# astaka-pe/Dual-DMP

Hardware: AMD Instinct MI355X
Metric: training iters/sec + MAD score, 1M-face mesh @ 1/2/4/8 MI355X (higher is better)
Workload: dtype f32 (f16x3 split-MFMA GEMMs, f32 accumulate); 1 GPU; synthetic torus-grid manifold mesh, 1000000 faces / 500000 verts, float32 features, k=(3,4,4,4,1), bnfloop=1, native numbering (BASELINE.json configs[2]); faces=1000000, verts=500000, parallelism=1 GPU, hipgraph_replay=True, two_streams=True

## Files before the change

dual-dmp_amd/csrc/ddmp_internal.h:

```cpp
#pragma once
#include "../../include/ddmp_hip.h"
#ifdef __cplusplus
extern "C" {
#endif
int ddmp_bf16_to_f32(const uint16_t* in, float* out, int64_t n, ddmp_stream stream);
int ddmp_graph_tables(const ddmp_graph* g, const int32_t** rowptr, const int32_t** col, const float** dinv);
int ddmp_bn_bwd_apply_f32(const float* dZ, int64_t lddz, const float* Y, int64_t ldy, float* dY, int64_t lddy,
                          int64_t n_rows, int C, const float* scale, const float* shift, const float* c1,
                          const float* c0, float slope, double* dbias_sums , void* workspace,
                          size_t workspace_bytes, ddmp_stream stream);
int ddmp_gemm_nn_bf16(const uint16_t* A, int64_t lda, const float* W, int64_t ldw, uint16_t* Y, int64_t ldy,
                      int64_t n_rows, int M, int K, void* workspace, size_t workspace_bytes, ddmp_stream stream);
int ddmp_gemm_nt_bf16(const uint16_t* A, int64_t lda, const float* W, int64_t ldw, uint16_t* Y, int64_t ldy,
                      int64_t n_rows, int K, int M, const float* bias, const float* pro_scale, const float* pro_shift,
                      float slope, void* workspace, size_t workspace_bytes, ddmp_stream stream);
size_t ddmp_gemm_rows_bf16_workspace_bytes(int K, int M);
int ddmp_gemm_tn_bf16(const uint16_t* G, int64_t ldg, const uint16_t* Z, int64_t ldz, float* dW, int64_t lddw,
                      int64_t n_rows, int M, int K, const float* pro_scale, const float* pro_shift, float slope,
                      void* workspace, size_t workspace_bytes, ddmp_stream stream);
size_t ddmp_gemm_tn_bf16_workspace_bytes(int64_t n_rows, int M, int K);
int ddmp_head_bwd_bf16(const uint16_t* Y, int64_t ldy, int64_t n_rows, const float* scale, const float* shift,
                       float slope, const float* W1, const float* b1, const float* W2, const float* b2, int kind,
                       const float* dout, uint16_t* dZ, int64_t lddz, float* dW1, float* db1, float* dW2, float* db2,
                       void* workspace, size_t workspace_bytes, ddmp_stream stream);
int ddmp_head_bwd_f32(const float* Y, int64_t ldy, int64_t n_rows, const float* scale, const float* shift,
                      float slope, const float* W1, const float* b1, const float* W2, const float* b2,
                      int kind, const float* dout, float* dZ, int64_t lddz, float* dW1, float* db1,
                      float* dW2, float* db2, void* workspace, size_t workspace_bytes, ddmp_stream stream);
int ddmp_head_fwd_bf16(const uint16_t* Y, int64_t ldy, int64_t n_rows, const float* scale, const float* shift,
                       float slope, const float* W1, const float* b1, const float* W2, const float* b2, int kind,
                       const float* x_pos , float* out, ddmp_stream stream);
int ddmp_head_fwd_f32(const float* Y, int64_t ldy, int64_t n_rows, const float* scale, const float* shift,
                      float slope, const float* W1, const float* b1, const float* W2, const float* b2,
                      int kind, const float* x_pos , float* out, ddmp_stream stream);
int ddmp_spmm_bf16(const ddmp_graph* g, const uint16_t* X, int64_t ldx, uint16_t* Y, int64_t ldy, int C,
                   const float* bias, const float* pro_scale, const float* pro_shift, float slope, ddmp_stream stream);
int ddmp_spmm_bnbwd_bf16(const ddmp_graph* g, const uint16_t* dZ, int64_t lddz, const uint16_t* Yb, int64_t ldyb,
                         uint16_t* out, int64_t ld_out, int C, const float* a, const float* b, const float* c1,
                         const float* c0, float slope, ddmp_stream stream);
size_t ddmp_spmm_bnred_bf16_workspace_bytes(int64_t n_rows, int C);
size_t ddmp_spmm_bnred_workspace_bytes(int64_t n_rows, int C);
#ifdef __cplusplus
}

namespace ddmp {
struct CallCtx;
}
int ddmp_bn_stats(const void* Y, int64_t ldy, int64_t n_rows, int C, int dtype, double* sums, void* workspace,
                  size_t workspace_bytes, ddmp_stream stream, ddmp::CallCtx& ctx);
int ddmp_bn_stats_f32(const float* Y, int64_t ldy, int64_t n_rows, int C, double* sums, void* workspace, size_t workspace_bytes,
                      ddmp_stream stream, ddmp::CallCtx& ctx);
int ddmp_bn_stats_bf16(const uint16_t* Y, int64_t ldy, int64_t n_rows, int C, double* sums, void* workspace,
                       size_t workspace_bytes, ddmp_stream stream, ddmp::CallCtx& ctx);
int ddmp_bn_bwd_reduce(const void* dZ, int64_t lddz, const void* Y, int64_t ldy, int64_t n_rows, int C, int dtype,
                       const float* scale, const float* shift, const float* mean, const float* rstd, float slope, double* sums2,
                       void* workspace, size_t workspace_bytes, ddmp_stream stream, ddmp::CallCtx& ctx);
int ddmp_bn_bwd_reduce_f32(const float* dZ, int64_t lddz, const float* Y, int64_t ldy, int64_t n_rows, int C, const float* scale,
                           const float* shift, const float* mean, const float* rstd, float slope, double* sums2 ,
                           void* workspace, size_t workspace_bytes, ddmp_stream stream, ddmp::CallCtx& ctx);
int ddmp_bn_bwd_reduce_bf16(const uint16_t* dZ, int64_t lddz, const uint16_t* Y, int64_t ldy, int64_t n_rows, int C,
                            const float* scale, const float* shift, const float* mean, const float* rstd, float slope,
                            double* sums2, void* workspace, size_t workspace_bytes, ddmp_stream stream, ddmp::CallCtx& ctx);
int ddmp_spmm_stats(const ddmp_graph* g, const void* X, int64_t ldx, void* Y, int64_t ldy, int C, int dtype, const float* bias,
                    const float* pro_scale, const float* pro_shift, float slope, const float* ref, double* sums2, void* workspace,
                    size_t workspace_bytes, ddmp_stream stream, ddmp::CallCtx& ctx);
int ddmp_spmm_stats_f32(const ddmp_graph* g, const float* X, int64_t ldx, float* Y, int64_t ldy, int C, const float* bias,
                        const float* pro_scale, const float* pro_shift, float slope, const float* ref ,
                        double* sums2 , void* workspace, size_t workspace_bytes, ddmp_stream stream, ddmp::CallCtx& ctx);
int ddmp_spmm_stats_bf16(const ddmp_graph* g, const uint16_t* X, int64_t ldx, uint16_t* Y, int64_t ldy, int C,
                         const float* bias , const float* pro_scale , const float* pro_shift ,
                         float slope, const float* ref , double* sums2 , void* workspace,
                         size_t workspace_bytes, ddmp_stream stream, ddmp::CallCtx& ctx);
int ddmp_spmm_bnred(const ddmp_graph* g, const void* X, int64_t ldx, void* Y, int64_t ldy, int C, int dtype, const void* Yp,
                    int64_t ldyp, const float* scale, const float* shift, const float* mean, const float* rstd, float slope,
                    double* sums2, void* workspace, size_t workspace_bytes, ddmp_stream stream, ddmp::CallCtx& ctx);
int ddmp_spmm_bnred_f32(const ddmp_graph* g, const float* X, int64_t ldx, float* Y, int64_t ldy, int C, const float* Yp,
                        int64_t ldyp, const float* scale, const float* shift, const float* mean, const float* rstd, float slope,
                        double* sums2 , void* workspace, size_t workspace_bytes, ddmp_stream stream, ddmp::CallCtx& ctx);
int ddmp_spmm_bnred_bf16(const ddmp_graph* g, const uint16_t* X, int64_t ldx, uint16_t* Y, int64_t ldy, int C, const uint16_t* Yp,
                         int64_t ldyp, const float* scale, const float* shift, const float* mean, const float* rstd, float slope,
                         double* sums2 , void* workspace, size_t workspace_bytes, ddmp_stream stream, ddmp::CallCtx& ctx);
int ddmp_gemm_nt(const void* A, int64_t lda, const float* W, int64_t ldw, void* Y, int64_t ldy, int64_t n_rows, int K, int M,
                 int dtype, const float* bias, const float* pro_scale, const float* pro_shift, float slope, void* workspace,
                 size_t workspace_bytes, ddmp_stream stream, ddmp::CallCtx& ctx);
int ddmp_gemm_nt_f32(const float* A, int64_t lda, const float* W, int64_t ldw, float* Y, int64_t ldy, int64_t n_rows, int K,
                     int M, const float* bias, const float* pro_scale, const float* pro_shift, float slope, void* workspace,
                     size_t workspace_bytes, ddmp_stream stream, ddmp::CallCtx& ctx);
int ddmp_gemm_nn(const void* A, int64_t lda, const float* W, int64_t ldw, void* Y, int64_t ldy, int64_t n_rows, int M, int K,
                 int dtype, void* workspace, size_t workspace_bytes, ddmp_stream stream, ddmp::CallCtx& ctx);
int ddmp_gemm_nn_f32(const float* A, int64_t lda, const float* W, int64_t ldw, float* Y, int64_t ldy, int64_t n_rows, int M,
                     int K, void* workspace , size_t workspace_bytes, ddmp_stream stream, ddmp::CallCtx& ctx);
int ddmp_gemm_tn(const void* G, int64_t ldg, const void* Z, int64_t ldz, float* dW, int64_t lddw, int64_t n_rows, int M, int K,
                 int dtype, const float* pro_scale, const float* pro_shift, float slope, void* workspace, size_t workspace_bytes,
                 ddmp_stream stream, ddmp::CallCtx& ctx);
int ddmp_gemm_tn_f32(const float* G, int64_t ldg, const float* Z, int64_t ldz, float* dW, int64_t lddw, int64_t n_rows, int M,
                     int K, const float* pro_scale, const float* pro_shift, float slope, void* workspace, size_t workspace_bytes,
                     ddmp_stream stream, ddmp::CallCtx& ctx);
int ddmp_gemm_nt_stats_f32(const float* A, int64_t lda, const float* W, int64_t ldw, float* Y, int64_t ldy, int64_t n_rows, int K,
                           int M, const float* bias, const float* pro_scale, const float* pro_shift, float slope, double* sums2,
                           void* workspace, size_t workspace_bytes, void* stats_ws, size_t stats_ws_bytes, ddmp_stream stream,
                           ddmp::CallCtx& ctx);
int ddmp_gemm_nt_stats_bf16(const uint16_t* A, int64_t lda, const float* W, int64_t ldw, uint16_t* Y, int64_t ldy, int64_t n_rows,
                            int K, int M, const float* bias, const float* pro_scale, const float* pro_shift, float slope,
                            double* sums2, void* workspace, size_t workspace_bytes, void* stats_ws, size_t stats_ws_bytes,
                            ddmp_stream stream, ddmp::CallCtx& ctx);
int ddmp_gemm_nn_bnred_f32(const float* A, int64_t lda, const float* W, int64_t ldw, float* out, int64_t ld_out, int64_t n_rows,
                           int M, int K, const float* Yp, int64_t ldyp, const float* scale, const float* shift, const float* mean,
                           const float* rstd, float slope, double* sums2, void* workspace, size_t workspace_bytes, void* stats_ws,
                           size_t stats_ws_bytes, ddmp_stream stream, ddmp::CallCtx& ctx);
int ddmp_gemm_nn_bnbwd_f32(const float* dZ, int64_t lddz, const float* Yb, int64_t ldyb, const float* W, int64_t ldw, float* out,
                           int64_t ld_out, int64_t n_rows, int M, int K, const float* a, const float* b, const float* c1,
                           const float* c0, float slope, void* workspace, size_t workspace_bytes, ddmp_stream stream,
                           ddmp::CallCtx& ctx);
int ddmp_gemm_tn_bnbwd_f32(const float* dZ, int64_t lddz, const float* Yb, int64_t ldyb, const float* Z, int64_t ldz, float* dW,
                           int64_t lddw, int64_t n_rows, int M, int K, const float* a, const float* b, const float* c1,
                           const float* c0, const float* pro_scale, const float* pro_shift, float slope, void* workspace,
                           size_t workspace_bytes, ddmp_stream stream, ddmp::CallCtx& ctx);
#endif
```

dual-dmp_amd/csrc/gemm.hip:

```cpp
#include "ddmp_common.h"
#include "finalize.h"
#include "gemm_tn_rm.h"

#include <algorithm>
#include <cstdlib>
#include <type_traits>
#include <vector>

namespace {

using namespace ddmp;

typedef float f32x16 __attribute__((ext_vector_type(16)));

constexpr int kBM = 128;
constexpr int kBK = 32;
constexpr int kLd = kBK + 4;

template <int TN, bool B_KMAJOR, bool PRO>
__global__ __launch_bounds__(256) void gemm_rows_kernel(
    const float* __restrict__ A, int64_t lda, const float* __restrict__ B, int64_t ldb,
    float* __restrict__ Y, int64_t ldy, int n_rows, int KD, int MD,
    const float* __restrict__ bias, const float* __restrict__ pscale, const float* __restrict__ pshift,
    float slope, int n_row_tiles, int n_col_tiles) {
// ... 592 lines not shown
        if constexpr (PM == 0) {
            if (NJ == 4) {
                if (mode == 6) DDMP_PANEL_RS(3, 4); else DDMP_PANEL_RS(2, 4);
            } else {
                if (mode == 6) DDMP_PANEL_RS(3, 2); else DDMP_PANEL_RS(2, 2);
            }
        }
#undef DDMP_PANEL_RS
    } else if (WC == 4) {
        if (mode == 6) DDMP_PANEL(2, 4, 3, 4); else DDMP_PANEL(2, 4, 2, 4);
    } else if (WC == 2) {
        if (mode == 6) DDMP_PANEL(4, 2, 3, 4); else DDMP_PANEL(4, 2, 2, 4);
    } else {
        if (NJ == 4) {
            if (mode == 6) DDMP_PANEL(8, 1, 3, 4); else DDMP_PANEL(8, 1, 2, 4);
        } else if (NJ == 2) {
            if (mode == 6) DDMP_PANEL(8, 1, 3, 2); else DDMP_PANEL(8, 1, 2, 2);
        } else {
            if (mode == 6) DDMP_PANEL(8, 1, 3, 1); else DDMP_PANEL(8, 1, 2, 1);
        }
    }
#undef DDMP_PANEL
    if (stats && sums) {
        const size_t pbytes = ((size_t)n_row_tiles * WR * 2 * MP * sizeof(double) + 255) / 256 * 256;
        fpartials_reduce(stats, n_row_tiles * WR, MP, MD, (double*)((char*)stats + pbytes), sums, st, ctx.take_fin(MD));
    }
}

static inline bool ws_ok(int KD, int MD, const float* Y, int64_t ldy, const void* ws, size_t ws_bytes) {
    return ws_enabled() && KD % 32 == 0 && KD >= 96 && MD % 4 == 0 && MD <= 1024 && ldy % 4 == 0 &&
           (reinterpret_cast<uintptr_t>(Y) & 15) == 0 && ws && (reinterpret_cast<uintptr_t>(ws) & 15) == 0 &&
           ws_bytes >= ddmp_gemm_rows_workspace_bytes(KD, MD);
}

static int g_gemm_mode = -1, g_gemm_f16 = 0;
static int gemm_mode() {
    if (g_gemm_mode < 0) {
        const char* e = getenv("DDMP_GEMM_MODE");
        int m = e ? atoi(e) : 13;
        g_gemm_f16 = m == 13 ? m : 0;
        g_gemm_mode = (m == 0 || m == 3 || m == 6) ? m : 6;
    }
    return g_gemm_mode;
}
static int gemm_f16() {
    (void)gemm_mode();
    return g_gemm_f16;
}
extern "C" int ddmp_set_gemm_mode(int mode) {
    if (mode != 0 && mode != 3 && mode != 6 && mode != 13) return DDMP_EINVAL;
    g_gemm_f16 = mode > 10 ? mode : 0;
    g_gemm_mode = mode > 10 ? 6 : mode;
    return DDMP_OK;
}
extern "C" int ddmp_get_gemm_mode(void) { return gemm_f16() ? gemm_f16() : gemm_mode(); }

extern "C" int ddmp_gemm_scales_roll(float* slots, int n_slots, ddmp_stream stream) {
    ARG_TRY(slots && n_slots > 0);
    hipLaunchKernelGGL(f16s_roll_kernel, dim3((unsigned)cdiv(n_slots, 64)), dim3(64), 0, (hipStream_t)stream, slots, n_slots);
    LAUNCH_TRY();
    return DDMP_OK;
}

static inline bool aligned16(const void* p) { return (reinterpret_cast<uintptr_t>(p) & 15) == 0; }

extern "C" size_t ddmp_gemm_rows_workspace_bytes(int K, int M) {
    if (K <= 0 || M <= 0) return 0;
    const size_t kp = ((size_t)K + 127) / 128 * 128, mp = ((size_t)M + 127) / 128 * 128;
    return 3 * kp * mp * 2;
}

static bool presplit_w(const float* W, int64_t ldw, int M, int K, int transpose, void* ws, size_t ws_bytes,
                       hipStream_t st, bool prepared) {
    const int mode = gemm_mode();
    const int RK = transpose ? M : K;
    if (mode == 0 || !ws || ws_bytes < ddmp_gemm_rows_workspace_bytes(K, M) || RK % 8 != 0 ||
        (reinterpret_cast<uintptr_t>(ws) & 15))
        return false;
    const int grid = (int)std::min<int64_t>(cdiv((int64_t)M * K, 256), 1024);
    if (w_prepared(prepared, W, ldw, ws, kWPlain, mode == 6 ? 3 : 2, M, K, transpose, 0)) return true;
    if (mode == 6)
        hipLaunchKernelGGL((split_w_kernel<3>), dim3(grid), dim3(256), 0, st, W, ldw, M, K, transpose, (__bf16*)ws);
    else
        hipLaunchKernelGGL((split_w_kernel<2>), dim3(grid), dim3(256), 0, st, W, ldw, M, K, transpose, (__bf16*)ws);
    return hipGetLastError() == hipSuccess;
}

static WPrepDesc plan_w(int form, int64_t n_rows, const float* W, int64_t ldw, int M, int K, int has_pro, void* planes,
                        size_t planes_bytes) {
    WPrepDesc d{W, planes, ldw, 0, 0, 0, 0, 0, 0};
    const int mode = gemm_mode();
    if (mode == 0 || !planes || (reinterpret_cast<uintptr_t>(planes) & 15) || planes_bytes < ddmp_gemm_rows_workspace_bytes(K, M))
        return d;
    const int KD = form ? M : K, MD = form ? K : M;
    d.transpose = form ? 1 : 0;
    d.nterm = mode == 6 ? 3 : 2;
    float dummy;
    if (!(has_pro && KD > 512) && panel_ok(KD, MD, &dummy, MD, planes, planes_bytes, n_rows)) {
        const int WC = MD > 256 ? 4 : MD > 128 ? 2 : 1;
        const int NJ = MD > 128 ? 4 : MD > 64 ? 4 : MD > 32 ? 2 : 1;
        d.P = 32 * NJ * WC;
        d.MD = MD;
        d.KD = KD;
        if (mode == 6 && WC > 1 && gemm_f16()) {
            d.kind = kWPanelF16;
            d.nterm = 2;
        } else {
            d.kind = kWPanelB16;
        }
        return d;
    }
    if (ws_ok(KD, MD, (const float*)nullptr, 4, planes, planes_bytes)) {
        d.kind = kWTiled;
        d.MD = MD;
        d.KD = KD;
        d.P = 64 * (MD > 64 ? 2 : 1);
        return d;
    }
    if (KD % 8 == 0) {
        d.kind = kWPlain;
        d.MD = M;
        d.KD = K;
    }
    return d;
}

extern "C" int ddmp_gemm_forget_planes(const void* planes) {
    for (size_t e = 0; e < g_w_registry.size();)
        if (planes == nullptr || g_w_registry[e].planes == planes) g_w_registry.erase(g_w_registry.begin() + e); else ++e;
    return DDMP_OK;
}

extern "C" int ddmp_gemm_prepare_weights(int n, const float* const* W, const int64_t* ldw, const int* M, const int* K,
                                         const int* form, const int* has_pro, void* const* planes, const size_t* planes_bytes,
                                         int64_t n_rows, float* scratch, ddmp_stream stream) {
    ARG_TRY(n > 0 && n <= kWPrepMax && W && ldw && M && K && form && planes && planes_bytes && scratch && n_rows > 0);
    WPrepBatch b;
    b.n = 0;
    bool any_f16 = false;
    for (int i = 0; i < n; ++i) {
        ARG_TRY(W[i] && M[i] > 0 && K[i] > 0 && ldw[i] >= K[i] && aligned16(W[i]) && ldw[i] % 4 == 0);
        const WPrepDesc d = plan_w(form[i], n_rows, W[i], ldw[i], M[i], K[i], has_pro ? has_pro[i] : 0, planes[i], planes_bytes[i]);
        for (size_t e = 0; e < g_w_registry.size();)
            if (g_w_registry[e].planes == planes[i]) g_w_registry.erase(g_w_registry.begin() + e); else ++e;
        if (d.kind == 0) continue;
        any_f16 |= d.kind == kWPanelF16;
        b.d[b.n++] = d;
    }
    if (b.n == 0) return DDMP_OK;
    hipStream_t st = (hipStream_t)stream;
    if (any_f16) hipLaunchKernelGGL(wprep_max_kernel, dim3(8, (unsigned)b.n), dim3(256), 0, st, b, scratch);
    hipLaunchKernelGGL(wprep_split_kernel, dim3(128, (unsigned)b.n), dim3(256), 0, st, b, (const float*)scratch);
    LAUNCH_TRY();
    for (int i = 0; i < b.n; ++i) g_w_registry.push_back(b.d[i]);
    return DDMP_OK;
}

int ddmp_gemm_nt_f32(const float* A, int64_t lda, const float* W, int64_t ldw, float* Y, int64_t ldy, int64_t n_rows, int K,
                     int M, const float* bias, const float* pro_scale, const float* pro_shift, float slope, void* workspace,
                     size_t workspace_bytes, ddmp_stream stream, ddmp::CallCtx& ctx) {
    ARG_TRY(A && W && Y && n_rows > 0 && K > 0 && M > 0 && n_rows < INT32_MAX);
    ARG_TRY(K % 4 == 0 && lda % 4 == 0 && ldw % 4 == 0 && lda >= K && ldw >= K && ldy >= M);
    ARG_TRY(aligned16(A) && aligned16(W));
    ARG_TRY((pro_scale == nullptr) == (pro_shift == nullptr));
    ARG_TRY(!pro_scale || (aligned16(pro_scale) && aligned16(pro_shift)));
    hipStream_t st = (hipStream_t)stream;
    const int n_row_tiles = (int)cdiv(n_rows, kBM);
    const int TN = M > 64 ? 2 : 1;
    const int n_col_tiles = (int)cdiv(M, 64 * TN);
    dim3 grid((unsigned)(cdiv(n_row_tiles, kXcd) * kXcd * n_col_tiles)), block(256);
    if (gemm_mode() != 0 && !(pro_scale && K > 512) && panel_ok(K, M, Y, ldy, workspace, workspace_bytes, n_rows)) {
        if (pro_scale) launch_panel<1>(gemm_mode(), A, lda, nullptr, 0, W, ldw, 0, workspace, Y, ldy, (int)n_rows, K, M, bias, pro_scale, pro_shift, nullptr, nullptr, slope, st, nullptr, nullptr, ctx);
        else launch_panel<0>(gemm_mode(), A, lda, nullptr, 0, W, ldw, 0, workspace, Y, ldy, (int)n_rows, K, M, bias, nullptr, nullptr, nullptr, nullptr, slope, st, nullptr, nullptr, ctx);
        LAUNCH_TRY();
        return DDMP_OK;
    }
    if (gemm_mode() != 0 && !(pro_scale && K > 512) && ws_ok(K, M, Y, ldy, workspace, workspace_bytes)) {
        if (pro_scale) launch_ws<true>(gemm_mode(), A, lda, W, ldw, 0, workspace, Y, ldy, (int)n_rows, K, M, bias, pro_scale, pro_shift, slope, st, ctx.prepared);
        else launch_ws<false>(gemm_mode(), A, lda, W, ldw, 0, workspace, Y, ldy, (int)n_rows, K, M, bias, nullptr, nullptr, slope, st, ctx.prepared);
        LAUNCH_TRY();
        return DDMP_OK;
    }
    const bool pre = !(pro_scale && K > 512) && presplit_w(W, ldw, M, K, 0, workspace, workspace_bytes, st, ctx.prepared);
    const float* Bop = pre ? (const float*)workspace : W;
#define DDMP_LAUNCH_NT(KERNEL_, PRO_)                                                                    \
    hipLaunchKernelGGL((KERNEL_), grid, block, 0, st, A, lda, Bop, ldw, Y, ldy, (int)n_rows, K, M, bias, \
                       pro_scale, pro_shift, slope, n_row_tiles, n_col_tiles)
#define DDMP_NT_PICK(TN_, NTERM_, PRO_)                                                                   \
    do {                                                                                                  \
        if (pre && kt_) DDMP_LAUNCH_NT((gemm_rows_bf16_kernel<TN_, NTERM_, false, PRO_, true, true>), PRO_);   \
        else if (pre) DDMP_LAUNCH_NT((gemm_rows_bf16_kernel<TN_, NTERM_, false, PRO_, false, true>), PRO_);    \
        else if (kt_) DDMP_LAUNCH_NT((gemm_rows_bf16_kernel<TN_, NTERM_, false, PRO_, true, false>), PRO_);    \
        else DDMP_LAUNCH_NT((gemm_rows_bf16_kernel<TN_, NTERM_, false, PRO_, false, false>), PRO_);            \
    } while (0)
#define DDMP_NT_BY_MODE(TN_, PRO_)                                                          \
    do {                                                                                    \
        const int mode_ = (PRO_ && K > 512) ? 0 : gemm_mode();                              \
        const bool kt_ = (K % 16) != 0;                                                     \
        if (mode_ == 6) DDMP_NT_PICK(TN_, 3, PRO_);                                         \
        else if (mode_ == 3) DDMP_NT_PICK(TN_, 2, PRO_);                                    \
        else hipLaunchKernelGGL((gemm_rows_kernel<TN_, false, PRO_>), grid, block, 0, st, A, lda, W, ldw, Y, ldy,  \
                                (int)n_rows, K, M, bias, pro_scale, pro_shift, slope, n_row_tiles, n_col_tiles); \
    } while (0)
    if (TN == 2) {
        if (pro_scale) DDMP_NT_BY_MODE(2, true); else DDMP_NT_BY_MODE(2, false);
    } else {
        if (pro_scale) DDMP_NT_BY_MODE(1, true); else DDMP_NT_BY_MODE(1, false);
    }
#undef DDMP_NT_PICK
#undef DDMP_NT_BY_MODE
#undef DDMP_LAUNCH_NT
    LAUNCH_TRY();
    return DDMP_OK;
}
extern "C" int ddmp_gemm_nt_f32(const float* A, int64_t lda, const float* W, int64_t ldw, float* Y,
                                int64_t ldy, int64_t n_rows, int K, int M, const float* bias,
                                const float* pro_scale, const float* pro_shift, float slope,
                                void* workspace, size_t workspace_bytes, ddmp_stream stream) {
    ddmp::CallCtx ctx;
    return ddmp_gemm_nt_f32(A, lda, W, ldw, Y, ldy, n_rows, K, M, bias, pro_scale, pro_shift, slope, workspace, workspace_bytes,
                            stream, ctx);
}

int ddmp_gemm_nn_f32(const float* A, int64_t lda, const float* W, int64_t ldw, float* Y, int64_t ldy, int64_t n_rows, int M,
                     int K, void* workspace, size_t workspace_bytes, ddmp_stream stream, ddmp::CallCtx& ctx) {
    ARG_TRY(A && W && Y && n_rows > 0 && K > 0 && M > 0 && n_rows < INT32_MAX);
    ARG_TRY(M % 4 == 0 && K % 4 == 0 && lda % 4 == 0 && ldw % 4 == 0 && lda >= M && ldw >= K && ldy >= K);
    ARG_TRY(aligned16(A) && aligned16(W));
    hipStream_t st = (hipStream_t)stream;
    const int n_row_tiles = (int)cdiv(n_rows, kBM);
    const int TN = K > 64 ? 2 : 1;
    const int n_col_tiles = (int)cdiv(K, 64 * TN);
    dim3 grid((unsigned)(cdiv(n_row_tiles, kXcd) * kXcd * n_col_tiles)), block(256);
    if (gemm_mode() != 0 && panel_ok(M, K, Y, ldy, workspace, workspace_bytes, n_rows)) {
        launch_panel<0>(gemm_mode(), A, lda, nullptr, 0, W, ldw, 1, workspace, Y, ldy, (int)n_rows, M, K, nullptr, nullptr, nullptr, nullptr, nullptr, 0.f, st, nullptr, nullptr, ctx);
        LAUNCH_TRY();
        return DDMP_OK;
    }
    if (gemm_mode() != 0 && ws_ok(M, K, Y, ldy, workspace, workspace_bytes)) {
        launch_ws<false>(gemm_mode(), A, lda, W, ldw, 1, workspace, Y, ldy, (int)n_rows, M, K, nullptr, nullptr, nullptr, 0.f, st, ctx.prepared);
        LAUNCH_TRY();
        return DDMP_OK;
    }
    const bool pre = presplit_w(W, ldw, M, K, 1, workspace, workspace_bytes, st, ctx.prepared);
#define DDMP_LAUNCH_NN(KERNEL_)                                                                        \
    hipLaunchKernelGGL((KERNEL_), grid, block, 0, st, A, lda, W, ldw, Y, ldy, (int)n_rows, M, K, nullptr, \
                       nullptr, nullptr, 0.f, n_row_tiles, n_col_tiles)
#define DDMP_LAUNCH_NNP(KERNEL_)                                                                       \
    hipLaunchKernelGGL((KERNEL_), grid, block, 0, st, A, lda, (const float*)workspace, (int64_t)M, Y, ldy, \
                       (int)n_rows, M, K, nullptr, nullptr, nullptr, 0.f, n_row_tiles, n_col_tiles)
    const int mode = gemm_mode();
    const bool kt = (M % 16) != 0;
    if (pre) {
        if (TN == 2) {
            if (mode == 6 && kt) DDMP_LAUNCH_NNP((gemm_rows_bf16_kernel<2, 3, false, false, true, true>));
            else if (mode == 6) DDMP_LAUNCH_NNP((gemm_rows_bf16_kernel<2, 3, false, false, false, true>));
            else if (kt) DDMP_LAUNCH_NNP((gemm_rows_bf16_kernel<2, 2, false, false, true, true>));
            else DDMP_LAUNCH_NNP((gemm_rows_bf16_kernel<2, 2, false, false, false, true>));
        } else {
            if (mode == 6 && kt) DDMP_LAUNCH_NNP((gemm_rows_bf16_kernel<1, 3, false, false, true, true>));
            else if (mode == 6) DDMP_LAUNCH_NNP((gemm_rows_bf16_kernel<1, 3, false, false, false, true>));
            else if (kt) DDMP_LAUNCH_NNP((gemm_rows_bf16_kernel<1, 2, false, false, true, true>));
            else DDMP_LAUNCH_NNP((gemm_rows_bf16_kernel<1, 2, false, false, false, true>));
        }
    } else if (TN == 2) {
        if (mode == 6 && kt) DDMP_LAUNCH_NN((gemm_rows_bf16_kernel<2, 3, true, false, true, false>));
        else if (mode == 6) DDMP_LAUNCH_NN((gemm_rows_bf16_kernel<2, 3, true, false, false, false>));
        else if (mode == 3 && kt) DDMP_LAUNCH_NN((gemm_rows_bf16_kernel<2, 2, true, false, true, false>));
        else if (mode == 3) DDMP_LAUNCH_NN((gemm_rows_bf16_kernel<2, 2, true, false, false, false>));
        else DDMP_LAUNCH_NN((gemm_rows_kernel<2, true, false>));
    } else {
        if (mode == 6 && kt) DDMP_LAUNCH_NN((gemm_rows_bf16_kernel<1, 3, true, false, true, false>));
        else if (mode == 6) DDMP_LAUNCH_NN((gemm_rows_bf16_kernel<1, 3, true, false, false, false>));
        else if (mode == 3 && kt) DDMP_LAUNCH_NN((gemm_rows_bf16_kernel<1, 2, true, false, true, false>));
        else if (mode == 3) DDMP_LAUNCH_NN((gemm_rows_bf16_kernel<1, 2, true, false, false, false>));
        else DDMP_LAUNCH_NN((gemm_rows_kernel<1, true, false>));
    }
#undef DDMP_LAUNCH_NNP
#undef DDMP_LAUNCH_NN
    LAUNCH_TRY();
    return DDMP_OK;
}

static inline bool tn_wide_ok(int rows_per_split, int64_t ld0, int64_t ld1, int64_t ld2) {
    const int64_t r = (int64_t)rows_per_split + 64, lim = (int64_t)1 << 31;
    return r * ld0 * 4 < lim && r * ld1 * 4 < lim && r * ld2 * 4 < lim;
}
static void launch_tn_wide(const float* G, int64_t ldg, const float* G2, int64_t ldg2, const float* Z, int64_t ldz, float* part,
                           int64_t sstride, int64_t n_rows, int M, int K, const TnPlan& p, const float* ps, const float* psh,
                           const float* ga, const float* gb, const float* gk1, const float* gk0, float slope, float* gslot,
                           float* zslot, int target, int heal, hipStream_t st) {
    ddmp::TnRmArgs a;
    a.G = G; a.ldg = ldg; a.G2 = G2; a.ldg2 = ldg2; a.Z = Z; a.ldz = ldz; a.part = part; a.ld_out = K; a.split_stride = sstride;
    a.n_rows = (int)n_rows; a.M = M; a.K = K; a.rows_per_split = p.rows_per_split; a.n_tiles_m = p.n_tiles_m;
    a.n_tiles_k = p.n_tiles_k; a.n_splits = p.n_splits; a.pscale = ps; a.pshift = psh; a.ga = ga; a.gb = gb; a.gk1 = gk1;
    a.gk0 = gk0; a.slope = slope; a.gslot = gslot; a.zslot = zslot; a.target = target; a.heal = heal;
    a.tm = p.tm; a.tk = p.tk;
    ddmp::launch_tn_rm(a, st);
}

extern "C" size_t ddmp_gemm_tn_workspace_bytes(int64_t n_rows, int M, int K) {
    if (n_rows <= 0 || M <= 0 || K <= 0) return 0;
    const TnPlan p = tn_plan(n_rows, M, K), q = tn_plan(n_rows, M, K, true);
    return (size_t)std::max(p.n_splits, q.n_splits) * (size_t)M * (size_t)K * sizeof(float) + 64;
}

int ddmp_gemm_tn_f32(const float* G, int64_t ldg, const float* Z, int64_t ldz, float* dW, int64_t lddw, int64_t n_rows, int M,
                     int K, const float* pro_scale, const float* pro_shift, float slope, void* workspace, size_t workspace_bytes,
                     ddmp_stream stream, ddmp::CallCtx& ctx) {
    ARG_TRY(G && Z && dW && n_rows > 0 && M > 0 && K > 0 && n_rows < INT32_MAX);
    ARG_TRY(M % 4 == 0 && K % 4 == 0 && ldg % 4 == 0 && ldz % 4 == 0 && ldg >= M && ldz >= K && lddw >= K);
    ARG_TRY(aligned16(G) && aligned16(Z));
    ARG_TRY((pro_scale == nullptr) == (pro_shift == nullptr));
    ARG_TRY(!pro_scale || (aligned16(pro_scale) && aligned16(pro_shift)));
    hipStream_t st = (hipStream_t)stream;
    const bool f16_route = gemm_mode() == 6 && gemm_f16();
    TnPlan p = tn_plan(n_rows, M, K, f16_route);
    if (p.T == 4 && p.tm + p.tk < 512 && !tn_wide_ok(p.rows_per_split, ldg, 0, ldz)) p = tn_plan(n_rows, M, K);
    const size_t need = (size_t)p.n_splits * (size_t)M * (size_t)K * sizeof(float) + 64;
    if (!workspace || workspace_bytes < need) return DDMP_EWORKSPACE;
    float* part = (float*)workspace;
    const int64_t sstride = (int64_t)M * K;
    const int n_tiles = p.n_tiles_m * p.n_tiles_k;
    if (p.T == 4) {
        dim3 pgrid((unsigned)(cdiv(p.n_splits, kXcd) * kXcd * n_tiles)), pblock(512);
        float* gslot = nullptr;
        float* zslot = nullptr;
        int target = 0, heal_ = 0;
#define DDMP_LAUNCH_TNP(KERNEL_)                                                                              \
    hipLaunchKernelGGL((KERNEL_), pgrid, pblock, 0, st, G, ldg, (const float*)nullptr, (int64_t)0, Z, ldz, part, \
                       (int64_t)K, sstride, (int)n_rows, M, K, p.rows_per_split, p.n_tiles_m, p.n_tiles_k,       \
                       p.n_splits, pro_scale, pro_shift, (const float*)nullptr, (const float*)nullptr,           \
                       (const float*)nullptr, (const float*)nullptr, slope, gslot, zslot, target, heal_)
        const int mode_ = gemm_mode();
        if (mode_ == 6 && gemm_f16() && tn_wide_ok(p.rows_per_split, ldg, 0, ldz)) {
            float* tail = (float*)((char*)workspace + need - 64);
            const bool own = !(ctx.slot_a && ctx.slot_b);
            gslot = own ? tail : ctx.slot_a;
            zslot = own ? tail + 4 : ctx.slot_b;
            const bool prime = own || ctx.prime;
            target = prime ? kF16TargetExact : kF16TargetStale;
            if (prime) {
                f16s_measure<0>(G, ldg, nullptr, 0, n_rows, M, nullptr, nullptr, nullptr, nullptr, slope, gslot, st);
                if (pro_scale) f16s_measure<1>(Z, ldz, nullptr, 0, n_rows, K, pro_scale, pro_shift, nullptr, nullptr, slope, zslot, st);
                else f16s_measure<0>(Z, ldz, nullptr, 0, n_rows, K, nullptr, nullptr, nullptr, nullptr, slope, zslot, st);
            }
            for (heal_ = 0; heal_ <= (prime ? 0 : 1); ++heal_)
                launch_tn_wide(G, ldg, nullptr, 0, Z, ldz, part, sstride, n_rows, M, K, p, pro_scale, pro_shift, nullptr, nullptr,
                               nullptr, nullptr, slope, gslot, zslot, target, heal_, st);
            heal_ = 0;
        } else if (pro_scale) {
            if (mode_ == 6) DDMP_LAUNCH_TNP((gemm_tn_panel_kernel<3, true, false>)); else DDMP_LAUNCH_TNP((gemm_tn_panel_kernel<2, true, false>));
        } else {
            if (mode_ == 6) DDMP_LAUNCH_TNP((gemm_tn_panel_kernel<3, false, false>)); else DDMP_LAUNCH_TNP((gemm_tn_panel_kernel<2, false, false>));
        }
#undef DDMP_LAUNCH_TNP
        LAUNCH_TRY();
        hipLaunchKernelGGL(reduce_splits_kernel, dim3((unsigned)cdiv((int64_t)M * K, 256)), dim3(256), 0, st, part,
                           sstride, p.n_splits, dW, lddw, M, K);
        LAUNCH_TRY();
        return DDMP_OK;
    }
    dim3 grid((unsigned)(cdiv(p.n_splits, kXcd) * kXcd * n_tiles)), block(256);
#define DDMP_LAUNCH_TN(KERNEL_)                                                                           \
    hipLaunchKernelGGL((KERNEL_), grid, block, 0, st, G, ldg, Z, ldz, part, (int64_t)K, sstride, (int)n_rows, \
                       M, K, p.rows_per_split, p.n_tiles_m, p.n_tiles_k, p.n_splits, pro_scale, pro_shift, slope)
#define DDMP_TN_BY_MODE(T_, PRO_)                                                 \
    do {                                                                          \
        const int mode_ = gemm_mode();                                            \
        if (mode_ == 6) DDMP_LAUNCH_TN((gemm_tn_bf16_kernel<T_, 3, PRO_, (T_ == 1 ? 32 : 16)>));       \
        else if (mode_ == 3) DDMP_LAUNCH_TN((gemm_tn_bf16_kernel<T_, 2, PRO_, (T_ == 1 ? 32 : 16)>));  \
        else DDMP_LAUNCH_TN((gemm_tn_kernel<T_, PRO_>));                          \
    } while (0)
    if (p.T == 2) {
        if (pro_scale) DDMP_TN_BY_MODE(2, true); else DDMP_TN_BY_MODE(2, false);
    } else {
        if (pro_scale) DDMP_TN_BY_MODE(1, true); else DDMP_TN_BY_MODE(1, false);
    }
#undef DDMP_TN_BY_MODE
#undef DDMP_LAUNCH_TN
    LAUNCH_TRY();
    hipLaunchKernelGGL(reduce_splits_kernel, dim3((unsigned)cdiv((int64_t)M * K, 256)), dim3(256), 0, st, part,
                       sstride, p.n_splits, dW, lddw, M, K);
    LAUNCH_TRY();
    return DDMP_OK;
}


extern "C" int ddmp_gemm_nn_bnred_supported(int M, int K, int64_t n_rows) {
    if (gemm_mode() == 6 && gemm_f16() && rr_enabled() && panel_enabled() && n_rows >= kRRMinRows && M % 32 == 0 && M >= 64 &&
        M <= kMaxProK && K > 128 && K <= 512 && K % 4 == 0)
        return 1;
    static const bool narrow = !ddmp::unfused("dgrad_red_narrow");
    return (narrow && (gemm_mode() == 6 || gemm_mode() == 3) && panel_enabled() && n_rows >= kPanelMinRows && M % 32 == 0 &&
            M >= 32 && M <= kMaxProK && (K == 128 || K == 64)) ? 2 : 0;
}
int ddmp_gemm_nn_bnred_f32(const float* A, int64_t lda, const float* W, int64_t ldw, float* out, int64_t ld_out, int64_t n_rows,
                           int M, int K, const float* Yp, int64_t ldyp, const float* scale, const float* shift, const float* mean,
                           const float* rstd, float slope, double* sums2, void* workspace, size_t workspace_bytes, void* stats_ws,
                           size_t stats_ws_bytes, ddmp_stream stream, ddmp::CallCtx& ctx) {
    ARG_TRY(A && W && out && Yp && scale && shift && mean && rstd && sums2 && n_rows > 0 && n_rows < INT32_MAX);
    ARG_TRY(M % 4 == 0 && K % 4 == 0 && lda % 4 == 0 && ldw % 4 == 0 && lda >= M && ldw >= K && ld_out >= K && ldyp >= K);
    ARG_TRY(aligned16(A) && aligned16(W));
    const int form = ddmp_gemm_nn_bnred_supported(M, K, n_rows);
    if (!form || (form == 1 && !rr_route_ok(n_rows, M, lda, 0)) || !panel_ok(M, K, out, ld_out, workspace, workspace_bytes, n_rows))
        return DDMP_EINVAL;
    if (stats_ws_bytes < ddmp_gemm_nt_stats_workspace_bytes(n_rows, K)) return DDMP_EWORKSPACE;
    const float* bn4[4] = {scale, shift, mean, rstd};
    launch_panel<0>(gemm_mode(), A, lda, nullptr, 0, W, ldw, 1, workspace, out, ld_out, (int)n_rows, M, K, nullptr, nullptr, nullptr,
                    nullptr, nullptr, slope, (hipStream_t)stream, (double*)stats_ws, sums2, ctx, Yp, ldyp, bn4);
    LAUNCH_TRY();
    return DDMP_OK;
}
extern "C" int ddmp_gemm_nn_bnred_f32(const float* A, int64_t lda, const float* W, int64_t ldw, float* out, int64_t ld_out,
                                      int64_t n_rows, int M, int K, const float* Yp, int64_t ldyp, const float* scale,
                                      const float* shift, const float* mean, const float* rstd, float slope, double* sums2,
                                      void* workspace, size_t workspace_bytes, void* stats_ws, size_t stats_ws_bytes,
                                      ddmp_stream stream) {
    ddmp::CallCtx ctx;
    return ddmp_gemm_nn_bnred_f32(A, lda, W, ldw, out, ld_out, n_rows, M, K, Yp, ldyp, scale, shift, mean, rstd, slope, sums2,
                                  workspace, workspace_bytes, stats_ws, stats_ws_bytes, stream, ctx);
}

extern "C" int ddmp_gemm_bnbwd_supported(int cout, int cin, int64_t n_rows) {
    if (gemm_mode() == 0 || !panel_enabled() || !tn_panel_enabled() || n_rows < kTnPanelMinRows) return 0;
    const bool nn = cout % 32 == 0 && cout >= 64 && cout <= kMaxProK && cin % 4 == 0 && cin >= 16 && cin <= 512;
    const bool tn = cout % 4 == 0 && ((cout >= 256 && cin >= 256) || cin <= 128);
    static const bool narrow = !ddmp::unfused("bnbwd_narrow");
    return (nn && tn && (cin > 128 || narrow)) ? 1 : 0;
}

extern "C" int ddmp_gemm_tn_bnbwd_supported(int cout, int cin, int64_t n_rows) {
    if (gemm_mode() == 0 || !tn_panel_enabled() || n_rows < kTnPanelMinRows) return 0;
    const int mode_ = gemm_mode();
    const bool panel = cout >= 256 && cin >= 256;
    return (cout % 4 == 0 && cin % 4 == 0 && (panel || mode_ == 6 || mode_ == 3)) ? 1 : 0;
}

int ddmp_gemm_nn_bnbwd_f32(const float* dZ, int64_t lddz, const float* Yb, int64_t ldyb, const float* W, int64_t ldw, float* out,
                           int64_t ld_out, int64_t n_rows, int M, int K, const float* a, const float* b, const float* c1,
                           const float* c0, float slope, void* workspace, size_t workspace_bytes, ddmp_stream stream,
                           ddmp::CallCtx& ctx) {
    ARG_TRY(dZ && Yb && W && out && a && b && c1 && c0 && n_rows > 0 && n_rows < INT32_MAX && M > 0 && K > 0);
    ARG_TRY(lddz % 4 == 0 && ldyb % 4 == 0 && ldw % 4 == 0 && lddz >= M && ldyb >= M && ldw >= K && ld_out >= K);
    ARG_TRY(aligned16(dZ) && aligned16(Yb) && aligned16(W));
    if (!ddmp_gemm_bnbwd_supported(M, K, n_rows) || !panel_ok(M, K, out, ld_out, workspace, workspace_bytes, n_rows)) return DDMP_EINVAL;
    launch_panel<2>(gemm_mode(), dZ, lddz, Yb, ldyb, W, ldw, 1, workspace, out, ld_out, (int)n_rows, M, K, nullptr, a, b,
                    c1, c0, slope, (hipStream_t)stream, nullptr, nullptr, ctx);
    LAUNCH_TRY();
    return DDMP_OK;
}
extern "C" int ddmp_gemm_nn_bnbwd_f32(const float* dZ, int64_t lddz, const float* Yb, int64_t ldyb, const float* W,
                                      int64_t ldw, float* out, int64_t ld_out, int64_t n_rows, int M, int K,
                                      const float* a, const float* b, const float* c1, const float* c0, float slope,
                                      void* workspace, size_t workspace_bytes, ddmp_stream stream) {
    ddmp::CallCtx ctx;
    return ddmp_gemm_nn_bnbwd_f32(dZ, lddz, Yb, ldyb, W, ldw, out, ld_out, n_rows, M, K, a, b, c1, c0, slope, workspace,
                                  workspace_bytes, stream, ctx);
}

int ddmp_gemm_tn_bnbwd_f32(const float* dZ, int64_t lddz, const float* Yb, int64_t ldyb, const float* Z, int64_t ldz, float* dW,
                           int64_t lddw, int64_t n_rows, int M, int K, const float* a, const float* b, const float* c1,
                           const float* c0, const float* pro_scale, const float* pro_shift, float slope, void* workspace,
                           size_t workspace_bytes, ddmp_stream stream, ddmp::CallCtx& ctx) {
    ARG_TRY(dZ && Yb && Z && dW && a && b && c1 && c0 && n_rows > 0 && n_rows < INT32_MAX && M > 0 && K > 0);
    ARG_TRY(M % 4 == 0 && K % 4 == 0 && lddz >= M && ldyb >= M && ldz >= K && lddw >= K);
    ARG_TRY((pro_scale == nullptr) == (pro_shift == nullptr));
    if (!ddmp_gemm_tn_bnbwd_supported(M, K, n_rows)) return DDMP_EINVAL;
    hipStream_t st = (hipStream_t)stream;
    const bool f16_route = gemm_mode() == 6 && gemm_f16() && lddz % 4 == 0 && ldyb % 4 == 0 && ldz % 4 == 0 && aligned16(dZ) &&
                           aligned16(Yb) && aligned16(Z);
    TnPlan p = tn_plan(n_rows, M, K, f16_route);
    if (p.T == 4 && p.tm + p.tk < 512 && !tn_wide_ok(p.rows_per_split, lddz, ldyb, ldz)) p = tn_plan(n_rows, M, K);
    const size_t need = (size_t)p.n_splits * (size_t)M * (size_t)K * sizeof(float) + 64;
    if (!workspace || workspace_bytes < need) return DDMP_EWORKSPACE;
    float* part = (float*)workspace;
    const int64_t sstride = (int64_t)M * K;
    const int n_tiles = p.n_tiles_m * p.n_tiles_k;
    if (p.T != 4) {
        const int mode_ = gemm_mode();
        if (mode_ != 6 && mode_ != 3) return DDMP_EINVAL;
        dim3 grid((unsigned)(cdiv(p.n_splits, kXcd) * kXcd * n_tiles)), block(256);
#define DDMP_LAUNCH_TNG(T_, NT_, PRO_)                                                                                 \
    hipLaunchKernelGGL((gemm_tn_bf16_kernel<T_, NT_, PRO_, (T_ == 1 ? 32 : 16), true>), grid, block, 0, st, dZ, lddz, Z, ldz,  \
                       part, (int64_t)K, sstride, (int)n_rows, M, K, p.rows_per_split, p.n_tiles_m, p.n_tiles_k,       \
                       p.n_splits, pro_scale, pro_shift, slope, Yb, ldyb, a, b, c1, c0)
        if (p.T == 2) {
            if (mode_ == 6) { if (pro_scale) DDMP_LAUNCH_TNG(2, 3, true); else DDMP_LAUNCH_TNG(2, 3, false); }
            else { if (pro_scale) DDMP_LAUNCH_TNG(2, 2, true); else DDMP_LAUNCH_TNG(2, 2, false); }
        } else {
            if (mode_ == 6) { if (pro_scale) DDMP_LAUNCH_TNG(1, 3, true); else DDMP_LAUNCH_TNG(1, 3, false); }
            else { if (pro_scale) DDMP_LAUNCH_TNG(1, 2, true); else DDMP_LAUNCH_TNG(1, 2, false); }
        }
#undef DDMP_LAUNCH_TNG
        LAUNCH_TRY();
        hipLaunchKernelGGL(reduce_splits_kernel, dim3((unsigned)cdiv((int64_t)M * K, 256)), dim3(256), 0, st, part, sstride,
                           p.n_splits, dW, lddw, M, K);
        LAUNCH_TRY();
        return DDMP_OK;
    }
    dim3 pgrid((unsigned)(cdiv(p.n_splits, kXcd) * kXcd * n_tiles)), pblock(512);
    float* gslot = nullptr;
    float* zslot = nullptr;
    int target = 0, heal_ = 0;
#define DDMP_LAUNCH_TNP(KERNEL_)                                                                                 \
    hipLaunchKernelGGL((KERNEL_), pgrid, pblock, 0, st, dZ, lddz, Yb, ldyb, Z, ldz, part, (int64_t)K, sstride,     \
                       (int)n_rows, M, K, p.rows_per_split, p.n_tiles_m, p.n_tiles_k, p.n_splits, pro_scale,       \
                       pro_shift, a, b, c1, c0, slope, gslot, zslot, target, heal_)
    const int mode_ = gemm_mode();
    if (mode_ == 6 && gemm_f16() && lddz % 4 == 0 && ldyb % 4 == 0 && ldz % 4 == 0 && tn_wide_ok(p.rows_per_split, lddz, ldyb, ldz) &&
        aligned16(dZ) && aligned16(Yb) && aligned16(Z)) {
        float* tail = (float*)((char*)workspace + need - 64);
        const bool own = !(ctx.slot_a && ctx.slot_b);
        gslot = own ? tail : ctx.slot_a;
        zslot = own ? tail + 4 : ctx.slot_b;
        const bool prime = own || ctx.prime;
        target = prime ? kF16TargetExact : kF16TargetStale;
        if (prime) {
            f16s_measure<2>(dZ, lddz, Yb, ldyb, n_rows, M, a, b, c1, c0, slope, gslot, st);
            if (pro_scale) f16s_measure<1>(Z, ldz, nullptr, 0, n_rows, K, pro_scale, pro_shift, nullptr, nullptr, slope, zslot, st);
            else f16s_measure<0>(Z, ldz, nullptr, 0, n_rows, K, nullptr, nullptr, nullptr, nullptr, slope, zslot, st);
        }
        for (heal_ = 0; heal_ <= (prime ? 0 : 1); ++heal_)
            launch_tn_wide(dZ, lddz, Yb, ldyb, Z, ldz, part, sstride, n_rows, M, K, p, pro_scale, pro_shift, a, b, c1, c0, slope,
                           gslot, zslot, target, heal_, st);
        heal_ = 0;
    } else if (pro_scale) {
        if (mode_ == 6) DDMP_LAUNCH_TNP((gemm_tn_panel_kernel<3, true, true>)); else DDMP_LAUNCH_TNP((gemm_tn_panel_kernel<2, true, true>));
    } else {
        if (mode_ == 6) DDMP_LAUNCH_TNP((gemm_tn_panel_kernel<3, false, true>)); else DDMP_LAUNCH_TNP((gemm_tn_panel_kernel<2, false, true>));
    }
#undef DDMP_LAUNCH_TNP
    LAUNCH_TRY();
    hipLaunchKernelGGL(reduce_splits_kernel, dim3((unsigned)cdiv((int64_t)M * K, 256)), dim3(256), 0, st, part, sstride,
                       p.n_splits, dW, lddw, M, K);
    LAUNCH_TRY();
    return DDMP_OK;
}
extern "C" int ddmp_gemm_tn_bnbwd_f32(const float* dZ, int64_t lddz, const float* Yb, int64_t ldyb, const float* Z,
                                      int64_t ldz, float* dW, int64_t lddw, int64_t n_rows, int M, int K,
                                      const float* a, const float* b, const float* c1, const float* c0,
                                      const float* pro_scale, const float* pro_shift, float slope, void* workspace,
                                      size_t workspace_bytes, ddmp_stream stream) {
    ddmp::CallCtx ctx;
    return ddmp_gemm_tn_bnbwd_f32(dZ, lddz, Yb, ldyb, Z, ldz, dW, lddw, n_rows, M, K, a, b, c1, c0, pro_scale, pro_shift, slope,
                                  workspace, workspace_bytes, stream, ctx);
}


extern "C" size_t ddmp_gemm_nt_stats_workspace_bytes(int64_t n_rows, int M) {
    if (n_rows <= 0 || M <= 0) return 0;
    const size_t fused = (size_t)(cdiv(n_rows, 64) + 8) * 2 * 512 * sizeof(double) + 256 + fpartials_mid_bytes(512);
    return std::max(fused, ddmp_colreduce_workspace_bytes(n_rows, M));
}

int ddmp_gemm_nt_stats_f32(const float* A, int64_t lda, const float* W, int64_t ldw, float* Y, int64_t ldy, int64_t n_rows, int K,
                           int M, const float* bias, const float* pro_scale, const float* pro_shift, float slope, double* sums2,
                           void* workspace, size_t workspace_bytes, void* stats_ws, size_t stats_ws_bytes, ddmp_stream stream,
                           ddmp::CallCtx& ctx) {
    ARG_TRY(sums2 && stats_ws);
    if (stats_ws_bytes < ddmp_gemm_nt_stats_workspace_bytes(n_rows, M)) return DDMP_EWORKSPACE;
    const bool fused = A && W && Y && n_rows > 0 && n_rows < INT32_MAX && K > 0 && M > 0 && K % 4 == 0 && lda % 4 == 0 &&
                       ldw % 4 == 0 && lda >= K && ldw >= K && ldy >= M && aligned16(A) && aligned16(W) &&
                       (pro_scale == nullptr) == (pro_shift == nullptr) && gemm_mode() != 0 && !(pro_scale && K > 512) &&
                       panel_ok(K, M, Y, ldy, workspace, workspace_bytes, n_rows);
    if (fused) {
        hipStream_t st = (hipStream_t)stream;
        if (pro_scale) launch_panel<1>(gemm_mode(), A, lda, nullptr, 0, W, ldw, 0, workspace, Y, ldy, (int)n_rows, K, M, bias, pro_scale, pro_shift, nullptr, nullptr, slope, st, (double*)stats_ws, sums2, ctx);
        else launch_panel<0>(gemm_mode(), A, lda, nullptr, 0, W, ldw, 0, workspace, Y, ldy, (int)n_rows, K, M, bias, nullptr, nullptr, nullptr, nullptr, slope, st, (double*)stats_ws, sums2, ctx);
        LAUNCH_TRY();
        return DDMP_OK;
    }
    int rc = ddmp_gemm_nt_f32(A, lda, W, ldw, Y, ldy, n_rows, K, M, bias, pro_scale, pro_shift, slope, workspace,
                              workspace_bytes, stream, ctx);
    if (rc != DDMP_OK) return rc;
    return ddmp_bn_stats_f32(Y, ldy, n_rows, M, sums2, stats_ws, stats_ws_bytes, stream, ctx);
}
extern "C" int ddmp_gemm_nt_stats_f32(const float* A, int64_t lda, const float* W, int64_t ldw, float* Y, int64_t ldy,
                                      int64_t n_rows, int K, int M, const float* bias, const float* pro_scale,
                                      const float* pro_shift, float slope, double* sums2, void* workspace,
                                      size_t workspace_bytes, void* stats_ws, size_t stats_ws_bytes,
                                      ddmp_stream stream) {
    ddmp::CallCtx ctx;
    return ddmp_gemm_nt_stats_f32(A, lda, W, ldw, Y, ldy, n_rows, K, M, bias, pro_scale, pro_shift, slope, sums2, workspace,
                                  workspace_bytes, stats_ws, stats_ws_bytes, stream, ctx);
}
```

dual-dmp_amd/csrc/head.hip:

```cpp
#include "b16_common.h"

#include <algorithm>

namespace {

using namespace ddmp;

constexpr int H0 = 32, H1 = 16, H2 = 3;
constexpr int kNPar = H1 * H0 + H1 + H2 * H1 + H2;

struct HeadW {
    const float *W1, *b1, *W2, *b2;
};

__device__ __forceinline__ void load_row32(const float* __restrict__ yrow, float (&y)[H0]) {
#pragma unroll
    for (int q = 0; q < H0 / 4; ++q) {
        const float4 v = *reinterpret_cast<const float4*>(yrow + q * 4);
        y[q * 4 + 0] = v.x; y[q * 4 + 1] = v.y; y[q * 4 + 2] = v.z; y[q * 4 + 3] = v.w;
    }
}
__device__ __forceinline__ void load_row32(const bf16_t* __restrict__ yrow, float (&y)[H0]) {
#pragma unroll
    for (int q = 0; q < H0 / 8; ++q) {
        float t[8];
        bf_unpack8(ld8b(yrow + q * 8), t);
#pragma unroll
        for (int e = 0; e < 8; ++e) y[q * 8 + e] = t[e];
    }
}
__device__ __forceinline__ void store_quad(float* p, const float (&d)[4]) {
    *reinterpret_cast<float4*>(p) = make_float4(d[0], d[1], d[2], d[3]);
}
__device__ __forceinline__ void store_quad(bf16_t* p, const float (&d)[4]) {
    *reinterpret_cast<uint2*>(p) = make_uint2(bf_pack(d[0], d[1]), bf_pack(d[2], d[3]));
}

template <typename T>
__device__ __forceinline__ void head_forward_row(const T* __restrict__ yrow, const float* __restrict__ scale,
                                                 const float* __restrict__ shift, float slope, const HeadW& w,
                                                 float (&z)[H0], float (&tp)[H1], float (&u)[H2]) {
    load_row32(yrow, z);
#pragma unroll
    for (int j = 0; j < H0; ++j) z[j] = lrelu(fmaf(z[j], scale[j], shift[j]), slope);
#pragma unroll
    for (int i = 0; i < H1; ++i) {
        float s = w.b1[i];
#pragma unroll
        for (int j = 0; j < H0; ++j) s = fmaf(w.W1[i * H0 + j], z[j], s);
        tp[i] = s;
    }
#pragma unroll
    for (int o = 0; o < H2; ++o) {
        float s = w.b2[o];
#pragma unroll
        for (int i = 0; i < H1; ++i) s = fmaf(w.W2[o * H1 + i], lrelu(tp[i], slope), s);
        u[o] = s;
    }
}

template <typename T>
__global__ __launch_bounds__(256) void head_fwd_kernel(const T* __restrict__ Y, int64_t ldy, int n_rows,
                                                       const float* __restrict__ scale,
                                                       const float* __restrict__ shift, float slope, HeadW w,
                                                       int kind, const float* __restrict__ x_pos,
                                                       float* __restrict__ out) {
    for (int row = blockIdx.x * 256 + threadIdx.x; row < n_rows; row += gridDim.x * 256) {
        float z[H0], tp[H1], u[H2];
        head_forward_row(Y + (int64_t)row * ldy, scale, shift, slope, w, z, tp, u);
        float* o = out + (int64_t)row * 3;
        if (kind == 0) {
            const float* xp = x_pos + (int64_t)row * 3;
            o[0] = xp[0] + u[0];
            o[1] = xp[1] + u[1];
            o[2] = xp[2] + u[2];
        } else {
            const float v0 = tanhf(u[0]), v1 = tanhf(u[1]), v2 = tanhf(u[2]);
            const float r = sqrtf(v0 * v0 + v1 * v1 + v2 * v2);
            const float s = 1.0f / (r + 1.0e-12f);
            o[0] = v0 * s;
            o[1] = v1 * s;
            o[2] = v2 * s;
        }
    }
}

template <typename T>
__global__ __launch_bounds__(256) void head_bwd_kernel(const T* __restrict__ Y, int64_t ldy, int n_rows,
                                                       const float* __restrict__ scale,
                                                       const float* __restrict__ shift, float slope, HeadW w,
                                                       int kind, const float* __restrict__ dout,
                                                       T* __restrict__ dZ, int64_t lddz,
                                                       float* __restrict__ partial ) {
    __shared__ float zs[256][H0 + 1];
    __shared__ float dtps[256][H1 + 1];
    __shared__ float ts[256][H1 + 1];
    __shared__ float dus[256][4];
    const int tid = threadIdx.x;
    const int w1_j = tid & 31, w1_i = tid >> 5;
    float accA = 0.f, accB = 0.f;
    float accC = 0.f;

    const int n_tiles = (n_rows + 255) / 256;
    for (int tile = blockIdx.x; tile < n_tiles; tile += gridDim.x) {
        const int row = tile * 256 + tid;
        float z[H0], tp[H1], u[H2], du[H2], dtp[H1];
        if (row < n_rows) {
            head_forward_row(Y + (int64_t)row * ldy, scale, shift, slope, w, z, tp, u);
            const float* g = dout + (int64_t)row * 3;
            if (kind == 0) {
                du[0] = g[0]; du[1] = g[1]; du[2] = g[2];
            } else {
                const float v0 = tanhf(u[0]), v1 = tanhf(u[1]), v2 = tanhf(u[2]);
                const float r = sqrtf(v0 * v0 + v1 * v1 + v2 * v2);
                const float s = 1.0f / (r + 1.0e-12f);
                const float gv = g[0] * v0 + g[1] * v1 + g[2] * v2;
                const float k = r > 0.f ? s * s * gv / r : 0.f;
                du[0] = (s * g[0] - k * v0) * (1.f - v0 * v0);
                du[1] = (s * g[1] - k * v1) * (1.f - v1 * v1);
                du[2] = (s * g[2] - k * v2) * (1.f - v2 * v2);
            }
#pragma unroll
            for (int i = 0; i < H1; ++i) {
                float s = 0.f;
#pragma unroll
                for (int o = 0; o < H2; ++o) s = fmaf(w.W2[o * H1 + i], du[o], s);
                dtp[i] = s * lrelu_grad(tp[i], slope);
            }
            T* dz = dZ + (int64_t)row * lddz;
#pragma unroll
            for (int q = 0; q < H0 / 4; ++q) {
                float d[4];
#pragma unroll
                for (int e = 0; e < 4; ++e) {
                    float s = 0.f;
#pragma unroll
                    for (int i = 0; i < H1; ++i) s = fmaf(w.W1[i * H0 + q * 4 + e], dtp[i], s);
                    d[e] = s;
                }
                store_quad(dz + q * 4, d);
            }
        } else {
#pragma unroll
            for (int j = 0; j < H0; ++j) z[j] = 0.f;
#pragma unroll
            for (int i = 0; i < H1; ++i) { tp[i] = 0.f; dtp[i] = 0.f; }
            du[0] = du[1] = du[2] = 0.f;
        }
        __syncthreads();
#pragma unroll
        for (int j = 0; j < H0; ++j) zs[tid][j] = z[j];
#pragma unroll
        for (int i = 0; i < H1; ++i) {
            dtps[tid][i] = dtp[i];
            ts[tid][i] = row < n_rows ? lrelu(tp[i], slope) : 0.f;
        }
        dus[tid][0] = du[0]; dus[tid][1] = du[1]; dus[tid][2] = du[2];
        __syncthreads();
        for (int r = 0; r < 256; ++r) {
            const float zj = zs[r][w1_j];
            accA = fmaf(dtps[r][w1_i], zj, accA);
            accB = fmaf(dtps[r][w1_i + 8], zj, accB);
        }
        if (tid < H2 * H1) {
            const int o = tid / H1, i = tid % H1;
            for (int r = 0; r < 256; ++r) accC = fmaf(dus[r][o], ts[r][i], accC);
        } else if (tid >= 64 && tid < 64 + H1) {
            for (int r = 0; r < 256; ++r) accC += dtps[r][tid - 64];
        } else if (tid >= 128 && tid < 128 + H2) {
            for (int r = 0; r < 256; ++r) accC += dus[r][tid - 128];
        }
    }
    float* p = partial + (int64_t)blockIdx.x * kNPar;
    p[w1_i * H0 + w1_j] = accA;
    p[(w1_i + 8) * H0 + w1_j] = accB;
    if (tid < H2 * H1) p[H1 * H0 + H1 + tid] = accC;
    else if (tid >= 64 && tid < 64 + H1) p[H1 * H0 + (tid - 64)] = accC;
    else if (tid >= 128 && tid < 128 + H2) p[H1 * H0 + H1 + H2 * H1 + (tid - 128)] = accC;
}

__global__ __launch_bounds__(256) void head_reduce_kernel(const float* __restrict__ partial, int nblk,
                                                          float* __restrict__ dW1, float* __restrict__ db1,
                                                          float* __restrict__ dW2, float* __restrict__ db2) {
    __shared__ double sm[256];
    const int i = blockIdx.x * 32 + (threadIdx.x & 31), sl = threadIdx.x >> 5;
    double s = 0.0;
    if (i < kNPar)
        for (int b = sl; b < nblk; b += 8) s += (double)partial[(int64_t)b * kNPar + i];
    sm[threadIdx.x] = s;
    __syncthreads();
    if (sl != 0 || i >= kNPar) return;
    double r = 0.0;
#pragma unroll
    for (int u = 0; u < 8; ++u) r += sm[threadIdx.x + 32 * u];
    const float v = (float)r;
    if (i < H1 * H0) dW1[i] = v;
    else if (i < H1 * H0 + H1) db1[i - H1 * H0] = v;
    else if (i < H1 * H0 + H1 + H2 * H1) dW2[i - H1 * H0 - H1] = v;
    else db2[i - H1 * H0 - H1 - H2 * H1] = v;
}

int head_bwd_blocks(int64_t n_rows) { return (int)std::max<int64_t>(1, std::min<int64_t>(512, cdiv(n_rows, 256))); }

}

extern "C" int ddmp_head_fwd_f32(const float* Y, int64_t ldy, int64_t n_rows, const float* scale,
                                 const float* shift, float slope, const float* W1, const float* b1,
                                 const float* W2, const float* b2, int kind, const float* x_pos, float* out,
                                 ddmp_stream stream) {
    ARG_TRY(Y && scale && shift && W1 && b1 && W2 && b2 && out && n_rows > 0 && n_rows < INT32_MAX);
    ARG_TRY(ldy >= H0 && ldy % 4 == 0 && (kind == 0 || kind == 1) && (kind == 1 || x_pos));
    const int grid = (int)std::min<int64_t>(cdiv(n_rows, 256), 256 * 8);
    HeadW w{W1, b1, W2, b2};
    hipLaunchKernelGGL(head_fwd_kernel<float>, dim3(grid), dim3(256), 0, (hipStream_t)stream, Y, ldy, (int)n_rows, scale,
                       shift, slope, w, kind, x_pos, out);
    LAUNCH_TRY();
    return DDMP_OK;
}

extern "C" size_t ddmp_head_bwd_workspace_bytes(int64_t n_rows) {
    if (n_rows <= 0) return 0;
    return (size_t)head_bwd_blocks(n_rows) * kNPar * sizeof(float);
}

extern "C" int ddmp_head_bwd_f32(const float* Y, int64_t ldy, int64_t n_rows, const float* scale,
                                 const float* shift, float slope, const float* W1, const float* b1,
                                 const float* W2, const float* b2, int kind, const float* dout, float* dZ,
                                 int64_t lddz, float* dW1, float* db1, float* dW2, float* db2, void* ws,
                                 size_t ws_bytes, ddmp_stream stream) {
    ARG_TRY(Y && scale && shift && W1 && b1 && W2 && b2 && dout && dZ && dW1 && db1 && dW2 && db2);
    ARG_TRY(n_rows > 0 && n_rows < INT32_MAX && ldy >= H0 && ldy % 4 == 0 && lddz >= H0 && lddz % 4 == 0);
    ARG_TRY(kind == 0 || kind == 1);
    const int nblk = head_bwd_blocks(n_rows);
    if (!ws || ws_bytes < (size_t)nblk * kNPar * sizeof(float)) return DDMP_EWORKSPACE;
    HeadW w{W1, b1, W2, b2};
    hipLaunchKernelGGL(head_bwd_kernel<float>, dim3(nblk), dim3(256), 0, (hipStream_t)stream, Y, ldy, (int)n_rows, scale,
                       shift, slope, w, kind, dout, dZ, lddz, (float*)ws);
    LAUNCH_TRY();
    hipLaunchKernelGGL(head_reduce_kernel, dim3((unsigned)cdiv(kNPar, 32)), dim3(256), 0, (hipStream_t)stream,
                       (const float*)ws, nblk, dW1, db1, dW2, db2);
    LAUNCH_TRY();
    return DDMP_OK;
}


extern "C" int ddmp_head_fwd_bf16(const uint16_t* Y, int64_t ldy, int64_t n_rows, const float* scale, const float* shift,
                                  float slope, const float* W1, const float* b1, const float* W2, const float* b2,
                                  int kind, const float* x_pos, float* out, ddmp_stream stream) {
    ARG_TRY(Y && scale && shift && W1 && b1 && W2 && b2 && out && n_rows > 0 && n_rows < INT32_MAX);
    ARG_TRY(ldy >= H0 && ldy % 8 == 0 && b16_aligned(Y) && (kind == 0 || kind == 1) && (kind == 1 || x_pos));
    const int grid = (int)std::min<int64_t>(cdiv(n_rows, 256), 256 * 8);
    HeadW w{W1, b1, W2, b2};
    hipLaunchKernelGGL(head_fwd_kernel<bf16_t>, dim3(grid), dim3(256), 0, (hipStream_t)stream, Y, ldy, (int)n_rows, scale,
                       shift, slope, w, kind, x_pos, out);
    LAUNCH_TRY();
    return DDMP_OK;
}

extern "C" int ddmp_head_bwd_bf16(const uint16_t* Y, int64_t ldy, int64_t n_rows, const float* scale, const float* shift,
                                  float slope, const float* W1, const float* b1, const float* W2, const float* b2,
                                  int kind, const float* dout, uint16_t* dZ, int64_t lddz, float* dW1, float* db1,
                                  float* dW2, float* db2, void* ws, size_t ws_bytes, ddmp_stream stream) {
    ARG_TRY(Y && scale && shift && W1 && b1 && W2 && b2 && dout && dZ && dW1 && db1 && dW2 && db2);
    ARG_TRY(n_rows > 0 && n_rows < INT32_MAX && ldy >= H0 && ldy % 8 == 0 && lddz >= H0 && lddz % 8 == 0);
    ARG_TRY((kind == 0 || kind == 1) && b16_aligned(Y) && b16_aligned(dZ));
    const int nblk = head_bwd_blocks(n_rows);
    if (!ws || ws_bytes < (size_t)nblk * kNPar * sizeof(float)) return DDMP_EWORKSPACE;
    HeadW w{W1, b1, W2, b2};
    hipLaunchKernelGGL(head_bwd_kernel<bf16_t>, dim3(nblk), dim3(256), 0, (hipStream_t)stream, Y, ldy, (int)n_rows, scale,
                       shift, slope, w, kind, dout, dZ, lddz, (float*)ws);
    LAUNCH_TRY();
    hipLaunchKernelGGL(head_reduce_kernel, dim3((unsigned)cdiv(kNPar, 32)), dim3(256), 0, (hipStream_t)stream,
                       (const float*)ws, nblk, dW1, db1, dW2, db2);
    LAUNCH_TRY();
    return DDMP_OK;
}
```

dual-dmp_amd/csrc/opts.hip:

```cpp
#include "ddmp_common.h"
#include "finalize.h"

namespace {
using ddmp::FinalizeArgs;

struct OptCall {
    int err = DDMP_OK;
    ddmp::CallCtx ctx;
    const double* sums;
    ddmp_stream stream;
    OptCall(const ddmp_opts* o, ddmp_stream stream_, const double* sums_ = nullptr, int width = 0) : sums(sums_), stream(stream_) {
        if (o) err = fill(*o, width);
    }
    int fill(const ddmp_opts& o, int width) {
        ARG_TRY(o.struct_size >= sizeof(ddmp_opts));
        ARG_TRY(!(o.flags & ~(DDMP_OPT_BN_FWD | DDMP_OPT_BN_BWD | DDMP_OPT_SCALES | DDMP_OPT_PREPARED)));
        ARG_TRY(!((o.flags & DDMP_OPT_BN_FWD) && (o.flags & DDMP_OPT_BN_BWD)));
        if (o.flags & (DDMP_OPT_BN_FWD | DDMP_OPT_BN_BWD)) {
            FinalizeArgs& f = ctx.fin;
            f.kind = (o.flags & DDMP_OPT_BN_FWD) ? 1 : 2;
            f.C = o.bn_C; f.n_total = o.bn_n_total; f.eps = o.bn_eps; f.momentum = o.bn_momentum;
            for (int i = 0; i < 3; ++i) f.in[i] = o.bn_in[i];
            for (int i = 0; i < 6; ++i) f.out[i] = o.bn_out[i];
            ARG_TRY(sums && f.C == width && f.n_total > 0 && f.C > 0 && f.in[0] && f.in[1] && f.out[0] && f.out[1] && f.out[2] && f.out[3]);
            if (f.kind == 1) ARG_TRY((f.out[4] == nullptr) == (f.out[5] == nullptr));
            else ARG_TRY(f.in[2]);
        }
        if (o.flags & DDMP_OPT_SCALES) {
            ctx.slot_a = o.slot_a; ctx.slot_b = o.slot_b; ctx.prime = o.prime;
        }
        ctx.prepared = (o.flags & DDMP_OPT_PREPARED) != 0;
        return DDMP_OK;
    }
    int finish(int rc) {
        const FinalizeArgs& f = ctx.fin;
        if (rc != DDMP_OK || f.kind == 0 || ctx.fin_done) return rc;
        if (f.kind == 1)
            return ddmp_bn_prepare_f32(sums, f.n_total, f.C, f.in[0], f.in[1], f.eps, f.momentum, f.out[0], f.out[1], f.out[2],
                                       f.out[3], f.out[4], f.out[5], stream);
        return ddmp_bn_bwd_prepare_f32(sums, f.n_total, f.C, f.in[0], f.in[1], f.in[2], f.out[0], f.out[1], f.out[2], f.out[3], stream);
    }
};
}

extern "C" int ddmp_bn_stats_o(const void* Y, int64_t ldy, int64_t n_rows, int C, int dtype, double* sums, void* workspace, size_t workspace_bytes, ddmp_stream stream, const ddmp_opts* opts) {
    OptCall c(opts, stream, sums, C);
    if (c.err) return c.err;
    return c.finish(ddmp_bn_stats(Y, ldy, n_rows, C, dtype, sums, workspace, workspace_bytes, stream, c.ctx));
}

extern "C" int ddmp_bn_bwd_reduce_o(const void* dZ, int64_t lddz, const void* Y, int64_t ldy, int64_t n_rows, int C, int dtype, const float* scale, const float* shift, const float* mean, const float* rstd, float slope, double* sums2, void* workspace, size_t workspace_bytes, ddmp_stream stream, const ddmp_opts* opts) {
    OptCall c(opts, stream, sums2, C);
    if (c.err) return c.err;
    return c.finish(ddmp_bn_bwd_reduce(dZ, lddz, Y, ldy, n_rows, C, dtype, scale, shift, mean, rstd, slope, sums2, workspace, workspace_bytes, stream, c.ctx));
}

extern "C" int ddmp_spmm_stats_o(const ddmp_graph* g, const void* X, int64_t ldx, void* Y, int64_t ldy, int C, int dtype, const float* bias, const float* pro_scale, const float* pro_shift, float slope, const float* ref, double* sums2, void* workspace, size_t workspace_bytes, ddmp_stream stream, const ddmp_opts* opts) {
    OptCall c(opts, stream, sums2, C);
    if (c.err) return c.err;
    return c.finish(ddmp_spmm_stats(g, X, ldx, Y, ldy, C, dtype, bias, pro_scale, pro_shift, slope, ref, sums2, workspace, workspace_bytes, stream, c.ctx));
}

extern "C" int ddmp_spmm_bnred_o(const ddmp_graph* g, const void* X, int64_t ldx, void* Y, int64_t ldy, int C, int dtype, const void* Yp, int64_t ldyp, const float* scale, const float* shift, const float* mean, const float* rstd, float slope, double* sums2, void* workspace, size_t workspace_bytes, ddmp_stream stream, const ddmp_opts* opts) {
    OptCall c(opts, stream, sums2, C);
    if (c.err) return c.err;
    return c.finish(ddmp_spmm_bnred(g, X, ldx, Y, ldy, C, dtype, Yp, ldyp, scale, shift, mean, rstd, slope, sums2, workspace, workspace_bytes, stream, c.ctx));
}

extern "C" int ddmp_gemm_nt_o(const void* A, int64_t lda, const float* W, int64_t ldw, void* Y, int64_t ldy, int64_t n_rows, int K, int M, int dtype, const float* bias, const float* pro_scale, const float* pro_shift, float slope, void* workspace, size_t workspace_bytes, ddmp_stream stream, const ddmp_opts* opts) {
    OptCall c(opts, stream);
    if (c.err) return c.err;
    return c.finish(ddmp_gemm_nt(A, lda, W, ldw, Y, ldy, n_rows, K, M, dtype, bias, pro_scale, pro_shift, slope, workspace, workspace_bytes, stream, c.ctx));
}

extern "C" int ddmp_gemm_nn_o(const void* A, int64_t lda, const float* W, int64_t ldw, void* Y, int64_t ldy, int64_t n_rows, int M, int K, int dtype, void* workspace, size_t workspace_bytes, ddmp_stream stream, const ddmp_opts* opts) {
    OptCall c(opts, stream);
    if (c.err) return c.err;
    return c.finish(ddmp_gemm_nn(A, lda, W, ldw, Y, ldy, n_rows, M, K, dtype, workspace, workspace_bytes, stream, c.ctx));
}

extern "C" int ddmp_gemm_tn_o(const void* G, int64_t ldg, const void* Z, int64_t ldz, float* dW, int64_t lddw, int64_t n_rows, int M, int K, int dtype, const float* pro_scale, const float* pro_shift, float slope, void* workspace, size_t workspace_bytes, ddmp_stream stream, const ddmp_opts* opts) {
    OptCall c(opts, stream);
    if (c.err) return c.err;
    return c.finish(ddmp_gemm_tn(G, ldg, Z, ldz, dW, lddw, n_rows, M, K, dtype, pro_scale, pro_shift, slope, workspace, workspace_bytes, stream, c.ctx));
}

extern "C" int ddmp_gemm_nt_stats_f32_o(const float* A, int64_t lda, const float* W, int64_t ldw, float* Y, int64_t ldy, int64_t n_rows, int K, int M, const float* bias , const float* pro_scale , const float* pro_shift , float slope, double* sums2 , void* workspace, size_t workspace_bytes, void* stats_ws, size_t stats_ws_bytes, ddmp_stream stream, const ddmp_opts* opts) {
    OptCall c(opts, stream, sums2, M);
    if (c.err) return c.err;
    return c.finish(ddmp_gemm_nt_stats_f32(A, lda, W, ldw, Y, ldy, n_rows, K, M, bias, pro_scale, pro_shift, slope, sums2, workspace, workspace_bytes, stats_ws, stats_ws_bytes, stream, c.ctx));
}

extern "C" int ddmp_gemm_nt_stats_bf16_o(const uint16_t* A, int64_t lda, const float* W, int64_t ldw, uint16_t* Y, int64_t ldy, int64_t n_rows, int K, int M, const float* bias, const float* pro_scale, const float* pro_shift, float slope, double* sums2, void* workspace, size_t workspace_bytes, void* stats_ws, size_t stats_ws_bytes, ddmp_stream stream, const ddmp_opts* opts) {
    OptCall c(opts, stream, sums2, M);
    if (c.err) return c.err;
    return c.finish(ddmp_gemm_nt_stats_bf16(A, lda, W, ldw, Y, ldy, n_rows, K, M, bias, pro_scale, pro_shift, slope, sums2, workspace, workspace_bytes, stats_ws, stats_ws_bytes, stream, c.ctx));
}

extern "C" int ddmp_gemm_nn_bnred_f32_o(const float* A, int64_t lda, const float* W, int64_t ldw, float* out, int64_t ld_out, int64_t n_rows, int M, int K, const float* Yp, int64_t ldyp, const float* scale, const float* shift, const float* mean, const float* rstd, float slope, double* sums2, void* workspace, size_t workspace_bytes, void* stats_ws, size_t stats_ws_bytes, ddmp_stream stream, const ddmp_opts* opts) {
    OptCall c(opts, stream, sums2, K);
    if (c.err) return c.err;
    return c.finish(ddmp_gemm_nn_bnred_f32(A, lda, W, ldw, out, ld_out, n_rows, M, K, Yp, ldyp, scale, shift, mean, rstd, slope, sums2, workspace, workspace_bytes, stats_ws, stats_ws_bytes, stream, c.ctx));
}

extern "C" int ddmp_gemm_nn_bnbwd_f32_o(const float* dZ, int64_t lddz, const float* Yb, int64_t ldyb, const float* W, int64_t ldw, float* out, int64_t ld_out, int64_t n_rows, int M, int K, const float* a, const float* b, const float* c1, const float* c0, float slope, void* workspace, size_t workspace_bytes, ddmp_stream stream, const ddmp_opts* opts) {
    OptCall c(opts, stream);
    if (c.err) return c.err;
    return c.finish(ddmp_gemm_nn_bnbwd_f32(dZ, lddz, Yb, ldyb, W, ldw, out, ld_out, n_rows, M, K, a, b, c1, c0, slope, workspace, workspace_bytes, stream, c.ctx));
}

extern "C" int ddmp_gemm_tn_bnbwd_f32_o(const float* dZ, int64_t lddz, const float* Yb, int64_t ldyb, const float* Z, int64_t ldz, float* dW, int64_t lddw, int64_t n_rows, int M, int K, const float* a, const float* b, const float* c1, const float* c0, const float* pro_scale , const float* pro_shift , float slope, void* workspace, size_t workspace_bytes, ddmp_stream stream, const ddmp_opts* opts) {
    OptCall c(opts, stream);
    if (c.err) return c.err;
    return c.finish(ddmp_gemm_tn_bnbwd_f32(dZ, lddz, Yb, ldyb, Z, ldz, dW, lddw, n_rows, M, K, a, b, c1, c0, pro_scale, pro_shift, slope, workspace, workspace_bytes, stream, c.ctx));
}
```

dual-dmp_amd/engine.py:

```python
from __future__ import annotations

import math
from typing import List, Optional

import os

import torch

from . import ops
from .ops import SLOPE

def _unfused(name):
    f = getattr(ops, "unfused", None)
    return bool(f and f(name))


POS_WIDTHS = [16, 32, 64, 128, 256, 256, 512, 512, 256, 256, 128, 64, 32, 16, 3]
NORM_WIDTHS = [7, 32, 64, 128, 256, 256, 512, 512, 256, 256, 128, 64, 32, 16, 3]


def _pad4(c):
    return (c + 3) // 4 * 4


# ... 100 lines not shown
                a = math.sqrt(6.0 / (true[0] + true[1]))
                v[:, :true[1]].copy_(torch.empty(true).uniform_(-a, a, generator=generator))
            elif name.startswith("bn") and name.endswith("weight"):
                v.fill_(1.0)
            elif name.startswith("linear"):
                fan_in = 32 if name.startswith("linear1") else 16
                b = 1.0 / math.sqrt(fan_in)
                v.copy_(torch.empty(stored).uniform_(-b, b, generator=generator))
        with torch.no_grad():
            arena.copy_(cpu.to(arena.device))


class GcnEngine:

    def __init__(self, graph: ops.Graph, widths: List[int], kind: int, x0: torch.Tensor,
                 x_pos: Optional[torch.Tensor] = None, comm=None, n_total: Optional[int] = None,
                 perm: Optional[torch.Tensor] = None, dtype: torch.dtype = torch.float32, split=None, overlap: bool = False):
        if dtype not in (torch.float32, torch.bfloat16):
            raise ValueError("feature dtype must be torch.float32 or torch.bfloat16")
        self.dtype = dtype
        self.g = graph
        self.overlap = bool(overlap)
        self.split = None
        if self.overlap and split is not None and 0 < split[2] < graph.n_rows:
            self.split = tuple(split)
            self.n_int = int(split[2])
        self._halo_ahead = None
        self.kind = kind
        self.layout = ArenaLayout(widths)
        self.comm = comm or NoComm()
        self.n_rows, self.n_cols = graph.n_rows, graph.n_cols
        self.n_total = float(n_total if n_total is not None else graph.n_rows)
        dev = x0.device
        self.device = dev
        L = self.layout
        assert x0.shape[0] >= self.n_cols and x0.shape[1] == L.cin[0]
        self.x0 = torch.zeros((self.n_cols, L.cin_p[0]), dtype=dtype, device=dev)
        self.x0[:, :L.cin[0]] = x0[:self.n_cols].to(dtype)
        self.x_pos = None if x_pos is None else x_pos[:self.n_rows].contiguous().to(torch.float32)
        eq_agg = not _unfused("equal_width")
        self.agg_first = [L.cin_p[l] < L.cout[l] or (eq_agg and L.cin_p[l] == L.cout[l]) for l in range(12)]
        supported = getattr(ops, "gemm_bnbwd_supported", None)
        def _bnbwd_ok(l):
            if not supported or l == 0 or not self.agg_first[l]:
                return False
            if dtype == torch.float32:
                return supported(L.cout[l], L.cin_p[l], self.n_rows)
            try:
                return supported(L.cout[l], L.cin_p[l], self.n_rows, dtype) and not _unfused("bf16_gemm")
            except TypeError:
                return False
        self.fuse_bnbwd = [bool(_bnbwd_ok(l)) for l in range(12)]
        tn_ok = getattr(ops, "gemm_tn_bnbwd_supported", None)
        self.fuse_bnbwd0 = bool(tn_ok and self.agg_first[0] and tn_ok(L.cout[0], L.cin_p[0], self.n_rows, dtype)
                                and not _unfused("bnbwd_l0"))
        gather_ok = getattr(ops, "spmm_bnbwd_supported", None)
        few_entries = dtype == torch.float32 or getattr(graph, "max_row_nnz", 99) <= 4
        self.fuse_gather_bwd = [bool(gather_ok) and isinstance(self.comm, NoComm) and not self.agg_first[l] and l > 0
                                and gather_ok(L.cout[l]) and few_entries and not _unfused("gather_bwd")
                                for l in range(12)]
        cmax = max(L.cout)
        nc = self.n_cols

        def buf(c):
            return torch.empty((nc, c), dtype=dtype, device=dev)

        self.Y = [buf(L.cout[l]) for l in range(12)]
        self.P = [buf(L.cin_p[l]) if self.agg_first[l] else None for l in range(12)]
        self._flat = [torch.empty(nc * cmax, dtype=dtype, device=dev) for _ in range(6)]
        self.bn4 = [torch.zeros((4, L.cout[l]), dtype=torch.float32, device=dev) for l in range(12)]
        st_ok = getattr(ops, "spmm_stats_supported", None)
        self.fuse_spmm_stats = [bool(st_ok) and not self.agg_first[l] and st_ok(L.cout[l], dtype)
                                and not _unfused("stats") for l in range(12)]
        self.c10s = [torch.empty((2, L.cout[l]), dtype=torch.float32, device=dev) for l in range(12)]
        self._wplanes = None
        self._prep_weights = (dtype == torch.float32 and hasattr(ops, "gemm_prepare_weights")
                              and not _unfused("wprep"))
        self._tail_fused = (isinstance(self.comm, NoComm) and hasattr(ops, "BnFwd")
                            and not _unfused("tail"))
        self.scale_slots = torch.zeros((12, 2, 4), dtype=torch.float32, device=dev)
        self._slot = [[self.scale_slots[l, o] for o in range(2)] for l in range(12)]
        self._prime = True
        self._f16 = False
        self.sums = torch.empty(2 * cmax, dtype=torch.float64, device=dev)
        self.sums_b = torch.empty(2 * cmax, dtype=torch.float64, device=dev) if self.split else None
        self.running = [torch.zeros((2, L.cout[l]), dtype=torch.float32, device=dev) for l in range(12)]
        for r in self.running:
            r[1].fill_(1.0)
        self.num_batches_tracked = torch.zeros(12, dtype=torch.int64, device=dev)
        self.out = torch.empty((self.n_rows, 3), dtype=torch.float32, device=dev)
        self._p1_ready = False
        self.perm = self.inv = None
        if perm is not None:
            self.perm = perm.to(dev)
            self.inv = torch.empty_like(self.perm)
            self.inv[self.perm] = torch.arange(self.n_rows, device=dev)
            self.out_orig = torch.empty_like(self.out)

    def __del__(self):
        try:
            planes = getattr(self, "_wplanes", None)
            if planes and hasattr(ops, "gemm_forget_planes"):
                for buf in planes.values():
                    ops.gemm_forget_planes(buf)
        except Exception:
            pass

    def _work(self, i, c):
        return self._flat[i][: self.n_cols * c].view(self.n_cols, c)

    def _scales(self, l, a, b=None):
        if self._f16:
            return {"scales": (self._slot[l][a], None if b is None else self._slot[l][b], self._prime)}
        return {}

    def check_scales(self) -> int:
        cnt = self.scale_slots[:, :, 3]
        c = cnt.cpu()
        if bool((c < 0).any()):
            where = [(int(l), int(o)) for l, o in (c < 0).nonzero().tolist()]
            cnt.zero_()
            raise OverflowError("non-finite GEMM operand (layer, operand): %s -- NaN or inf in the activations / "
                                "gradients of the last iterations" % where)
        healed = int(c.sum().item())
        if healed:
            cnt.zero_()
        return healed

    @staticmethod
    def _drain(steps):
        for h in steps:
            if h is not None:
                h.wait()

    def forward(self, params: torch.Tensor, update_running: bool = True, use_running: bool = False) -> torch.Tensor:
        self._drain(self.forward_steps(params, update_running, use_running))
        return self.result

    def backward(self, params: torch.Tensor, grads: torch.Tensor, dout: torch.Tensor) -> torch.Tensor:
        self._drain(self.backward_steps(params, grads, dout))
        return grads

    def _bn4_from_running(self, l, gamma, beta):
        rm, rv = self.running[l][0], self.running[l][1]
        rstd = torch.rsqrt(rv + ops.BN_EPS)
        b = self.bn4[l]
        b[0] = gamma * rstd
        b[1] = beta - rm * b[0]
        b[2] = rm
        b[3] = rstd

    def _prepare_weights(self, params: torch.Tensor):
        if not self._prep_weights:
            return
        L = self.layout
        if self._wplanes is None:
            need = ops.gemm_rows_workspace_bytes
            self._wplanes = {(l, form): torch.empty(need(L.cin_p[l], L.cout[l]), dtype=torch.uint8, device=self.device)
                             for l in range(12) for form in (0, 1) if not (form == 1 and l == 0)}
            self._wscratch = torch.empty(8 * len(self._wplanes), dtype=torch.float32, device=self.device)
            self._wplan = (None, None)
        if self._wplan[0] != params.data_ptr():
            items = []
            for (l, form), buf in self._wplanes.items():
                W = L.view(params, "conv%d.lin.weight" % (l + 1), true_shape=False)
                items.append((W, form, form == 0 and not self.agg_first[l] and l > 0, buf))
            self._wplan = (params.data_ptr(), ops.WeightPlan(items, self.n_rows, self._wscratch))
        self._wplan[1].run()

    def _wp(self, l, form):
        return {} if self._wplanes is None else {"wplanes": self._wplanes[(l, form)]}

    def _start_halo(self, t):
        comm, n = self.comm, self.n_rows
        start = getattr(comm, "start_halo_overlapped", None)
        if start is None or os.environ.get("DDMP_DIST_SPLIT") == "noverlap":
            h = comm.start_halo(t, n)
            if h is not None:
                h.wait()
            return None
        return start(t, n)

    def _halves(self):
        g_int, g_bnd, ni = self.split
        return ((g_int, 0, ni, self.sums), (g_bnd, ni, self.n_rows, self.sums_b))

    def _add_sums(self, width):
        if self.split:
            self.sums[:width] += self.sums_b[:width]

    def _agg(self, launch, h):
        if self.split:
            for k, (gh, r0, r1, sums) in enumerate(self._halves()):
                if k == 1:
                    yield h
                launch(gh, r0, r1, sums)
        else:
            yield h
            launch(self.g, 0, self.n_rows, self.sums)

    def forward_steps(self, params: torch.Tensor, update_running: bool = True, use_running: bool = False):
        L, g, n, comm = self.layout, self.g, self.n_rows, self.comm
        self.n_forward = getattr(self, "n_forward", 0) + 1
        self._f16 = hasattr(ops, "gemm_scales_roll") and self.dtype == torch.float32 and ops.get_gemm_mode() == 13
        self._prepare_weights(params)
        X, pro = self.x0, None
        halo_started = False
        tail = self._tail_fused and not use_running
        for l in range(12):
            i = l + 1
            W = L.view(params, "conv%d.lin.weight" % i, true_shape=False)
            b = L.view(params, "conv%d.bias" % i)
            Y = self.Y[l]
            bnk = {"bn": ops.BnFwd(self.n_total, L.view(params, "bn%d.weight" % i), L.view(params, "bn%d.bias" % i), self.bn4[l],
                                   running=(self.running[l][0], self.running[l][1]) if update_running else None)} if tail else {}
            if self.agg_first[l]:
                P = self.P[l]
                if self.overlap and l > 0:
                    h = self._halo_ahead if halo_started else self._start_halo(X)
                    self._halo_ahead = None
                    yield from self._agg(lambda gh, r0, r1, _: ops.spmm(gh, X, out=P[r0:r1], pro=pro), h)
                elif l > 0 or not self._p1_ready:
                    if l > 0 and not halo_started:
                        yield comm.start_halo(X, n)
                    ops.spmm(g, X, out=P[:n], pro=pro)
                    self._p1_ready = True
                if hasattr(ops, "gemm_nt_stats"):
                    ops.gemm_nt_stats(P, W, self.sums, out=Y, bias=b, n_rows=n, **self._wp(l, 0), **self._scales(l, 0), **bnk)
                else:
                    ops.gemm_nt(P, W, out=Y, bias=b, n_rows=n)
                    ops.bn_stats(Y, sums=self.sums, n_rows=n, **bnk)
            else:
                H = self._work(0, L.cout[l])
                ops.gemm_nt(X, W, out=H, pro=pro, n_rows=n, **self._wp(l, 0), **self._scales(l, 0))
                if self.overlap:
                    if self.fuse_spmm_stats[l]:
                        yield from self._agg(lambda gh, r0, r1, sums: ops.spmm_stats(gh, H, Y[r0:r1], self.bn4[l][2], sums, bias=b),
                                             self._start_halo(H))
                        self._add_sums(2 * L.cout[l])
                    else:
                        yield from self._agg(lambda gh, r0, r1, _: ops.spmm(gh, H, out=Y[r0:r1], bias=b), self._start_halo(H))
                        ops.bn_stats(Y, sums=self.sums, n_rows=n, **bnk)
                else:
                    yield comm.start_halo(H, n)
                    if self.fuse_spmm_stats[l]:
                        ops.spmm_stats(g, H, Y[:n], self.bn4[l][2], self.sums, bias=b, **bnk)
                    else:
                        ops.spmm(g, H, out=Y[:n], bias=b)
                        ops.bn_stats(Y, sums=self.sums, n_rows=n, **bnk)
            halo_started = l < 11 and self.agg_first[l + 1]
            fused = None if self.overlap else getattr(comm, "halo_and_sums", None)
            if self.overlap:
                yield comm.start_all_reduce(self.sums[: 2 * L.cout[l]])
                if halo_started:
                    self._halo_ahead = self._start_halo(Y)
            elif halo_started and fused is not None and fused(Y, n, self.sums[: 2 * L.cout[l]]):
                yield None
            else:
                h_stats = comm.start_all_reduce(self.sums[: 2 * L.cout[l]])
                h_halo = comm.start_halo(Y, n) if halo_started else None
                yield _Both(h_stats, h_halo)
            if use_running:
                self._bn4_from_running(l, L.view(params, "bn%d.weight" % i), L.view(params, "bn%d.bias" % i))
            elif not tail:
                ops.bn_prepare(self.sums, self.n_total, L.view(params, "bn%d.weight" % i), L.view(params, "bn%d.bias" % i),
                               self.bn4[l], running=(self.running[l][0], self.running[l][1]) if update_running else None)
            X, pro = Y, (self.bn4[l][0], self.bn4[l][1])
        if update_running:
            self.num_batches_tracked += 1
        ops.head_fwd(self.Y[11], self.bn4[11], L.view(params, "linear1.weight"), L.view(params, "linear1.bias"),
                     L.view(params, "linear2.weight"), L.view(params, "linear2.bias"), self.kind, self.x_pos,
                     self.out, n_rows=n)
        self.result = self.out
        if self.inv is not None:
            torch.index_select(self.out, 0, self.inv, out=self.out_orig)
            self.result = self.out_orig

    def backward_steps(self, params: torch.Tensor, grads: torch.Tensor, dout: torch.Tensor):
        L, g, n, comm = self.layout, self.g, self.n_rows, self.comm
        free = list(range(len(self._flat)))

        def take(c):
            k = free.pop(0)
            return k, self._work(k, c)

        def release(k):
            free.append(k)

        def wgrad(l, fn, *bufs):
            fn()

        kz, dZ = take(32)
        if self.perm is not None:
            dout = dout.index_select(0, self.perm)
        tail = self._tail_fused

        def arm(l):
            if tail:
                return {"bn": ops.BnBwd(self.n_total, self.bn4[l], L.view(grads, "bn%d.weight" % (l + 1)),
                                        L.view(grads, "bn%d.bias" % (l + 1)), self.c10s[l])}
            return {}

        torch._foreach_zero_([L.view(grads, "conv%d.bias" % (l + 1)) for l in range(12)])
        ops.head_bwd(self.Y[11], self.bn4[11], L.view(params, "linear1.weight"), L.view(params, "linear1.bias"),
                     L.view(params, "linear2.weight"), L.view(params, "linear2.bias"), self.kind, dout.contiguous(), dZ,
                     L.view(grads, "linear1.weight"), L.view(grads, "linear1.bias"),
                     L.view(grads, "linear2.weight"), L.view(grads, "linear2.bias"), n_rows=n)
        have_sums = False
        fuse_red = hasattr(ops, "spmm_bnred") and (self.dtype == torch.float32
                                                   or not _unfused("bf16_spmm_red"))

        def spmm_to_dz(src, dst, l):
            if fuse_red and l > 0:
                ops.spmm_bnred(g, src, dst[:n], self.Y[l - 1], self.bn4[l - 1], self.sums, **arm(l - 1))
                return True
            ops.spmm(g, src, out=dst[:n])
            return False

        def spmm_to_dz_split(src, dst, l):
            red = fuse_red and l > 0
            if red:
                yield from self._agg(lambda gh, r0, r1, sums: ops.spmm_bnred(gh, src, dst[r0:r1], self.Y[l - 1][r0:r1],
                                                                            self.bn4[l - 1], sums), self._start_halo(src))
                self._add_sums(2 * L.cout[l - 1])
            else:
                yield from self._agg(lambda gh, r0, r1, _: ops.spmm(gh, src, out=dst[r0:r1]), self._start_halo(src))
            return red

        fuse_dgrad_red = (getattr(ops, "gemm_nn_bnred_supported", None) is not None
                          and not _unfused("dgrad_red"))

        def dgrad_to_dz(dH, W, dZ, l):
            if fuse_dgrad_red and ops.gemm_nn_bnred_supported(L.cout[l], L.cin_p[l], n, self.dtype):
                ops.gemm_nn_bnred(dH, W, self.Y[l - 1], self.bn4[l - 1], self.sums, out=dZ, n_rows=n, **self._wp(l, 1),
                                  **self._scales(l, 1), **arm(l - 1))
                return True
            ops.gemm_nn(dH, W, out=dZ, n_rows=n, **self._wp(l, 1), **self._scales(l, 1))
            return False

        for l in range(11, -1, -1):
            i = l + 1
            co, ci = L.cout[l], L.cin_p[l]
            W = L.view(params, "conv%d.lin.weight" % i, true_shape=False)
            dW = L.view(grads, "conv%d.lin.weight" % i, true_shape=False)
            Y, bn4, c10 = self.Y[l], self.bn4[l], self.c10s[l]
            if not have_sums:
                ops.bn_bwd_reduce(dZ, Y, bn4, sums2=self.sums, n_rows=n, **arm(l))
            have_sums = False
            yield comm.start_all_reduce(self.sums[: 2 * co])
            if not tail:
                ops.bn_bwd_prepare(self.sums, self.n_total, bn4, L.view(grads, "bn%d.weight" % i),
                                   L.view(grads, "bn%d.bias" % i), c10)
            if self.fuse_bnbwd[l]:
                kp, dP = take(ci)
                ops.gemm_nn_bnbwd(dZ, Y, W, bn4, c10, out=dP, n_rows=n, **self._wp(l, 1), **self._scales(l, 1))
                wgrad(l, lambda: ops.gemm_tn_bnbwd(dZ, Y, self.P[l], bn4, c10, out=dW, n_rows=n, **self._scales(l, 1, 0)), kz)
                release(kz)
                if self.overlap:
                    kz, dZ = take(ci)
                    have_sums = yield from spmm_to_dz_split(dP, dZ, l)
                else:
                    yield comm.start_halo(dP, n)
                    kz, dZ = take(ci)
                    have_sums = spmm_to_dz(dP, dZ, l)
                release(kp)
                continue
            if self.fuse_gather_bwd[l]:
                kh, dH = take(co)
                ops.spmm_bnbwd(g, dZ, Y, bn4, c10, dH[:n])
                release(kz)
                Xp, pro = self.Y[l - 1], (self.bn4[l - 1][0], self.bn4[l - 1][1])
                kz, dZ = take(ci)
                have_sums = dgrad_to_dz(dH, W, dZ, l)
                wgrad(l, lambda: ops.gemm_tn(dH, Xp, out=dW, pro=pro, n_rows=n, **self._scales(l, 1, 0)), kh)
                release(kh)
                continue
            if l == 0 and self.fuse_bnbwd0:
                wgrad(0, lambda: ops.gemm_tn_bnbwd(dZ, Y, self.P[0], bn4, c10, out=dW, n_rows=n, **self._scales(0, 1, 0)), kz)
                release(kz)
                continue
            ky, dY = take(co)
            ops.bn_bwd_apply(dZ, Y, bn4, c10, dY, None, n_rows=n)
            release(kz)
            if l > 0:
                Xp, pro = self.Y[l - 1], (self.bn4[l - 1][0], self.bn4[l - 1][1])
            else:
                Xp, pro = self.x0, None
            if self.agg_first[l]:
                if l > 0:
                    kp, dP = take(ci)
                    ops.gemm_nn(dY, W, out=dP, n_rows=n, **self._wp(l, 1), **self._scales(l, 1))
                wgrad(l, lambda: ops.gemm_tn(dY, self.P[l], out=dW, n_rows=n, **self._scales(l, 1, 0)), ky)
                if l > 0:
                    release(ky)
                    if self.overlap:
                        kz, dZ = take(ci)
                        have_sums = yield from spmm_to_dz_split(dP, dZ, l)
                    else:
                        yield comm.start_halo(dP, n)
                        kz, dZ = take(ci)
                        have_sums = spmm_to_dz(dP, dZ, l)
                    release(kp)
                else:
                    release(ky)
            else:
                if self.overlap:
                    h = self._start_halo(dY)
                    kh, dH = take(co)
                    yield from self._agg(lambda gh, r0, r1, _: ops.spmm(gh, dY, out=dH[r0:r1]), h)
                else:
                    yield comm.start_halo(dY, n)
                    kh, dH = take(co)
                    ops.spmm(g, dY, out=dH[:n])
                release(ky)
                if l > 0:
                    kz, dZ = take(ci)
                    have_sums = dgrad_to_dz(dH, W, dZ, l)
                wgrad(l, lambda: ops.gemm_tn(dH, Xp, out=dW, pro=pro, n_rows=n, **self._scales(l, 1, 0)), kh)
                release(kh)
        if self._f16:
            ops.gemm_scales_roll(self.scale_slots)
            self._prime = False
```

dual-dmp_amd/ops.py:

```python
from __future__ import annotations

import ctypes
import os
import threading
import weakref

import numpy as np
import torch

from . import _lib
from ._lib import DdmpError, check

SLOPE = 0.01
BN_EPS = 1e-5
BN_MOMENTUM = 0.1


_raw_stream = getattr(torch._C, "_cuda_getCurrentRawStream", None)


def _stream():
    if _raw_stream is not None:
        return ctypes.c_void_p(_raw_stream(torch.cuda.current_device()))
    return ctypes.c_void_p(torch.cuda.current_stream().cuda_stream)
# ... 1056 lines not shown
    wp = ws if wplanes is None else _wws(wplanes, L.ddmp_gemm_rows_workspace_bytes(K, M), a.device)[0]
    with _timed("gemm_nt", (K, M), 4.0 * n * (K + M) + 4.0 * K * M, 2.0 * n * K * M, survey=4.0 * n * (K + M)):
        o, keep = _mk_opts(bn, scales, wplanes is not None, want_bn=True, want_scales=True)
        st = L.ddmp_gemm_nt_stats_f32_o(_p(a), lda, _p(w), ldw, _p(out), ldy, n, K, M, _p(bias), _p(ps), _p(psh), slope,
                                        _p(sums), _p(wp), nb if wplanes is None else wp.numel(), ws.data_ptr() + nb,
                                        ws.numel() - nb, _stream(), o)
    check(st, "ddmp_gemm_nt_stats_f32")
    return out


def gemm_nn(a, w, out=None, n_rows=None, wplanes=None, scales=None):
    a, lda = _mat(a, "a")
    w, ldw = _mat(_chk(w, torch.float32, "w"), "w")
    n = a.shape[0] if n_rows is None else n_rows
    M, K = w.shape
    if a.shape[1] != M:
        raise DdmpError("gemm_nn: inner dimensions differ")
    if out is None:
        out = torch.empty((n, K), dtype=a.dtype, device=a.device)
    out, ldy = _mat(out, "out", a)
    L = _lib.lib()
    ws, prep = _wws(wplanes if a.dtype == torch.float32 else None, L.ddmp_gemm_rows_ws_bytes(K, M, _dt(a)), a.device)
    es = a.element_size()
    with _timed("gemm_nn", (M, K), es * n * (K + M) + 4.0 * K * M, 2.0 * n * K * M, survey=es * n * (K + M)):
        o, keep = _mk_opts(None, scales, prep, want_scales=True)
        st = L.ddmp_gemm_nn_o(_p(a), lda, _p(w), ldw, _p(out), ldy, n, M, K, _dt(a), _p(ws), ws.numel(), _stream(), o)
    check(st, "ddmp_gemm_nn")
    return out


def gemm_nn_bnred_supported(M, K, n_rows, dtype=torch.float32):
    return dtype == torch.float32 and bool(_lib.lib().ddmp_gemm_nn_bnred_supported(int(M), int(K), int(n_rows)))


def gemm_nn_bnred(a, w, yp, bn4, sums, out=None, slope=SLOPE, n_rows=None, wplanes=None, scales=None, bn=None):
    a, lda = _mat(a, "a")
    w, ldw = _mat(_chk(w, torch.float32, "w"), "w")
    yp, ldyp = _mat(yp, "yp", a)
    n = a.shape[0] if n_rows is None else n_rows
    M, K = w.shape
    if out is None:
        out = torch.empty((n, K), dtype=a.dtype, device=a.device)
    out, ldo = _mat(out, "out", a)
    L = _lib.lib()
    if a.dtype != torch.float32:
        raise DdmpError("gemm_nn_bnred: float32 features only")
    nb = (L.ddmp_gemm_rows_workspace_bytes(K, M) + 255) // 256 * 256
    sb = L.ddmp_gemm_nt_stats_workspace_bytes(n, K)
    ws = Workspace.get(nb + sb, a.device)
    wp = ws if wplanes is None else _wws(wplanes, L.ddmp_gemm_rows_workspace_bytes(K, M), a.device)[0]
    with _timed("gemm_nn", (M, K), 4.0 * n * (2 * K + M) + 4.0 * K * M, 2.0 * n * K * M, survey=4.0 * n * (K + M)):
        o, keep = _mk_opts(bn, scales, wplanes is not None, want_bn=True, want_scales=True)
        st = L.ddmp_gemm_nn_bnred_f32_o(_p(a), lda, _p(w), ldw, _p(out), ldo, n, M, K, _p(yp), ldyp, _p(bn4[0]), _p(bn4[1]),
                                        _p(bn4[2]), _p(bn4[3]), slope, _p(sums), _p(wp), nb if wplanes is None else wp.numel(),
                                        ws.data_ptr() + nb, ws.numel() - nb, _stream(), o)
    check(st, "ddmp_gemm_nn_bnred_f32")
    return out


def gemm_tn(g, z, out=None, pro=None, slope=SLOPE, n_rows=None, scales=None):
    g, ldg = _mat(g, "g")
    z, ldz = _mat(z, "z", g)
    n = g.shape[0] if n_rows is None else n_rows
    M, K = g.shape[1], z.shape[1]
    if out is None:
        out = torch.empty((M, K), dtype=torch.float32, device=g.device)
    out, ldo = _mat(_chk(out, torch.float32, "out"), "out")
    L = _lib.lib()
    need = L.ddmp_gemm_tn_ws_bytes(n, M, K, _dt(g))
    ws = Workspace.get(need, g.device)
    ps, psh = (None, None) if pro is None else pro
    es = g.element_size()
    with _timed("gemm_tn", (M, K), es * n * (K + M) + 4.0 * K * M, 2.0 * n * K * M, survey=es * n * (K + M)):
        o, keep = _mk_opts(None, scales, want_scales=True)
        st = L.ddmp_gemm_tn_o(_p(g), ldg, _p(z), ldz, _p(out), ldo, n, M, K, _dt(g), _p(ps), _p(psh), slope, _p(ws),
                              ws.numel(), _stream(), o)
    check(st, "ddmp_gemm_tn")
    return out


def gemm_bnbwd_supported(cout, cin, n_rows, dtype=torch.float32):
    if dtype == torch.bfloat16:
        return bool(_lib.lib().ddmp_gemm_fused_bf16_supported(int(cout), int(cin), int(n_rows)) & 2)
    if dtype != torch.float32:
        return False
    return bool(_lib.lib().ddmp_gemm_bnbwd_supported(int(cout), int(cin), int(n_rows)))


def gemm_tn_bnbwd_supported(cout, cin, n_rows, dtype=torch.float32):
    return dtype == torch.float32 and bool(_lib.lib().ddmp_gemm_tn_bnbwd_supported(int(cout), int(cin), int(n_rows)))


def rows_gather(src, idx, out=None, n_rows=None):
    src, lds = _mat(src, "src")
    n = idx.numel() if n_rows is None else n_rows
    if out is None:
        out = torch.empty((n, src.shape[1]), dtype=src.dtype, device=src.device)
    out, ldo = _mat(out, "out", src)
    check(_lib.lib().ddmp_rows_gather(_p(src), lds, _p(_chk(idx, torch.int64, "idx")), n, src.shape[1], _dt(src), _p(out), ldo, 0,
                                      _stream()), "ddmp_rows_gather")
    return out


def to_bf16(src, dst=None):
    src = _chk(src.contiguous(), torch.float32, "src")
    if dst is None:
        dst = torch.empty(src.shape, dtype=torch.bfloat16, device=src.device)
    check(_lib.lib().ddmp_f32_to_bf16(_p(src), _p(dst), src.numel(), _stream()), "ddmp_f32_to_bf16")
    return dst


def gemm_nn_bnbwd(dz, yb, w, bn4, c10, out=None, slope=SLOPE, n_rows=None, wplanes=None, scales=None):
    if dz.dtype == torch.bfloat16:
        dz, lddz = _mat(dz, "dz")
        yb, ldyb = _mat(yb, "yb", dz)
        w, ldw = _mat(_chk(w, torch.float32, "w"), "w")
        n = dz.shape[0] if n_rows is None else n_rows
        M, K = w.shape
        if out is None:
            out = torch.empty((n, K), dtype=dz.dtype, device=dz.device)
        out, ldo = _mat(out, "out", dz)
        L = _lib.lib()
        ws = Workspace.get(L.ddmp_gemm_rows_ws_bytes(K, M, _dt(dz)), dz.device)
        with _timed("gemm_nn", (M, K), 2.0 * n * (K + 2 * M) + 4.0 * K * M, 2.0 * n * K * M, survey=2.0 * n * (K + M)):
            st = L.ddmp_gemm_nn_bnbwd_bf16(_p(dz), lddz, _p(yb), ldyb, _p(w), ldw, _p(out), ldo, n, M, K, _p(bn4[0]), _p(bn4[1]),
                                           _p(c10[0]), _p(c10[1]), slope, _p(ws), ws.numel(), _stream())
        check(st, "ddmp_gemm_nn_bnbwd_bf16")
        return out
    dz, lddz = _mat(dz, "dz")
    yb, ldyb = _mat(yb, "yb")
    w, ldw = _mat(w, "w")
    n = dz.shape[0] if n_rows is None else n_rows
    M, K = w.shape
    if out is None:
        out = torch.empty((n, K), dtype=torch.float32, device=dz.device)
    out, ldo = _mat(out, "out")
    L = _lib.lib()
    ws, prep = _wws(wplanes, L.ddmp_gemm_rows_workspace_bytes(K, M), dz.device)
    with _timed("gemm_nn", (M, K), 4.0 * n * (K + 2 * M) + 4.0 * K * M, 2.0 * n * K * M, survey=4.0 * n * (K + M)):
        o, keep = _mk_opts(None, scales, prep, want_scales=True)
        st = L.ddmp_gemm_nn_bnbwd_f32_o(_p(dz), lddz, _p(yb), ldyb, _p(w), ldw, _p(out), ldo, n, M, K, _p(bn4[0]), _p(bn4[1]),
                                        _p(c10[0]), _p(c10[1]), slope, _p(ws), ws.numel(), _stream(), o)
    check(st, "ddmp_gemm_nn_bnbwd_f32")
    return out


def gemm_tn_bnbwd(dz, yb, z, bn4, c10, out=None, pro=None, slope=SLOPE, n_rows=None, scales=None):
    if dz.dtype == torch.bfloat16:
        dz, lddz = _mat(dz, "dz")
        yb, ldyb = _mat(yb, "yb", dz)
        z, ldz = _mat(z, "z", dz)
        n = dz.shape[0] if n_rows is None else n_rows
        M, K = yb.shape[1], z.shape[1]
        if out is None:
            out = torch.empty((M, K), dtype=torch.float32, device=dz.device)
        out, ldo = _mat(_chk(out, torch.float32, "out"), "out")
        L = _lib.lib()
        ws = Workspace.get(L.ddmp_gemm_tn_ws_bytes(n, M, K, _dt(dz)), dz.device)
        ps, psh = (None, None) if pro is None else pro
        with _timed("gemm_tn", (M, K), 2.0 * n * (K + 2 * M) + 4.0 * K * M, 2.0 * n * K * M, survey=2.0 * n * (K + M)):
            st = L.ddmp_gemm_tn_bnbwd_bf16(_p(dz), lddz, _p(yb), ldyb, _p(z), ldz, _p(out), ldo, n, M, K, _p(bn4[0]), _p(bn4[1]),
                                           _p(c10[0]), _p(c10[1]), _p(ps), _p(psh), slope, _p(ws), ws.numel(), _stream())
        check(st, "ddmp_gemm_tn_bnbwd_bf16")
        return out
    dz, lddz = _mat(dz, "dz")
    yb, ldyb = _mat(yb, "yb")
    z, ldz = _mat(z, "z")
    n = dz.shape[0] if n_rows is None else n_rows
    M, K = yb.shape[1], z.shape[1]
    if out is None:
        out = torch.empty((M, K), dtype=torch.float32, device=dz.device)
    out, ldo = _mat(out, "out")
    L = _lib.lib()
    ws = Workspace.get(L.ddmp_gemm_tn_workspace_bytes(n, M, K), dz.device)
    ps, psh = (None, None) if pro is None else pro
    with _timed("gemm_tn", (M, K), 4.0 * n * (K + 2 * M) + 4.0 * K * M, 2.0 * n * K * M, survey=4.0 * n * (K + M)):
        o, keep = _mk_opts(None, scales, want_scales=True)
        st = L.ddmp_gemm_tn_bnbwd_f32_o(_p(dz), lddz, _p(yb), ldyb, _p(z), ldz, _p(out), ldo, n, M, K, _p(bn4[0]), _p(bn4[1]),
                                        _p(c10[0]), _p(c10[1]), _p(ps), _p(psh), slope, _p(ws), ws.numel(), _stream(), o)
    check(st, "ddmp_gemm_tn_bnbwd_f32")
    return out


def _colws(n, C, device):
    need = _lib.lib().ddmp_colreduce_workspace_bytes(n, C)
    if need == 0:
        raise DdmpError("column reduction: unsupported width %d (power of two in [8,1024])" % C)
    return Workspace.get(need, device)


def bn_stats(y, sums=None, n_rows=None, bn=None):
    y, ldy = _mat(y, "y")
    n = y.shape[0] if n_rows is None else n_rows
    C = y.shape[1]
    if sums is None:
        sums = torch.empty(2 * C, dtype=torch.float64, device=y.device)
    ws = _colws(n, C, y.device)
    with _timed("bn_stats", C, float(y.element_size()) * n * C):
        o, keep = _mk_opts(bn, want_bn=True)
        st = _lib.lib().ddmp_bn_stats_o(_p(y), ldy, n, C, _dt(y), _p(sums), _p(ws), ws.numel(), _stream(), o)
    check(st, "ddmp_bn_stats")
    return sums


def bn_prepare(sums, n_total, gamma, beta, out4, running=None, eps=BN_EPS, momentum=BN_MOMENTUM):
    C = gamma.numel()
    rm, rv = (None, None) if running is None else running
    st = _lib.lib().ddmp_bn_prepare_f32(_p(sums), float(n_total), C, _p(gamma), _p(beta), eps, momentum,
                                        _p(out4[0]), _p(out4[1]), _p(out4[2]), _p(out4[3]), _p(rm), _p(rv), _stream())
    check(st, "ddmp_bn_prepare_f32")
    return out4


def bn_lrelu_apply(y, scale, shift, out=None, slope=SLOPE):
    y, ldy = _mat(y, "y")
    if out is None:
        out = torch.empty_like(y)
    out, ldz = _mat(out, "out", y)
    fn = _lib.lib().ddmp_bn_lrelu_apply_bf16 if y.dtype == torch.bfloat16 else _lib.lib().ddmp_bn_lrelu_apply_f32
    st = fn(_p(y), ldy, _p(out), ldz, y.shape[0], y.shape[1], _p(scale), _p(shift), slope, _stream())
    check(st, "ddmp_bn_lrelu_apply")
    return out


def bn_bwd_reduce(dz, y, bn4, sums2=None, slope=SLOPE, n_rows=None, bn=None):
    dz, lddz = _mat(dz, "dz")
    y, ldy = _mat(y, "y", dz)
    n = y.shape[0] if n_rows is None else n_rows
    C = y.shape[1]
    if sums2 is None:
        sums2 = torch.empty(2 * C, dtype=torch.float64, device=y.device)
    ws = _colws(n, C, y.device)
    with _timed("bn_bwd_reduce", C, 2.0 * y.element_size() * n * C):
        o, keep = _mk_opts(bn, want_bn=True)
        st = _lib.lib().ddmp_bn_bwd_reduce_o(_p(dz), lddz, _p(y), ldy, n, C, _dt(y), _p(bn4[0]), _p(bn4[1]), _p(bn4[2]),
                                             _p(bn4[3]), slope, _p(sums2), _p(ws), ws.numel(), _stream(), o)
    check(st, "ddmp_bn_bwd_reduce")
    return sums2


def bn_bwd_prepare(sums2, n_total, bn4, dgamma, dbeta, c10):
    C = dgamma.numel()
    st = _lib.lib().ddmp_bn_bwd_prepare_f32(_p(sums2), float(n_total), C, _p(bn4[0]), _p(bn4[2]), _p(bn4[3]),
                                            _p(dgamma), _p(dbeta), _p(c10[0]), _p(c10[1]), _stream())
    check(st, "ddmp_bn_bwd_prepare_f32")


def bn_bwd_apply(dz, y, bn4, c10, dy, dbias_sums, slope=SLOPE, n_rows=None):
    dz, lddz = _mat(dz, "dz")
    y, ldy = _mat(y, "y", dz)
    dy, lddy = _mat(dy, "dy", dz)
    n = y.shape[0] if n_rows is None else n_rows
    C = y.shape[1]
    ws = _colws(n, C, y.device)
    with _timed("bn_bwd_apply", C, 3.0 * y.element_size() * n * C):
        st = _lib.lib().ddmp_bn_bwd_apply(_p(dz), lddz, _p(y), ldy, _p(dy), lddy, n, C, _dt(y), _p(bn4[0]), _p(bn4[1]),
                                          _p(c10[0]), _p(c10[1]), slope, _p(dbias_sums), _p(ws), ws.numel(),
                                          _stream())
    check(st, "ddmp_bn_bwd_apply")
    return dy


def colsum(x, sums=None, n_rows=None):
    x, ldx = _mat(x, "x")
    n = x.shape[0] if n_rows is None else n_rows
    C = x.shape[1]
    if sums is None:
        sums = torch.empty(C, dtype=torch.float64, device=x.device)
    ws = _colws(n, C, x.device)
    st = _lib.lib().ddmp_colsum_f32(_p(x), ldx, n, C, _p(sums), _p(ws), ws.numel(), _stream())
    check(st, "ddmp_colsum_f32")
    return sums


def f64_to_f32(src, dst):
    st = _lib.lib().ddmp_f64_to_f32(_p(src), _p(dst), src.numel(), _stream())
    check(st, "ddmp_f64_to_f32")
    return dst


def head_fwd(y, bn4, W1, b1, W2, b2, kind, x_pos, out, slope=SLOPE, n_rows=None):
    y, ldy = _mat(y, "y")
    n = y.shape[0] if n_rows is None else n_rows
    with _timed("head_fwd", kind, n * (32.0 * y.element_size() + 12 + (12 if kind == 0 else 0))):
        st = _lib.lib().ddmp_head_fwd(_p(y), ldy, n, _dt(y), _p(bn4[0]), _p(bn4[1]), slope, _p(W1), _p(b1), _p(W2),
                                      _p(b2), kind, _p(x_pos), _p(out), _stream())
    check(st, "ddmp_head_fwd")
    return out


def head_bwd(y, bn4, W1, b1, W2, b2, kind, dout, dz, dW1, db1, dW2, db2, slope=SLOPE, n_rows=None):
    y, ldy = _mat(y, "y")
    dz, lddz = _mat(dz, "dz", y)
    n = y.shape[0] if n_rows is None else n_rows
    L = _lib.lib()
    ws = Workspace.get(L.ddmp_head_bwd_workspace_bytes(n), y.device)
    with _timed("head_bwd", kind, n * (64.0 * y.element_size() + 12)):
        st = L.ddmp_head_bwd(_p(y), ldy, n, _dt(y), _p(bn4[0]), _p(bn4[1]), slope, _p(W1), _p(b1), _p(W2), _p(b2), kind,
                             _p(dout), _p(dz), lddz, _p(dW1), _p(db1), _p(dW2), _p(db2), _p(ws), ws.numel(),
                             _stream())
    check(st, "ddmp_head_bwd")


def grad_sumsq(g, out=None):
    L = _lib.lib()
    if out is None:
        out = torch.empty(1, dtype=torch.float64, device=g.device)
    ws = Workspace.get(L.ddmp_sumsq_workspace_bytes(), g.device)
    with _timed("optimizer", "sumsq", 4.0 * g.numel()):
        st = L.ddmp_grad_sumsq_f32(_p(g), g.numel(), _p(out), _p(ws), ws.numel(), _stream())
    check(st, "ddmp_grad_sumsq_f32")
    return out


def grad_clip_(g, sumsq, max_norm):
    st = _lib.lib().ddmp_grad_clip_f32(_p(g), g.numel(), _p(sumsq), float(max_norm), _stream())
    check(st, "ddmp_grad_clip_f32")


def adam_step_(p, g, m, v, lr, step, betas=(0.9, 0.999), eps=1e-8, clip_sumsq=None, max_norm=0.0):
    with _timed("optimizer", "adam", 28.0 * p.numel()):
        st = _lib.lib().ddmp_adam_step_f32(_p(p), _p(g), _p(m), _p(v), p.numel(), float(lr), betas[0], betas[1], eps,
                                           int(step), _p(clip_sumsq), float(max_norm), _stream())
    check(st, "ddmp_adam_step_f32")


def adam_prepare(counter, lr, coef, betas=(0.9, 0.999)):
    check(_lib.lib().ddmp_adam_prepare(_p(counter), float(lr), betas[0], betas[1], _p(coef), _stream()), "ddmp_adam_prepare")


def adam_step_dev_(p, g, m, v, coef, betas=(0.9, 0.999), eps=1e-8, clip_sumsq=None, max_norm=0.0):
    with _timed("optimizer", "adam", 28.0 * p.numel()):
        st = _lib.lib().ddmp_adam_step_dev_f32(_p(p), _p(g), _p(m), _p(v), p.numel(), betas[0], betas[1], eps, _p(coef),
                                               _p(clip_sumsq), float(max_norm), _stream())
    check(st, "ddmp_adam_step_dev_f32")
```

include/ddmp_hip.h:

```cpp
#ifndef DDMP_HIP_H
#define DDMP_HIP_H

#include <stddef.h>
#include <stdint.h>

#ifdef __cplusplus
extern "C" {
#endif
#if defined(__GNUC__)
#pragma GCC visibility push(default)
#endif

#define DDMP_OK 0
#define DDMP_EINVAL (-1)
#define DDMP_ERANGE (-2)
#define DDMP_ENOMEM (-3)
#define DDMP_EWORKSPACE (-4)

#define DDMP_ABI_VERSION 3

typedef struct ddmp_graph ddmp_graph;
typedef void* ddmp_stream;

int ddmp_abi_version(void);
// ... 71 lines not shown
int ddmp_feast_fwd_f32(const ddmp_graph* g, const float* Hf, int64_t ldh, const float* P, int64_t ldp, int heads, int C,
                       const float* c, const float* bias , float* beta, float* Y, int64_t ldy, ddmp_stream stream);
int ddmp_feast_bwd_edge_f32(const ddmp_graph* g, const float* dOut, int64_t lddo, const float* Hf, int64_t ldh, int heads, int C,
                            const float* beta, float* dz, float* rs, ddmp_stream stream);
int ddmp_feast_bwd_node_f32(const ddmp_graph* g, const float* dOut, int64_t lddo, int heads, int C, const float* beta,
                            const float* dz, const float* rs, float* dHf, int64_t lddh, float* dP, int64_t lddp,
                            ddmp_stream stream);
size_t ddmp_feast_dc_workspace_bytes(int64_t n_rows, int heads);
int ddmp_feast_dc_f32(const float* rs, int64_t n_rows, int heads, float* dc, void* workspace, size_t workspace_bytes,
                      ddmp_stream stream);

int ddmp_gmm_fwd_f32(const ddmp_graph* g, const float* Hf, int64_t ldh, const float* attr, int dim, const float* mu,
                     const float* sigma, int K, int C, const float* R , int64_t ldr, const float* bias ,
                     float* w, float* Y, int64_t ldy, ddmp_stream stream);
int ddmp_gmm_bwd_edge_f32(const ddmp_graph* g, const float* dOut, int64_t lddo, const float* Hf, int64_t ldh, const float* attr,
                          int dim, const float* mu, const float* sigma, int K, int C, float* ge, float* parts,
                          float* dattr , ddmp_stream stream);
int ddmp_gmm_bwd_node_f32(const ddmp_graph* g, const float* dOut, int64_t lddo, int K, int C, const float* w, float* dHf,
                          int64_t lddh, float* dR , int64_t lddr, ddmp_stream stream);

int ddmp_gather_max_f32(const ddmp_graph* g, const float* B, int64_t ldb, const float* A , int64_t lda, int C, float* Y,
                        int64_t ldy, int32_t* arg , int64_t ldarg, ddmp_stream stream);
int ddmp_gather_max_bwd_f32(const ddmp_graph* g, const float* dG, int64_t lddg, const int32_t* arg, int64_t ldarg, int C, float* dA,
                            int64_t ldda, float* dB, int64_t lddb, ddmp_stream stream);

size_t ddmp_gemm_rows_workspace_bytes(int K, int M);
int ddmp_gemm_nt_f32(const float* A, int64_t lda, const float* W, int64_t ldw, float* Y, int64_t ldy,
                     int64_t n_rows, int K, int M, const float* bias,
                     const float* pro_scale, const float* pro_shift, float slope,
                     void* workspace , size_t workspace_bytes, ddmp_stream stream);
size_t ddmp_gemm_tn_workspace_bytes(int64_t n_rows, int M, int K);
int ddmp_set_gemm_mode(int mode);
int ddmp_get_gemm_mode(void);
int ddmp_gemm_scales_roll(float* slots, int n_slots, ddmp_stream stream);

size_t ddmp_colreduce_workspace_bytes(int64_t n_rows, int C);
int ddmp_bn_stats_f32(const float* Y, int64_t ldy, int64_t n_rows, int C, double* sums ,
                      void* workspace, size_t workspace_bytes, ddmp_stream stream);
int ddmp_bn_prepare_f32(const double* sums , double n_total, int C, const float* gamma,
                        const float* beta, float eps, float momentum, float* scale, float* shift,
                        float* mean, float* rstd, float* running_mean ,
                        float* running_var , ddmp_stream stream);
int ddmp_bn_lrelu_apply_f32(const float* Y, int64_t ldy, float* Z, int64_t ldz, int64_t n_rows, int C,
                            const float* scale, const float* shift, float slope, ddmp_stream stream);
int ddmp_bn_bwd_prepare_f32(const double* sums2, double n_total, int C, const float* scale, const float* mean,
                            const float* rstd, float* dgamma, float* dbeta, float* c1, float* c0,
                            ddmp_stream stream);
int ddmp_next_pending(void);
int ddmp_colsum_f32(const float* X, int64_t ldx, int64_t n_rows, int C, double* sums , void* workspace,
                    size_t workspace_bytes, ddmp_stream stream);
int ddmp_f64_to_f32(const double* in, float* out, int64_t n, ddmp_stream stream);

size_t ddmp_head_bwd_workspace_bytes(int64_t n_rows);

size_t ddmp_loss_partials_bytes(void);
int ddmp_loss_vertex_fwd(int64_t V, const float* pos, const double* real_pos, const int32_t* vv_ptr,
                         const int32_t* vv_idx, float* resid , double* partials, ddmp_stream stream);
int ddmp_loss_face_fwd(int64_t F, const float* pos, const float* norm, const double* real_norm,
                       const int32_t* faces, float* fc , float* fa , float* pn_coef ,
                       float* pn_dn , double* partials, ddmp_stream stream);
int ddmp_loss_bnf_fwd(int64_t F, const float* norm, const int32_t* f2f, const float* fc, const float* fa,
                      int loop, float* fcd , float* bnf_n , float* bnf_A ,
                      double* partials, ddmp_stream stream);
int ddmp_loss_finalize(const double* partials, int64_t V, int64_t F, const double* k_host , double gate4,
                       double* lossbuf , ddmp_stream stream);
int ddmp_loss_bnf_bwd(int64_t F, const int32_t* f2f, const float* fa, const float* fcd, int loop,
                      const float* bnf_n, const float* bnf_A, const double* partials, const double* coef,
                      float* G0 , float* scratch , ddmp_stream stream);
int ddmp_loss_face_bwd(int64_t F, const float* norm, const double* real_norm, const float* pn_dn,
                       const float* G0 , const float* n_last , const double* coef,
                       float* dnorm , ddmp_stream stream);
int ddmp_loss_vertex_bwd(int64_t V, const float* pos, const double* real_pos, const float* resid,
                         const int32_t* vv_ptr, const int32_t* vv_idx, const int32_t* vf_ptr,
                         const int32_t* vf_corner, const float* pn_coef, const float* norm, const double* coef,
                         float* dpos , ddmp_stream stream);

int ddmp_loss_vertex_fwd_part(int64_t V, const float* pos, const double* real_pos, const int32_t* vv_ptr,
                              const int32_t* vv_idx, float* resid, double* partials, const uint8_t* own, ddmp_stream stream);
int ddmp_loss_face_fwd_part(int64_t F, const float* pos, const float* norm, const double* real_norm, const int32_t* faces,
                            float* fc, float* fa, float* pn_coef, float* pn_dn, double* partials, const uint8_t* own,
                            ddmp_stream stream);
int ddmp_loss_bnf_sigma(int64_t F, const float* norm, const int32_t* f2f, const float* fc, float* fcd, float* bnf_n,
                        double* partials, const uint8_t* own, ddmp_stream stream);
int ddmp_loss_bnf_filter(int64_t F, int64_t F_glob, const int32_t* f2f, const float* fcd, const float* fa, int loop,
                         float* bnf_n, float* bnf_A, double* partials, const uint8_t* own, ddmp_stream stream);
int ddmp_loss_bnf_bwd_part(int64_t F, int64_t F_glob, const int32_t* f2f, const float* fa, const float* fcd, int loop,
                           const float* bnf_n, const float* bnf_A, const double* partials, const double* coef, float* G0,
                           float* scratch, ddmp_stream stream);

size_t ddmp_sumsq_workspace_bytes(void);
int ddmp_grad_sumsq_f32(const float* g, int64_t n, double* out , void* workspace, size_t workspace_bytes,
                        ddmp_stream stream);
int ddmp_grad_clip_f32(float* g, int64_t n, const double* sumsq, float max_norm, ddmp_stream stream);
int ddmp_adam_step_f32(float* p, const float* g, float* m, float* v, int64_t n, float lr, float beta1,
                       float beta2, float eps, int step, const double* clip_sumsq , float max_norm,
                       ddmp_stream stream);
int ddmp_spmm_stats_supported(int C);
int ddmp_spmm_stats_f32(const ddmp_graph* g, const float* X, int64_t ldx, float* Y, int64_t ldy, int C,
                        const float* bias , const float* pro_scale ,
                        const float* pro_shift , float slope, const float* ref ,
                        double* sums2 , void* workspace, size_t workspace_bytes, ddmp_stream stream);
int ddmp_spmm_stats(const ddmp_graph* g, const void* X, int64_t ldx, void* Y, int64_t ldy, int C, int dtype,
                    const float* bias, const float* pro_scale, const float* pro_shift, float slope, const float* ref,
                    double* sums2, void* workspace, size_t workspace_bytes, ddmp_stream stream);
int ddmp_spmm_bnbwd_supported(int C);
int ddmp_spmm_bnbwd_f32(const ddmp_graph* g, const float* dZ, int64_t lddz, const float* Yb, int64_t ldyb,
                        float* out, int64_t ld_out, int C, const float* a, const float* b, const float* c1,
                        const float* c0, float slope, ddmp_stream stream);


size_t ddmp_gemm_nt_stats_workspace_bytes(int64_t n_rows, int M);
int ddmp_gemm_nt_stats_f32(const float* A, int64_t lda, const float* W, int64_t ldw, float* Y, int64_t ldy,
                           int64_t n_rows, int K, int M, const float* bias ,
                           const float* pro_scale , const float* pro_shift , float slope,
                           double* sums2 , void* workspace, size_t workspace_bytes, void* stats_ws,
                           size_t stats_ws_bytes, ddmp_stream stream);

int ddmp_gemm_prepare_weights(int n, const float* const* W, const int64_t* ldw, const int* M, const int* K, const int* form,
                              const int* has_pro , void* const* planes, const size_t* planes_bytes,
                              int64_t n_rows, float* scratch, ddmp_stream stream);
int ddmp_gemm_forget_planes(const void* planes);
int ddmp_gemm_tn_bnbwd_supported(int cout, int cin, int64_t n_rows);
int ddmp_gemm_nn_bnred_supported(int M, int K, int64_t n_rows);
int ddmp_gemm_nn_bnred_f32(const float* A, int64_t lda, const float* W, int64_t ldw, float* out, int64_t ld_out,
                           int64_t n_rows, int M, int K, const float* Yp, int64_t ldyp, const float* scale,
                           const float* shift, const float* mean, const float* rstd, float slope, double* sums2,
                           void* workspace, size_t workspace_bytes, void* stats_ws, size_t stats_ws_bytes,
                           ddmp_stream stream);
int ddmp_gemm_bnbwd_supported(int cout, int cin, int64_t n_rows);
int ddmp_gemm_nn_bnbwd_f32(const float* dZ, int64_t lddz, const float* Yb, int64_t ldyb, const float* W, int64_t ldw,
                           float* out, int64_t ld_out, int64_t n_rows, int M, int K, const float* a, const float* b,
                           const float* c1, const float* c0, float slope, void* workspace, size_t workspace_bytes,
                           ddmp_stream stream);
int ddmp_gemm_tn_bnbwd_f32(const float* dZ, int64_t lddz, const float* Yb, int64_t ldyb, const float* Z, int64_t ldz,
                           float* dW, int64_t lddw, int64_t n_rows, int M, int K, const float* a, const float* b,
                           const float* c1, const float* c0, const float* pro_scale ,
                           const float* pro_shift , float slope, void* workspace, size_t workspace_bytes,
                           ddmp_stream stream);

int ddmp_adam_prepare(int32_t* step_counter, float lr, float beta1, float beta2, float* coef ,
                      ddmp_stream stream);
int ddmp_adam_step_dev_f32(float* p, const float* g, float* m, float* v, int64_t n, float beta1, float beta2,
                           float eps, const float* coef , const double* clip_sumsq ,
                           float max_norm, ddmp_stream stream);

int ddmp_face_normals_f32(int64_t F, const float* pos, const int32_t* faces, float* fn ,
                          float* fa , ddmp_stream stream);
int ddmp_vertex_update_f32(int64_t V, int64_t F, float* pos, const float* norm, const int32_t* faces,
                           const int32_t* vf_ptr, const int32_t* vf_corner, float* fc_scratch, int loop,
                           ddmp_stream stream);
size_t ddmp_mad_workspace_bytes(void);
int ddmp_mad_f64(int64_t F, const float* n1 , const double* n2 , double* out ,
                 void* workspace, size_t workspace_bytes, ddmp_stream stream);

size_t ddmp_surfdist_grid_bytes(int64_t F, int64_t max_refs);
int ddmp_surfdist_build(int64_t V, int64_t F, const float* pos , const int32_t* faces , void* grid,
                        size_t grid_bytes, int64_t* refs_needed_host , ddmp_stream stream);
size_t ddmp_surfdist_query_workspace_bytes(int64_t Q, int64_t F);
int ddmp_surfdist_query(int64_t F, const void* grid, size_t grid_bytes, int64_t Q, const float* points ,
                        float max_dist, int sort_queries, float* dist , double* stats ,
                        void* workspace, size_t workspace_bytes, ddmp_stream stream);

#define DDMP_F32 0
#define DDMP_BF16 1

int ddmp_gemm_fused_bf16_supported(int cout, int cin, int64_t n_rows);
size_t ddmp_gemm_nt_stats_bf16_workspace_bytes(int64_t n_rows, int M);
int ddmp_gemm_nt_stats_bf16(const uint16_t* A, int64_t lda, const float* W, int64_t ldw, uint16_t* Y, int64_t ldy,
                            int64_t n_rows, int K, int M, const float* bias, const float* pro_scale,
                            const float* pro_shift, float slope, double* sums2, void* workspace, size_t workspace_bytes,
                            void* stats_ws, size_t stats_ws_bytes, ddmp_stream stream);
int ddmp_gemm_nn_bnbwd_bf16(const uint16_t* dZ, int64_t lddz, const uint16_t* Yb, int64_t ldyb, const float* W,
                            int64_t ldw, uint16_t* out, int64_t ld_out, int64_t n_rows, int M, int K, const float* a,
                            const float* b, const float* c1, const float* c0, float slope, void* workspace,
                            size_t workspace_bytes, ddmp_stream stream);
int ddmp_gemm_tn_bnbwd_bf16(const uint16_t* dZ, int64_t lddz, const uint16_t* Yb, int64_t ldyb, const uint16_t* Z,
                            int64_t ldz, float* dW, int64_t lddw, int64_t n_rows, int M, int K, const float* a,
                            const float* b, const float* c1, const float* c0, const float* pro_scale,
                            const float* pro_shift, float slope, void* workspace, size_t workspace_bytes,
                            ddmp_stream stream);
int ddmp_bn_stats_bf16(const uint16_t* Y, int64_t ldy, int64_t n_rows, int C, double* sums , void* workspace,
                       size_t workspace_bytes, ddmp_stream stream);
int ddmp_bn_lrelu_apply_bf16(const uint16_t* Y, int64_t ldy, uint16_t* Z, int64_t ldz, int64_t n_rows, int C,
                             const float* scale, const float* shift, float slope, ddmp_stream stream);
int ddmp_bn_bwd_reduce_bf16(const uint16_t* dZ, int64_t lddz, const uint16_t* Y, int64_t ldy, int64_t n_rows, int C,
                            const float* scale, const float* shift, const float* mean, const float* rstd, float slope,
                            double* sums2 , void* workspace, size_t workspace_bytes, ddmp_stream stream);
int ddmp_bn_bwd_apply_bf16(const uint16_t* dZ, int64_t lddz, const uint16_t* Y, int64_t ldy, uint16_t* dY, int64_t lddy,
                           int64_t n_rows, int C, const float* scale, const float* shift, const float* c1,
                           const float* c0, float slope, double* dbias_sums , void* workspace,
                           size_t workspace_bytes, ddmp_stream stream);
int ddmp_rows_gather(const void* src, int64_t ld_src, const int64_t* idx, int64_t n, int C, int dtype, void* dst,
                     int64_t ld_dst, int scatter, ddmp_stream stream);
typedef struct ddmp_comm ddmp_comm;
typedef struct ddmp_halo_plan ddmp_halo_plan;
int ddmp_comm_unique_id(char* id128_host);
int ddmp_comm_create(int rank, int world, const char* id128_host, ddmp_comm** out);
int ddmp_comm_destroy(ddmp_comm* comm);
int ddmp_halo_plan_create(int world, int rank, int64_t n_rows, int64_t n_cols, const int64_t* send_idx_host,
                          const int64_t* send_counts_host, const int64_t* recv_counts_host, ddmp_halo_plan** out);
int ddmp_halo_plan_destroy(ddmp_halo_plan* plan);
size_t ddmp_halo_pack_bytes(const ddmp_halo_plan* plan, int C, int dtype);
int ddmp_halo_exchange(ddmp_comm* comm, const ddmp_halo_plan* plan, void* T, int64_t ld, int C, int dtype, void* pack_ws,
                       size_t ws_bytes, double* sums , int n_sums, ddmp_stream stream);
int ddmp_comm_allreduce_sum(ddmp_comm* comm, void* buf, int64_t n, int is_f64, ddmp_stream stream);
int ddmp_comm_allgather(ddmp_comm* comm, const void* send, void* recv, int64_t bytes_per_rank, ddmp_stream stream);
int ddmp_trace_marker(ddmp_stream stream);
int ddmp_build_ablation_flags(void);
int ddmp_copy_probe(const void* src, void* dst, int64_t bytes, int mode, ddmp_stream stream);
int ddmp_copy_probe_rows(const void* src, void* dst, int64_t n_rows, int row_bytes, ddmp_stream stream);
int ddmp_f32_to_bf16(const float* in, uint16_t* out, int64_t n, ddmp_stream stream);

int ddmp_spmm(const ddmp_graph* g, const void* X, int64_t ldx, void* Y, int64_t ldy, int C, int dtype, const float* bias,
              const float* pro_scale, const float* pro_shift, float slope, ddmp_stream stream);
size_t ddmp_spmm_bnred_ws_bytes(int64_t n_rows, int C, int dtype);
int ddmp_spmm_bnred(const ddmp_graph* g, const void* X, int64_t ldx, void* Y, int64_t ldy, int C, int dtype,
                    const void* Yp, int64_t ldyp, const float* scale, const float* shift, const float* mean,
                    const float* rstd, float slope, double* sums2, void* workspace, size_t workspace_bytes,
                    ddmp_stream stream);
int ddmp_spmm_bnbwd(const ddmp_graph* g, const void* dZ, int64_t lddz, const void* Yb, int64_t ldyb, void* out,
                    int64_t ld_out, int C, int dtype, const float* a, const float* b, const float* c1, const float* c0,
                    float slope, ddmp_stream stream);
size_t ddmp_gemm_rows_ws_bytes(int K, int M, int dtype);
int ddmp_gemm_nt(const void* A, int64_t lda, const float* W, int64_t ldw, void* Y, int64_t ldy, int64_t n_rows, int K,
                 int M, int dtype, const float* bias, const float* pro_scale, const float* pro_shift, float slope,
                 void* workspace, size_t workspace_bytes, ddmp_stream stream);
int ddmp_gemm_nn(const void* A, int64_t lda, const float* W, int64_t ldw, void* Y, int64_t ldy, int64_t n_rows, int M,
                 int K, int dtype, void* workspace, size_t workspace_bytes, ddmp_stream stream);
size_t ddmp_gemm_tn_ws_bytes(int64_t n_rows, int M, int K, int dtype);
int ddmp_gemm_tn(const void* G, int64_t ldg, const void* Z, int64_t ldz, float* dW, int64_t lddw, int64_t n_rows, int M,
                 int K, int dtype, const float* pro_scale, const float* pro_shift, float slope, void* workspace,
                 size_t workspace_bytes, ddmp_stream stream);
int ddmp_bn_stats(const void* Y, int64_t ldy, int64_t n_rows, int C, int dtype, double* sums, void* workspace,
                  size_t workspace_bytes, ddmp_stream stream);
int ddmp_bn_bwd_reduce(const void* dZ, int64_t lddz, const void* Y, int64_t ldy, int64_t n_rows, int C, int dtype,
                       const float* scale, const float* shift, const float* mean, const float* rstd, float slope,
                       double* sums2, void* workspace, size_t workspace_bytes, ddmp_stream stream);
int ddmp_bn_bwd_apply(const void* dZ, int64_t lddz, const void* Y, int64_t ldy, void* dY, int64_t lddy, int64_t n_rows,
                      int C, int dtype, const float* scale, const float* shift, const float* c1, const float* c0,
                      float slope, double* dbias_sums, void* workspace, size_t workspace_bytes, ddmp_stream stream);
int ddmp_head_fwd(const void* Y, int64_t ldy, int64_t n_rows, int dtype, const float* scale, const float* shift,
                  float slope, const float* W1, const float* b1, const float* W2, const float* b2, int kind,
                  const float* x_pos, float* out, ddmp_stream stream);
int ddmp_head_bwd(const void* Y, int64_t ldy, int64_t n_rows, int dtype, const float* scale, const float* shift,
                  float slope, const float* W1, const float* b1, const float* W2, const float* b2, int kind,
                  const float* dout, void* dZ, int64_t lddz, float* dW1, float* db1, float* dW2, float* db2,
                  void* workspace, size_t workspace_bytes, ddmp_stream stream);


#define DDMP_OPT_BN_FWD 1u
#define DDMP_OPT_BN_BWD 2u
#define DDMP_OPT_SCALES 4u
#define DDMP_OPT_PREPARED 8u
typedef struct ddmp_opts {
    uint32_t struct_size;
    uint32_t flags;
    double bn_n_total;
    int32_t bn_C;
    float bn_eps, bn_momentum;
    int32_t prime;
    const float* bn_in[3];
    float* bn_out[6];
    float* slot_a;
    float* slot_b;
} ddmp_opts;
int ddmp_bn_stats_o(const void* Y, int64_t ldy, int64_t n_rows, int C, int dtype, double* sums, void* workspace,
    size_t workspace_bytes, ddmp_stream stream, const ddmp_opts* opts);
int ddmp_bn_bwd_reduce_o(const void* dZ, int64_t lddz, const void* Y, int64_t ldy, int64_t n_rows, int C, int dtype,
    const float* scale, const float* shift, const float* mean, const float* rstd, float slope, double* sums2,
    void* workspace, size_t workspace_bytes, ddmp_stream stream, const ddmp_opts* opts);
int ddmp_spmm_stats_o(const ddmp_graph* g, const void* X, int64_t ldx, void* Y, int64_t ldy, int C, int dtype,
    const float* bias, const float* pro_scale, const float* pro_shift, float slope, const float* ref, double* sums2,
    void* workspace, size_t workspace_bytes, ddmp_stream stream, const ddmp_opts* opts);
int ddmp_spmm_bnred_o(const ddmp_graph* g, const void* X, int64_t ldx, void* Y, int64_t ldy, int C, int dtype,
    const void* Yp, int64_t ldyp, const float* scale, const float* shift, const float* mean, const float* rstd,
    float slope, double* sums2, void* workspace, size_t workspace_bytes, ddmp_stream stream, const ddmp_opts* opts);
int ddmp_gemm_nt_o(const void* A, int64_t lda, const float* W, int64_t ldw, void* Y, int64_t ldy, int64_t n_rows,
    int K, int M, int dtype, const float* bias, const float* pro_scale, const float* pro_shift, float slope,
    void* workspace, size_t workspace_bytes, ddmp_stream stream, const ddmp_opts* opts);
int ddmp_gemm_nn_o(const void* A, int64_t lda, const float* W, int64_t ldw, void* Y, int64_t ldy, int64_t n_rows,
    int M, int K, int dtype, void* workspace, size_t workspace_bytes, ddmp_stream stream, const ddmp_opts* opts);
int ddmp_gemm_tn_o(const void* G, int64_t ldg, const void* Z, int64_t ldz, float* dW, int64_t lddw, int64_t n_rows,
    int M, int K, int dtype, const float* pro_scale, const float* pro_shift, float slope, void* workspace,
    size_t workspace_bytes, ddmp_stream stream, const ddmp_opts* opts);
int ddmp_gemm_nt_stats_f32_o(const float* A, int64_t lda, const float* W, int64_t ldw, float* Y, int64_t ldy,
    int64_t n_rows, int K, int M, const float* bias , const float* pro_scale , const float* pro_shift , float slope,
    double* sums2 , void* workspace, size_t workspace_bytes, void* stats_ws, size_t stats_ws_bytes, ddmp_stream stream,
    const ddmp_opts* opts);
int ddmp_gemm_nt_stats_bf16_o(const uint16_t* A, int64_t lda, const float* W, int64_t ldw, uint16_t* Y, int64_t ldy,
    int64_t n_rows, int K, int M, const float* bias, const float* pro_scale, const float* pro_shift, float slope,
    double* sums2, void* workspace, size_t workspace_bytes, void* stats_ws, size_t stats_ws_bytes, ddmp_stream stream,
    const ddmp_opts* opts);
int ddmp_gemm_nn_bnred_f32_o(const float* A, int64_t lda, const float* W, int64_t ldw, float* out, int64_t ld_out,
    int64_t n_rows, int M, int K, const float* Yp, int64_t ldyp, const float* scale, const float* shift,
    const float* mean, const float* rstd, float slope, double* sums2, void* workspace, size_t workspace_bytes,
    void* stats_ws, size_t stats_ws_bytes, ddmp_stream stream, const ddmp_opts* opts);
int ddmp_gemm_nn_bnbwd_f32_o(const float* dZ, int64_t lddz, const float* Yb, int64_t ldyb, const float* W, int64_t ldw,
    float* out, int64_t ld_out, int64_t n_rows, int M, int K, const float* a, const float* b, const float* c1,
    const float* c0, float slope, void* workspace, size_t workspace_bytes, ddmp_stream stream, const ddmp_opts* opts);
int ddmp_gemm_tn_bnbwd_f32_o(const float* dZ, int64_t lddz, const float* Yb, int64_t ldyb, const float* Z, int64_t ldz,
    float* dW, int64_t lddw, int64_t n_rows, int M, int K, const float* a, const float* b, const float* c1,
    const float* c0, const float* pro_scale , const float* pro_shift , float slope, void* workspace,
    size_t workspace_bytes, ddmp_stream stream, const ddmp_opts* opts);

#if defined(__GNUC__)
#pragma GCC visibility pop
#endif
#ifdef __cplusplus
}
#endif
#endif
```

Before: 22.55 iters/s.

## Add specialized first-layer conv kernels and fuse BN reduction into head backward

Adds dedicated kernels for the first conv layer (K=8/16, M=32): a forward GEMM that also accumulates BN statistics, and a weight-gradient kernel that applies the BN/LeakyReLU backward in-register, both replacing the general GEMM paths. It also rewrites the head backward kernel so it emits the BN backward reduction sums for the last layer, which removes a separate reduction pass over Y[11]. The aim is to cut launches and memory traffic for narrow layers that the tiled GEMM handles poorly. The cost is extra code paths, plus a small-K register GEMM that may underuse hardware if row counts are low.

Result: no change. 22.74 iters/s, median of 6 (+0.9%).

```diff
diff --git a/dual-dmp_amd/csrc/conv1.hip b/dual-dmp_amd/csrc/conv1.hip
--- /dev/null
+++ b/dual-dmp_amd/csrc/conv1.hip
@@ -0,0 +1,194 @@
+#include "ddmp_common.h"
+#include "finalize.h"
+
+#include <algorithm>
+
+namespace {
+
+using namespace ddmp;
+
+#include "fpartials.inc"
+
+constexpr int kM = 32;
+constexpr int kRowsPerStep = 32;
+constexpr int kUnroll = 4;
+constexpr int kMaxGroups = kFpSingleGroups;
+
+template <int KQ>
+__global__ __launch_bounds__(256) void conv1_fwd_stats_kernel(const float* __restrict__ P, int64_t ldp,
+                                                              const float* __restrict__ W, int64_t ldw,
+                                                              const float* __restrict__ bias, float* __restrict__ Y,
+                                                              int64_t ldy, int n_rows, double* __restrict__ part) {
+    constexpr int K = 4 * KQ;
+    __shared__ double sm[256 * 8];
+    const int tid = threadIdx.x, cq = tid & 7, rl = tid >> 3;
+    float w[4][K], bv[4];
+#pragma unroll
+    for (int j = 0; j < 4; ++j) {
+#pragma unroll
+        for (int k = 0; k < K; ++k) w[j][k] = W[(int64_t)(cq * 4 + j) * ldw + k];
+        bv[j] = bias ? bias[cq * 4 + j] : 0.f;
+    }
+    double s0[4] = {0.0, 0.0, 0.0, 0.0}, s1[4] = {0.0, 0.0, 0.0, 0.0};
+    const int64_t step = (int64_t)gridDim.x * kRowsPerStep * kUnroll;
+    for (int64_t base = (int64_t)blockIdx.x * kRowsPerStep * kUnroll; base < n_rows; base += step) {
+        float p[kUnroll][K];
+#pragma unroll
+        for (int u = 0; u < kUnroll; ++u) {
+            const int64_t r = base + u * kRowsPerStep + rl;
+#pragma unroll
+            for (int q = 0; q < KQ; ++q) {
+                const float4 v = r < n_rows ? *reinterpret_cast<const float4*>(P + r * ldp + 4 * q) : make_float4(0.f, 0.f, 0.f, 0.f);
+                p[u][4 * q] = v.x; p[u][4 * q + 1] = v.y; p[u][4 * q + 2] = v.z; p[u][4 * q + 3] = v.w;
+            }
+        }
+#pragma unroll
+        for (int u = 0; u < kUnroll; ++u) {
+            const int64_t r = base + u * kRowsPerStep + rl;
+            if (r >= n_rows) continue;
+            float y[4];
+#pragma unroll
+            for (int j = 0; j < 4; ++j) {
+                float acc = 0.f;
+#pragma unroll
+                for (int k = 0; k < K; ++k) acc = fmaf(p[u][k], w[j][k], acc);
+                y[j] = acc + bv[j];
+                const double yd = y[j];
+                s0[j] += yd;
+                s1[j] = fma(yd, yd, s1[j]);
+            }
+            *reinterpret_cast<float4*>(Y + r * ldy + cq * 4) = make_float4(y[0], y[1], y[2], y[3]);
+        }
+    }
+#pragma unroll
+    for (int j = 0; j < 4; ++j) {
+        sm[tid * 8 + j] = s0[j];
+        sm[tid * 8 + 4 + j] = s1[j];
+    }
+    __syncthreads();
+    if (tid < 2 * kM) {
+        const int v = tid >> 5, c = tid & 31;
+        double t = 0.0;
+        for (int r = 0; r < kRowsPerStep; ++r) t += sm[(r * 8 + (c >> 2)) * 8 + v * 4 + (c & 3)];
+        part[(int64_t)blockIdx.x * 2 * kM + tid] = t;
+    }
+}
+
+template <int KQ>
+__global__ __launch_bounds__(256) void conv1_wgrad_kernel(const float* __restrict__ dZ, int64_t lddz,
+                                                          const float* __restrict__ Yb, int64_t ldyb,
+                                                          const float* __restrict__ P, int64_t ldp, int n_rows,
+                                                          const float* __restrict__ a, const float* __restrict__ b,
+                                                          const float* __restrict__ c1, const float* __restrict__ c0,
+                                                          float slope, float* __restrict__ part) {
+    constexpr int K = 4 * KQ, kRow = 2 * K + 1;
+    __shared__ float sm[256 * kRow];
+    const int tid = threadIdx.x, cq = tid & 7, rl = tid >> 3;
+    float av[4], bv[4], k1[4], k0[4], acc[4][K];
+#pragma unroll
+    for (int j = 0; j < 4; ++j) {
+        av[j] = a[cq * 4 + j]; bv[j] = b[cq * 4 + j]; k1[j] = c1[cq * 4 + j]; k0[j] = c0[cq * 4 + j];
+#pragma unroll
+        for (int k = 0; k < K; ++k) acc[j][k] = 0.f;
+    }
+    constexpr int U = 2;
+    const int64_t step = (int64_t)gridDim.x * kRowsPerStep * U;
+    for (int64_t base = (int64_t)blockIdx.x * kRowsPerStep * U; base < n_rows; base += step) {
+        float dz[U][4], y[U][4], p[U][K];
+#pragma unroll
+        for (int u = 0; u < U; ++u) {
+            const int64_t r = base + u * kRowsPerStep + rl;
+            const bool on = r < n_rows;
+            const float4 d4 = on ? *reinterpret_cast<const float4*>(dZ + r * lddz + cq * 4) : make_float4(0.f, 0.f, 0.f, 0.f);
+            const float4 y4 = on ? *reinterpret_cast<const float4*>(Yb + r * ldyb + cq * 4) : make_float4(0.f, 0.f, 0.f, 0.f);
+            dz[u][0] = d4.x; dz[u][1] = d4.y; dz[u][2] = d4.z; dz[u][3] = d4.w;
+            y[u][0] = y4.x; y[u][1] = y4.y; y[u][2] = y4.z; y[u][3] = y4.w;
+#pragma unroll
+            for (int q = 0; q < KQ; ++q) {
+                const float4 v = on ? *reinterpret_cast<const float4*>(P + r * ldp + 4 * q) : make_float4(0.f, 0.f, 0.f, 0.f);
+                p[u][4 * q] = v.x; p[u][4 * q + 1] = v.y; p[u][4 * q + 2] = v.z; p[u][4 * q + 3] = v.w;
+            }
+        }
+#pragma unroll
+        for (int u = 0; u < U; ++u) {
+#pragma unroll
+            for (int j = 0; j < 4; ++j) {
+                const float dy = fmaf(av[j], dz[u][j] * lrelu_grad(fmaf(y[u][j], av[j], bv[j]), slope), fmaf(k1[j], y[u][j], k0[j]));
+#pragma unroll
+                for (int k = 0; k < K; ++k) acc[j][k] = fmaf(dy, p[u][k], acc[j][k]);
+            }
+        }
+    }
+    float* out = part + (int64_t)blockIdx.x * kM * K;
+#pragma unroll
+    for (int h = 0; h < 2; ++h) {
+        __syncthreads();
+#pragma unroll
+        for (int j = 0; j < 2; ++j)
+#pragma unroll
+            for (int k = 0; k < K; ++k) sm[tid * kRow + j * K + k] = acc[2 * h + j][k];
+        __syncthreads();
+        if (tid < 16 * K) {
+            const int cqo = tid / (2 * K), rem = tid % (2 * K);
+            float t = 0.f;
+            for (int r = 0; r < kRowsPerStep; ++r) t += sm[(r * 8 + cqo) * kRow + rem];
+            out[(cqo * 4 + 2 * h + rem / K) * K + rem % K] = t;
+        }
+    }
+}
+
+int conv1_groups(int64_t n_rows) {
+    return (int)std::max<int64_t>(1, std::min<int64_t>(kMaxGroups, cdiv(n_rows, kRowsPerStep * kUnroll)));
+}
+
+}
+
+size_t ddmp_conv1_fwd_stats_ws_bytes(int64_t n_rows) {
+    return (size_t)conv1_groups(n_rows) * 2 * kM * sizeof(double) + fpartials_mid_bytes(kM);
+}
+
+bool ddmp_conv1_fwd_stats_ok(const float* A, int64_t lda, const float* W, int64_t ldw, const float* Y, int64_t ldy,
+                             int64_t n_rows, int K, int M) {
+    return A && W && Y && n_rows > 0 && n_rows < INT32_MAX && M == kM && (K == 8 || K == 16) && lda >= K && ldw >= K &&
+           ldy >= M && lda % 4 == 0 && ldy % 4 == 0 && (uintptr_t)A % 16 == 0 && (uintptr_t)Y % 16 == 0 && !unfused("l0");
+}
+
+int ddmp_conv1_fwd_stats_f32(const float* A, int64_t lda, const float* W, int64_t ldw, float* Y, int64_t ldy, int64_t n_rows,
+                             int K, const float* bias, double* sums2, void* stats_ws, size_t stats_ws_bytes, ddmp_stream stream,
+                             ddmp::CallCtx& ctx) {
+    ARG_TRY(sums2 && stats_ws && ddmp_conv1_fwd_stats_ok(A, lda, W, ldw, Y, ldy, n_rows, K, kM));
+    if (stats_ws_bytes < ddmp_conv1_fwd_stats_ws_bytes(n_rows)) return DDMP_EWORKSPACE;
+    const int groups = conv1_groups(n_rows);
+    double* part = (double*)stats_ws;
+    hipStream_t st = (hipStream_t)stream;
+    if (K == 8)
+        hipLaunchKernelGGL(conv1_fwd_stats_kernel<2>, dim3(groups), dim3(256), 0, st, A, lda, W, ldw, bias, Y, ldy, (int)n_rows, part);
+    else
+        hipLaunchKernelGGL(conv1_fwd_stats_kernel<4>, dim3(groups), dim3(256), 0, st, A, lda, W, ldw, bias, Y, ldy, (int)n_rows, part);
+    LAUNCH_TRY();
+    fpartials_reduce<double>(part, groups, kM, kM, part + (size_t)groups * 2 * kM, sums2, st, ctx.take_fin(kM));
+    LAUNCH_TRY();
+    return DDMP_OK;
+}
+
+bool ddmp_conv1_wgrad_ok(const float* dZ, int64_t lddz, const float* Yb, int64_t ldyb, const float* Z, int64_t ldz, int64_t n_rows,
+                         int M, int K) {
+    return dZ && Yb && Z && n_rows > 0 && n_rows < INT32_MAX && M == kM && (K == 8 || K == 16) && lddz >= M && ldyb >= M &&
+           ldz >= K && lddz % 4 == 0 && ldyb % 4 == 0 && ldz % 4 == 0 && (uintptr_t)dZ % 16 == 0 && (uintptr_t)Yb % 16 == 0 &&
+           (uintptr_t)Z % 16 == 0 && !unfused("l0");
+}
+
+int ddmp_conv1_wgrad_splits(int64_t n_rows) { return conv1_groups(n_rows); }
+
+int ddmp_conv1_wgrad_partials(const float* dZ, int64_t lddz, const float* Yb, int64_t ldyb, const float* Z, int64_t ldz,
+                              int64_t n_rows, int K, const float* a, const float* b, const float* c1, const float* c0, float slope,
+                              float* part, size_t part_bytes, ddmp_stream stream) {
+    const int splits = conv1_groups(n_rows);
+    if (!part || part_bytes < (size_t)splits * kM * K * sizeof(float)) return DDMP_EWORKSPACE;
+    hipStream_t st = (hipStream_t)stream;
+    if (K == 8)
+        hipLaunchKernelGGL(conv1_wgrad_kernel<2>, dim3(splits), dim3(256), 0, st, dZ, lddz, Yb, ldyb, Z, ldz, (int)n_rows, a, b, c1, c0, slope, part);
+    else
+        hipLaunchKernelGGL(conv1_wgrad_kernel<4>, dim3(splits), dim3(256), 0, st, dZ, lddz, Yb, ldyb, Z, ldz, (int)n_rows, a, b, c1, c0, slope, part);
+    return hipGetLastError() == hipSuccess ? splits : DDMP_EINVAL;
+}
diff --git a/dual-dmp_amd/csrc/ddmp_internal.h b/dual-dmp_amd/csrc/ddmp_internal.h
--- a/dual-dmp_amd/csrc/ddmp_internal.h
+++ b/dual-dmp_amd/csrc/ddmp_internal.h
@@ -61,6 +61,23 @@
 int ddmp_bn_bwd_reduce_bf16(const uint16_t* dZ, int64_t lddz, const uint16_t* Y, int64_t ldy, int64_t n_rows, int C,
                             const float* scale, const float* shift, const float* mean, const float* rstd, float slope,
                             double* sums2, void* workspace, size_t workspace_bytes, ddmp_stream stream, ddmp::CallCtx& ctx);
+bool ddmp_conv1_fwd_stats_ok(const float* A, int64_t lda, const float* W, int64_t ldw, const float* Y, int64_t ldy, int64_t n_rows,
+                             int K, int M);
+size_t ddmp_conv1_fwd_stats_ws_bytes(int64_t n_rows);
+int ddmp_conv1_fwd_stats_f32(const float* A, int64_t lda, const float* W, int64_t ldw, float* Y, int64_t ldy, int64_t n_rows,
+                             int K, const float* bias, double* sums2, void* stats_ws, size_t stats_ws_bytes, ddmp_stream stream,
+                             ddmp::CallCtx& ctx);
+bool ddmp_conv1_wgrad_ok(const float* dZ, int64_t lddz, const float* Yb, int64_t ldyb, const float* Z, int64_t ldz, int64_t n_rows,
+                         int M, int K);
+int ddmp_conv1_wgrad_splits(int64_t n_rows);
+int ddmp_conv1_wgrad_partials(const float* dZ, int64_t lddz, const float* Yb, int64_t ldyb, const float* Z, int64_t ldz,
+                              int64_t n_rows, int K, const float* a, const float* b, const float* c1, const float* c0, float slope,
+                              float* part, size_t part_bytes, ddmp_stream stream);
+int ddmp_head_bwd(const void* Y, int64_t ldy, int64_t n_rows, int dtype, const float* scale, const float* shift, float slope,
+                  const float* W1, const float* b1, const float* W2, const float* b2, int kind, const float* dout, void* dZ,
+                  int64_t lddz, float* dW1, float* db1, float* dW2, float* db2, const float* mean, const float* rstd,
+                  double* sums2 , void* workspace, size_t workspace_bytes, ddmp_stream stream,
+                  ddmp::CallCtx& ctx);
 int ddmp_spmm_stats(const ddmp_graph* g, const void* X, int64_t ldx, void* Y, int64_t ldy, int C, int dtype, const float* bias,
                     const float* pro_scale, const float* pro_shift, float slope, const float* ref, double* sums2, void* workspace,
                     size_t workspace_bytes, ddmp_stream stream, ddmp::CallCtx& ctx);
diff --git a/dual-dmp_amd/csrc/gemm.hip b/dual-dmp_amd/csrc/gemm.hip
--- a/dual-dmp_amd/csrc/gemm.hip
+++ b/dual-dmp_amd/csrc/gemm.hip
@@ -918,7 +918,8 @@
 extern "C" size_t ddmp_gemm_tn_workspace_bytes(int64_t n_rows, int M, int K) {
     if (n_rows <= 0 || M <= 0 || K <= 0) return 0;
     const TnPlan p = tn_plan(n_rows, M, K), q = tn_plan(n_rows, M, K, true);
-    return (size_t)std::max(p.n_splits, q.n_splits) * (size_t)M * (size_t)K * sizeof(float) + 64;
+    const int first = M == 32 && K <= 16 ? ddmp_conv1_wgrad_splits(n_rows) : 0;
+    return (size_t)std::max(std::max(p.n_splits, q.n_splits), first) * (size_t)M * (size_t)K * sizeof(float) + 64;
 }
 
 int ddmp_gemm_tn_f32(const float* G, int64_t ldg, const float* Z, int64_t ldz, float* dW, int64_t lddw, int64_t n_rows, int M,
@@ -1082,8 +1083,17 @@
     ARG_TRY(dZ && Yb && Z && dW && a && b && c1 && c0 && n_rows > 0 && n_rows < INT32_MAX && M > 0 && K > 0);
     ARG_TRY(M % 4 == 0 && K % 4 == 0 && lddz >= M && ldyb >= M && ldz >= K && lddw >= K);
     ARG_TRY((pro_scale == nullptr) == (pro_shift == nullptr));
+    hipStream_t st = (hipStream_t)stream;
+    if (!pro_scale && ddmp_conv1_wgrad_ok(dZ, lddz, Yb, ldyb, Z, ldz, n_rows, M, K)) {
+        const int splits = ddmp_conv1_wgrad_partials(dZ, lddz, Yb, ldyb, Z, ldz, n_rows, K, a, b, c1, c0, slope, (float*)workspace,
+                                                     workspace_bytes, stream);
+        if (splits < 0) return splits;
+        hipLaunchKernelGGL(reduce_splits_kernel, dim3((unsigned)cdiv((int64_t)M * K, 256)), dim3(256), 0, st, (const float*)workspace,
+                           (int64_t)M * K, splits, dW, lddw, M, K);
+        LAUNCH_TRY();
+        return DDMP_OK;
+    }
     if (!ddmp_gemm_tn_bnbwd_supported(M, K, n_rows)) return DDMP_EINVAL;
-    hipStream_t st = (hipStream_t)stream;
     const bool f16_route = gemm_mode() == 6 && gemm_f16() && lddz % 4 == 0 && ldyb % 4 == 0 && ldz % 4 == 0 && aligned16(dZ) &&
                            aligned16(Yb) && aligned16(Z);
     TnPlan p = tn_plan(n_rows, M, K, f16_route);
@@ -1176,6 +1186,9 @@
                            ddmp::CallCtx& ctx) {
     ARG_TRY(sums2 && stats_ws);
     if (stats_ws_bytes < ddmp_gemm_nt_stats_workspace_bytes(n_rows, M)) return DDMP_EWORKSPACE;
+    if (!pro_scale && !pro_shift && ddmp_conv1_fwd_stats_ok(A, lda, W, ldw, Y, ldy, n_rows, K, M) &&
+        stats_ws_bytes >= ddmp_conv1_fwd_stats_ws_bytes(n_rows))
+        return ddmp_conv1_fwd_stats_f32(A, lda, W, ldw, Y, ldy, n_rows, K, bias, sums2, stats_ws, stats_ws_bytes, stream, ctx);
     const bool fused = A && W && Y && n_rows > 0 && n_rows < INT32_MAX && K > 0 && M > 0 && K % 4 == 0 && lda % 4 == 0 &&
                        ldw % 4 == 0 && lda >= K && ldw >= K && ldy >= M && aligned16(A) && aligned16(W) &&
                        (pro_scale == nullptr) == (pro_shift == nullptr) && gemm_mode() != 0 && !(pro_scale && K > 512) &&
diff --git a/dual-dmp_amd/csrc/head.hip b/dual-dmp_amd/csrc/head.hip
--- a/dual-dmp_amd/csrc/head.hip
+++ b/dual-dmp_amd/csrc/head.hip
@@ -1,4 +1,5 @@
 #include "b16_common.h"
+#include "finalize.h"
 
 #include <algorithm>
 
@@ -8,72 +9,158 @@
 
 constexpr int H0 = 32, H1 = 16, H2 = 3;
 constexpr int kNPar = H1 * H0 + H1 + H2 * H1 + H2;
+constexpr int kNSmall = kNPar - H1 * H0;
+constexpr int kRec = 580;
+constexpr int kTile = 64;
+constexpr int kZs = H0 + 4, kDs = H1 + 4;
+constexpr int kMaxBlocks = 2048;
+constexpr int kSmallStride = 35;
+
+typedef float f32x4 __attribute__((ext_vector_type(4)));
 
 struct HeadW {
     const float *W1, *b1, *W2, *b2;
 };
-
-__device__ __forceinline__ void load_row32(const float* __restrict__ yrow, float (&y)[H0]) {
-#pragma unroll
-    for (int q = 0; q < H0 / 4; ++q) {
-        const float4 v = *reinterpret_cast<const float4*>(yrow + q * 4);
-        y[q * 4 + 0] = v.x; y[q * 4 + 1] = v.y; y[q * 4 + 2] = v.z; y[q * 4 + 3] = v.w;
-    }
-}
-__device__ __forceinline__ void load_row32(const bf16_t* __restrict__ yrow, float (&y)[H0]) {
-#pragma unroll
-    for (int q = 0; q < H0 / 8; ++q) {
-        float t[8];
-        bf_unpack8(ld8b(yrow + q * 8), t);
-#pragma unroll
-        for (int e = 0; e < 8; ++e) y[q * 8 + e] = t[e];
-    }
-}
-__device__ __forceinline__ void store_quad(float* p, const float (&d)[4]) {
-    *reinterpret_cast<float4*>(p) = make_float4(d[0], d[1], d[2], d[3]);
-}
-__device__ __forceinline__ void store_quad(bf16_t* p, const float (&d)[4]) {
-    *reinterpret_cast<uint2*>(p) = make_uint2(bf_pack(d[0], d[1]), bf_pack(d[2], d[3]));
+typedef const __attribute__((address_space(4))) float* cptr;
+__device__ __forceinline__ cptr at_use(cptr p) {
+    asm volatile("" : "+s"(p));
+    return p;
+}
+struct HeadWc {
+    cptr W1, b1, W2, b2;
+    __device__ explicit HeadWc(const HeadW& w) : W1((cptr)w.W1), b1((cptr)w.b1), W2((cptr)w.W2), b2((cptr)w.b2) {}
+};
+
+template <typename T> struct Piece;
+template <> struct Piece<float> {
+    static constexpr int VW = 4;
+    static __device__ __forceinline__ void ld(const float* p, float (&v)[4]) {
+        const float4 t = *reinterpret_cast<const float4*>(p);
+        v[0] = t.x; v[1] = t.y; v[2] = t.z; v[3] = t.w;
+    }
+    static __device__ __forceinline__ void st(float* p, float (&v)[4]) {
+        *reinterpret_cast<float4*>(p) = make_float4(v[0], v[1], v[2], v[3]);
+    }
+};
+template <> struct Piece<bf16_t> {
+    static constexpr int VW = 8;
+    static __device__ __forceinline__ void ld(const bf16_t* p, float (&v)[8]) { bf_unpack8(ld8b(p), v); }
+    static __device__ __forceinline__ void st(bf16_t* p, float (&v)[8]) {
+        const uint4 o = bf_pack8(v);
+        st8b(p, o);
+        bf_unpack8(o, v);
+    }
+};
+
+template <int VW> __device__ __forceinline__ void ld_coef(const float* __restrict__ p, float (&v)[VW]) {
+#pragma unroll
+    for (int k = 0; k < VW; ++k) v[k] = p[k];
+}
+template <int VW> __device__ __forceinline__ void lds_st(float* p, const float (&v)[VW]) {
+#pragma unroll
+    for (int q = 0; q < VW / 4; ++q)
+        *reinterpret_cast<float4*>(p + 4 * q) = make_float4(v[4 * q], v[4 * q + 1], v[4 * q + 2], v[4 * q + 3]);
+}
+template <int VW> __device__ __forceinline__ void lds_ld(const float* p, float (&v)[VW]) {
+#pragma unroll
+    for (int q = 0; q < VW / 4; ++q) {
+        const float4 t = *reinterpret_cast<const float4*>(p + 4 * q);
+        v[4 * q] = t.x; v[4 * q + 1] = t.y; v[4 * q + 2] = t.z; v[4 * q + 3] = t.w;
+    }
 }
 
 template <typename T>
-__device__ __forceinline__ void head_forward_row(const T* __restrict__ yrow, const float* __restrict__ scale,
-                                                 const float* __restrict__ shift, float slope, const HeadW& w,
-                                                 float (&z)[H0], float (&tp)[H1], float (&u)[H2]) {
-    load_row32(yrow, z);
-#pragma unroll
-    for (int j = 0; j < H0; ++j) z[j] = lrelu(fmaf(z[j], scale[j], shift[j]), slope);
+__device__ __forceinline__ void stage_rows(const T* __restrict__ Y, int64_t ldy, int row0, int n_rows,
+                                           const float (&a)[Piece<T>::VW], const float (&b)[Piece<T>::VW], float slope,
+                                           float* zs, float* ys ) {
+    constexpr int VW = Piece<T>::VW, CPR = H0 / VW, RPI = kTile / CPR;
+    const int lane = threadIdx.x, ch = lane % CPR, rl = lane / CPR;
+    float yr[CPR][VW];
+#pragma unroll
+    for (int q = 0; q < CPR; ++q) {
+        const int r = row0 + q * RPI + rl;
+        if (r < n_rows) {
+            Piece<T>::ld(Y + (int64_t)r * ldy + ch * VW, yr[q]);
+        } else {
+#pragma unroll
+            for (int k = 0; k < VW; ++k) yr[q][k] = 0.f;
+        }
+    }
+#pragma unroll
+    for (int q = 0; q < CPR; ++q) {
+        float z[VW];
+#pragma unroll
+        for (int k = 0; k < VW; ++k) z[k] = lrelu(fmaf(yr[q][k], a[k], b[k]), slope);
+        lds_st<VW>(zs + (q * RPI + rl) * kZs + ch * VW, z);
+        if (ys) lds_st<VW>(ys + (q * RPI + rl) * kZs + ch * VW, yr[q]);
+    }
+}
+
+__device__ __forceinline__ void stage3_in(const float* __restrict__ src, int row0, int n_rows, float* xs) {
+    const int64_t base = (int64_t)row0 * 3, end = (int64_t)n_rows * 3;
+#pragma unroll
+    for (int k = 0; k < 3; ++k) {
+        const int f = threadIdx.x + 64 * k;
+        xs[f] = base + f < end ? src[base + f] : 0.f;
+    }
+}
+__device__ __forceinline__ void stage3_out(float* __restrict__ dst, int row0, int n_rows, const float* xs) {
+    const int64_t base = (int64_t)row0 * 3, end = (int64_t)n_rows * 3;
+#pragma unroll
+    for (int k = 0; k < 3; ++k) {
+        const int f = threadIdx.x + 64 * k;
+        if (base + f < end) dst[base + f] = xs[f];
+    }
+}
+
+__device__ __forceinline__ void head_mlp(const float* zrow, float slope, const HeadWc& w, float (&z)[H0], float (&tp)[H1],
+                                         float (&u)[H2]) {
+    lds_ld<H0>(zrow, z);
+    const cptr W1 = at_use(w.W1), b1 = at_use(w.b1), W2 = at_use(w.W2), b2 = at_use(w.b2);
 #pragma unroll
     for (int i = 0; i < H1; ++i) {
-        float s = w.b1[i];
-#pragma unroll
-        for (int j = 0; j < H0; ++j) s = fmaf(w.W1[i * H0 + j], z[j], s);
+        float s = b1[i];
+#pragma unroll
+        for (int j = 0; j < H0; ++j) s = fmaf(W1[i * H0 + j], z[j], s);
         tp[i] = s;
     }
 #pragma unroll
     for (int o = 0; o < H2; ++o) {
-        float s = w.b2[o];
-#pragma unroll
-        for (int i = 0; i < H1; ++i) s = fmaf(w.W2[o * H1 + i], lrelu(tp[i], slope), s);
+        float s = b2[o];
+#pragma unroll
+        for (int i = 0; i < H1; ++i) s = fmaf(W2[o * H1 + i], lrelu(tp[i], slope), s);
         u[o] = s;
     }
 }
 
 template <typename T>
-__global__ __launch_bounds__(256) void head_fwd_kernel(const T* __restrict__ Y, int64_t ldy, int n_rows,
-                                                       const float* __restrict__ scale,
-                                                       const float* __restrict__ shift, float slope, HeadW w,
-                                                       int kind, const float* __restrict__ x_pos,
-                                                       float* __restrict__ out) {
-    for (int row = blockIdx.x * 256 + threadIdx.x; row < n_rows; row += gridDim.x * 256) {
+__global__ __launch_bounds__(kTile) void head_fwd_kernel(const T* __restrict__ Y, int64_t ldy, int n_rows,
+                                                         const float* __restrict__ scale,
+                                                         const float* __restrict__ shift, float slope, HeadW wg,
+                                                         int kind, const float* __restrict__ x_pos,
+                                                         float* __restrict__ out) {
+    const HeadWc w(wg);
+    constexpr int VW = Piece<T>::VW, CPR = H0 / VW;
+    __shared__ __attribute__((aligned(16))) float zs[kTile * kZs];
+    __shared__ float xs[kTile * 3];
+    const int lane = threadIdx.x;
+    float a[VW], b[VW];
+    ld_coef<VW>(scale + (lane % CPR) * VW, a);
+    ld_coef<VW>(shift + (lane % CPR) * VW, b);
+    const int n_tiles = (n_rows + kTile - 1) / kTile;
+    for (int tile = blockIdx.x; tile < n_tiles; tile += gridDim.x) {
+        const int row0 = tile * kTile;
+        __syncthreads();
+        stage_rows<T>(Y, ldy, row0, n_rows, a, b, slope, zs, nullptr);
+        if (kind == 0) stage3_in(x_pos, row0, n_rows, xs);
+        __syncthreads();
         float z[H0], tp[H1], u[H2];
-        head_forward_row(Y + (int64_t)row * ldy, scale, shift, slope, w, z, tp, u);
-        float* o = out + (int64_t)row * 3;
+        head_mlp(zs + lane * kZs, slope, w, z, tp, u);
+        float* o = xs + lane * 3;
         if (kind == 0) {
-            const float* xp = x_pos + (int64_t)row * 3;
-            o[0] = xp[0] + u[0];
-            o[1] = xp[1] + u[1];
-            o[2] = xp[2] + u[2];
+            o[0] += u[0];
+            o[1] += u[1];
+            o[2] += u[2];
         } else {
             const float v0 = tanhf(u[0]), v1 = tanhf(u[1]), v2 = tanhf(u[2]);
             const float r = sqrtf(v0 * v0 + v1 * v1 + v2 * v2);
@@ -82,32 +169,56 @@
             o[1] = v1 * s;
             o[2] = v2 * s;
         }
-    }
-}
-
-template <typename T>
-__global__ __launch_bounds__(256) void head_bwd_kernel(const T* __restrict__ Y, int64_t ldy, int n_rows,
-                                                       const float* __restrict__ scale,
-                                                       const float* __restrict__ shift, float slope, HeadW w,
-                                                       int kind, const float* __restrict__ dout,
-                                                       T* __restrict__ dZ, int64_t lddz,
-                                                       float* __restrict__ partial ) {
-    __shared__ float zs[256][H0 + 1];
-    __shared__ float dtps[256][H1 + 1];
-    __shared__ float ts[256][H1 + 1];
-    __shared__ float dus[256][4];
-    const int tid = threadIdx.x;
-    const int w1_j = tid & 31, w1_i = tid >> 5;
-    float accA = 0.f, accB = 0.f;
-    float accC = 0.f;
-
-    const int n_tiles = (n_rows + 255) / 256;
+        __syncthreads();
+        stage3_out(out, row0, n_rows, xs);
+    }
+}
+
+template <typename T, bool RED>
+__global__ __launch_bounds__(kTile) void head_bwd_kernel(const T* __restrict__ Y, int64_t ldy, int n_rows,
+                                                         const float* __restrict__ scale,
+                                                         const float* __restrict__ shift, float slope, HeadW wg,
+                                                         int kind, const float* __restrict__ dout,
+                                                         T* __restrict__ dZ, int64_t lddz,
+                                                         const float* __restrict__ mean, const float* __restrict__ rstd,
+                                                         float* __restrict__ partial, double* __restrict__ partial2) {
+    const HeadWc w(wg);
+    constexpr int VW = Piece<T>::VW, CPR = H0 / VW, RPI = kTile / CPR;
+    __shared__ __attribute__((aligned(16))) float sm[kTile * kZs + kTile * kDs + (RED ? kTile * kZs : 0)];
+    __shared__ float xs[kTile * 3];
+    static_assert(kTile * kSmallStride <= kTile * kZs + kTile * kDs, "lane reduction image");
+    static_assert(kTile * 2 * 8 * sizeof(double) <= sizeof(sm), "column sum image");
+    float* zs = sm;
+    float* ds = sm + kTile * kZs;
+    float* ys = ds + kTile * kDs;
+    const int lane = threadIdx.x, ch = lane % CPR, rl = lane / CPR;
+    float a[VW], b[VW], mu[VW], rs[VW];
+    ld_coef<VW>(scale + ch * VW, a);
+    ld_coef<VW>(shift + ch * VW, b);
+    if (RED) {
+        ld_coef<VW>(mean + ch * VW, mu);
+        ld_coef<VW>(rstd + ch * VW, rs);
+    }
+    f32x4 acc0 = {0.f, 0.f, 0.f, 0.f}, acc1 = {0.f, 0.f, 0.f, 0.f};
+    float small[kNSmall];
+#pragma unroll
+    for (int v = 0; v < kNSmall; ++v) small[v] = 0.f;
+    double s0[VW], s1[VW];
+#pragma unroll
+    for (int k = 0; k < VW; ++k) s0[k] = s1[k] = 0.0;
+
+    const int n_tiles = (n_rows + kTile - 1) / kTile;
     for (int tile = blockIdx.x; tile < n_tiles; tile += gridDim.x) {
-        const int row = tile * 256 + tid;
-        float z[H0], tp[H1], u[H2], du[H2], dtp[H1];
-        if (row < n_rows) {
-            head_forward_row(Y + (int64_t)row * ldy, scale, shift, slope, w, z, tp, u);
-            const float* g = dout + (int64_t)row * 3;
+        const int row0 = tile * kTile;
+        __syncthreads();
+        stage_rows<T>(Y, ldy, row0, n_rows, a, b, slope, zs, RED ? ys : nullptr);
+        stage3_in(dout, row0, n_rows, xs);
+        __syncthreads();
+        float dtp[H1];
+        {
+            float z[H0], tp[H1], u[H2], du[H2];
+            head_mlp(zs + lane * kZs, slope, w, z, tp, u);
+            const float* g = xs + lane * 3;
             if (kind == 0) {
                 du[0] = g[0]; du[1] = g[1]; du[2] = g[2];
             } else {
@@ -120,87 +231,215 @@
                 du[1] = (s * g[1] - k * v1) * (1.f - v1 * v1);
                 du[2] = (s * g[2] - k * v2) * (1.f - v2 * v2);
             }
+            const cptr W2 = at_use(w.W2);
 #pragma unroll
             for (int i = 0; i < H1; ++i) {
                 float s = 0.f;
 #pragma unroll
-                for (int o = 0; o < H2; ++o) s = fmaf(w.W2[o * H1 + i], du[o], s);
+                for (int o = 0; o < H2; ++o) s = fmaf(W2[o * H1 + i], du[o], s);
                 dtp[i] = s * lrelu_grad(tp[i], slope);
-            }
-            T* dz = dZ + (int64_t)row * lddz;
-#pragma unroll
-            for (int q = 0; q < H0 / 4; ++q) {
-                float d[4];
-#pragma unroll
-                for (int e = 0; e < 4; ++e) {
-                    float s = 0.f;
-#pragma unroll
-                    for (int i = 0; i < H1; ++i) s = fmaf(w.W1[i * H0 + q * 4 + e], dtp[i], s);
-                    d[e] = s;
+                small[i] += dtp[i];
+                const float t = lrelu(tp[i], slope);
+#pragma unroll
+                for (int o = 0; o < H2; ++o) small[H1 + o * H1 + i] = fmaf(du[o], t, small[H1 + o * H1 + i]);
+            }
+#pragma unroll
+            for (int o = 0; o < H2; ++o) small[H1 + H2 * H1 + o] += du[o];
+        }
+        lds_st<H1>(ds + lane * kDs, dtp);
+        __syncthreads();
+#pragma unroll 4
+        for (int s = 0; s < kTile / 4; ++s) {
+            const int r = 4 * s + (lane >> 4);
+            const float av = ds[r * kDs + (lane & 15)];
+            const float b0 = zs[r * kZs + (lane & 15)], b1 = zs[r * kZs + 16 + (lane & 15)];
+            acc0 = __builtin_amdgcn_mfma_f32_16x16x4f32(av, b0, acc0, 0, 0, 0);
+            acc1 = __builtin_amdgcn_mfma_f32_16x16x4f32(av, b1, acc1, 0, 0, 0);
+        }
+        __syncthreads();
+        const cptr W1 = at_use(w.W1);
+#pragma unroll
+        for (int q = 0; q < H0 / 4; ++q) {
+            float d[4];
+#pragma unroll
+            for (int e = 0; e < 4; ++e) {
+                float s = 0.f;
+#pragma unroll
+                for (int i = 0; i < H1; ++i) s = fmaf(W1[i * H0 + q * 4 + e], dtp[i], s);
+                d[e] = s;
+            }
+            lds_st<4>(zs + lane * kZs + q * 4, d);
+        }
+        __syncthreads();
+#pragma unroll
+        for (int q = 0; q < CPR; ++q) {
+            const int r = row0 + q * RPI + rl;
+            if (r < n_rows) {
+                float d[VW];
+                lds_ld<VW>(zs + (q * RPI + rl) * kZs + ch * VW, d);
+                Piece<T>::st(dZ + (int64_t)r * lddz + ch * VW, d);
+                if (RED) {
+                    float y[VW];
+                    lds_ld<VW>(ys + (q * RPI + rl) * kZs + ch * VW, y);
+#pragma unroll
+                    for (int k = 0; k < VW; ++k) {
+                        const float g = d[k] * lrelu_grad(fmaf(y[k], a[k], b[k]), slope);
+                        s0[k] += g;
+                        s1[k] = fma((double)g, (double)((y[k] - mu[k]) * rs[k]), s1[k]);
+                    }
                 }
-                store_quad(dz + q * 4, d);
-            }
-        } else {
-#pragma unroll
-            for (int j = 0; j < H0; ++j) z[j] = 0.f;
-#pragma unroll
-            for (int i = 0; i < H1; ++i) { tp[i] = 0.f; dtp[i] = 0.f; }
-            du[0] = du[1] = du[2] = 0.f;
-        }
-        __syncthreads();
-#pragma unroll
-        for (int j = 0; j < H0; ++j) zs[tid][j] = z[j];
-#pragma unroll
-        for (int i = 0; i < H1; ++i) {
-            dtps[tid][i] = dtp[i];
-            ts[tid][i] = row < n_rows ? lrelu(tp[i], slope) : 0.f;
-        }
-        dus[tid][0] = du[0]; dus[tid][1] = du[1]; dus[tid][2] = du[2];
-        __syncthreads();
-        for (int r = 0; r < 256; ++r) {
-            const float zj = zs[r][w1_j];
-            accA = fmaf(dtps[r][w1_i], zj, accA);
-            accB = fmaf(dtps[r][w1_i + 8], zj, accB);
-        }
-        if (tid < H2 * H1) {
-            const int o = tid / H1, i = tid % H1;
-            for (int r = 0; r < 256; ++r) accC = fmaf(dus[r][o], ts[r][i], accC);
-        } else if (tid >= 64 && tid < 64 + H1) {
-            for (int r = 0; r < 256; ++r) accC += dtps[r][tid - 64];
-        } else if (tid >= 128 && tid < 128 + H2) {
-            for (int r = 0; r < 256; ++r) accC += dus[r][tid - 128];
-        }
-    }
-    float* p = partial + (int64_t)blockIdx.x * kNPar;
-    p[w1_i * H0 + w1_j] = accA;
-    p[(w1_i + 8) * H0 + w1_j] = accB;
-    if (tid < H2 * H1) p[H1 * H0 + H1 + tid] = accC;
-    else if (tid >= 64 && tid < 64 + H1) p[H1 * H0 + (tid - 64)] = accC;
-    else if (tid >= 128 && tid < 128 + H2) p[H1 * H0 + H1 + H2 * H1 + (tid - 128)] = accC;
-}
-
-__global__ __launch_bounds__(256) void head_reduce_kernel(const float* __restrict__ partial, int nblk,
-                                                          float* __restrict__ dW1, float* __restrict__ db1,
-                                                          float* __restrict__ dW2, float* __restrict__ db2) {
-    __shared__ double sm[256];
-    const int i = blockIdx.x * 32 + (threadIdx.x & 31), sl = threadIdx.x >> 5;
-    double s = 0.0;
-    if (i < kNPar)
-        for (int b = sl; b < nblk; b += 8) s += (double)partial[(int64_t)b * kNPar + i];
-    sm[threadIdx.x] = s;
+            }
+        }
+    }
+
+    float* p = partial + (int64_t)blockIdx.x * kRec;
+#pragma unroll
+    for (int r = 0; r < 4; ++r) {
+        p[(4 * (lane >> 4) + r) * H0 + (lane & 15)] = acc0[r];
+        p[(4 * (lane >> 4) + r) * H0 + 16 + (lane & 15)] = acc1[r];
+    }
+#pragma unroll
+    for (int v0 = 0; v0 < kNSmall; v0 += kSmallStride - 1) {
+        constexpr int kPer = kSmallStride - 1;
+        __syncthreads();
+#pragma unroll
+        for (int v = 0; v < kPer; ++v)
+            if (v0 + v < kNSmall) sm[lane * kSmallStride + v] = small[v0 + v];
+        __syncthreads();
+        if (lane < kPer && v0 + lane < kNSmall) {
+            float t = 0.f;
+            for (int l = 0; l < kTile; ++l) t += sm[l * kSmallStride + lane];
+            p[H1 * H0 + v0 + lane] = t;
+        }
+    }
+    if (RED) {
+        double* dsm = reinterpret_cast<double*>(sm);
+        __syncthreads();
+#pragma unroll
+        for (int k = 0; k < VW; ++k) {
+            dsm[lane * 2 * VW + k] = s0[k];
+            dsm[lane * 2 * VW + VW + k] = s1[k];
+        }
+        __syncthreads();
+        const int v = lane >> 5, c = lane & 31;
+        double t = 0.0;
+        for (int m = 0; m < RPI; ++m) t += dsm[(m * CPR + c / VW) * 2 * VW + v * VW + c % VW];
+        partial2[(int64_t)blockIdx.x * 64 + lane] = t;
+    }
+}
+
+constexpr int kParBlocks = (kNPar + 31) / 32;
+__global__ __launch_bounds__(1024) void head_reduce_kernel(const float* __restrict__ partial,
+                                                           const double* __restrict__ partial2, int nblk,
+                                                           float* __restrict__ dW1, float* __restrict__ db1,
+                                                           float* __restrict__ dW2, float* __restrict__ db2,
+                                                           double* __restrict__ sums2, FinalizeArgs fin) {
+    __shared__ double sm[2][1024];
+    const int c = threadIdx.x & 31, sl = threadIdx.x >> 5;
+    double t0 = 0.0, t1 = 0.0;
+    if (blockIdx.x < kParBlocks) {
+        const int i = blockIdx.x * 32 + c;
+        if (i < kNPar) {
+            int bk = sl;
+            for (; bk + 224 < nblk; bk += 256) {
+                float v[8];
+#pragma unroll
+                for (int u = 0; u < 8; ++u) v[u] = partial[(int64_t)(bk + 32 * u) * kRec + i];
+#pragma unroll
+                for (int u = 0; u < 8; ++u) t0 += (double)v[u];
+            }
+            for (; bk < nblk; bk += 32) t0 += (double)partial[(int64_t)bk * kRec + i];
+        }
+    } else {
+        int bk = sl;
+        for (; bk + 224 < nblk; bk += 256) {
+            double v[8], x[8];
+#pragma unroll
+            for (int u = 0; u < 8; ++u) {
+                v[u] = partial2[(int64_t)(bk + 32 * u) * 64 + c];
+                x[u] = partial2[(int64_t)(bk + 32 * u) * 64 + 32 + c];
+            }
+#pragma unroll
+            for (int u = 0; u < 8; ++u) {
+                t0 += v[u];
+                t1 += x[u];
+            }
+        }
+        for (; bk < nblk; bk += 32) {
+            t0 += partial2[(int64_t)bk * 64 + c];
+            t1 += partial2[(int64_t)bk * 64 + 32 + c];
+        }
+    }
+    sm[0][threadIdx.x] = t0;
+    sm[1][threadIdx.x] = t1;
     __syncthreads();
-    if (sl != 0 || i >= kNPar) return;
-    double r = 0.0;
-#pragma unroll
-    for (int u = 0; u < 8; ++u) r += sm[threadIdx.x + 32 * u];
-    const float v = (float)r;
-    if (i < H1 * H0) dW1[i] = v;
-    else if (i < H1 * H0 + H1) db1[i - H1 * H0] = v;
-    else if (i < H1 * H0 + H1 + H2 * H1) dW2[i - H1 * H0 - H1] = v;
-    else db2[i - H1 * H0 - H1 - H2 * H1] = v;
-}
-
-int head_bwd_blocks(int64_t n_rows) { return (int)std::max<int64_t>(1, std::min<int64_t>(512, cdiv(n_rows, 256))); }
+    if (sl != 0) return;
+    double r0 = 0.0, r1 = 0.0;
+#pragma unroll
+    for (int u = 0; u < 32; ++u) {
+        r0 += sm[0][c + 32 * u];
+        r1 += sm[1][c + 32 * u];
+    }
+    if (blockIdx.x < kParBlocks) {
+        const int i = blockIdx.x * 32 + c;
+        const float v = (float)r0;
+        if (i < H1 * H0) dW1[i] = v;
+        else if (i < H1 * H0 + H1) db1[i - H1 * H0] = v;
+        else if (i < H1 * H0 + H1 + H2 * H1) dW2[i - H1 * H0 - H1] = v;
+        else if (i < kNPar) db2[i - H1 * H0 - H1 - H2 * H1] = v;
+    } else {
+        sums2[c] = r0;
+        sums2[32 + c] = r1;
+        finalize_column(fin, c, r0, r1);
+    }
+}
+
+int head_blocks(int64_t n_rows) { return (int)std::max<int64_t>(1, std::min<int64_t>(kMaxBlocks, cdiv(n_rows, kTile))); }
+
+template <typename T>
+int head_fwd_launch(const T* Y, int64_t ldy, int64_t n_rows, const float* scale, const float* shift, float slope,
+                    const float* W1, const float* b1, const float* W2, const float* b2, int kind, const float* x_pos,
+                    float* out, ddmp_stream stream) {
+    constexpr int VW = Piece<T>::VW;
+    ARG_TRY(Y && scale && shift && W1 && b1 && W2 && b2 && out && n_rows > 0 && n_rows <= INT32_MAX - kTile);
+    ARG_TRY(ldy >= H0 && ldy % VW == 0 && (kind == 0 || kind == 1) && (kind == 1 || x_pos));
+    ARG_TRY((uintptr_t)Y % 16 == 0);
+    HeadW w{W1, b1, W2, b2};
+    hipLaunchKernelGGL(head_fwd_kernel<T>, dim3(head_blocks(n_rows)), dim3(kTile), 0, (hipStream_t)stream, Y, ldy,
+                       (int)n_rows, scale, shift, slope, w, kind, x_pos, out);
+    LAUNCH_TRY();
+    return DDMP_OK;
+}
+
+size_t head_records_bytes(int nblk) { return (size_t)nblk * kRec * sizeof(float); }
+
+template <typename T>
+int head_bwd_launch(const T* Y, int64_t ldy, int64_t n_rows, const float* scale, const float* shift, float slope,
+                    const float* W1, const float* b1, const float* W2, const float* b2, int kind, const float* dout, T* dZ,
+                    int64_t lddz, float* dW1, float* db1, float* dW2, float* db2, const float* mean, const float* rstd,
+                    double* sums2, void* ws, size_t ws_bytes, ddmp_stream stream, CallCtx& ctx) {
+    constexpr int VW = Piece<T>::VW;
+    ARG_TRY(Y && scale && shift && W1 && b1 && W2 && b2 && dout && dZ && dW1 && db1 && dW2 && db2);
+    ARG_TRY(n_rows > 0 && n_rows <= INT32_MAX - kTile && ldy >= H0 && ldy % VW == 0 && lddz >= H0 && lddz % VW == 0);
+    ARG_TRY((kind == 0 || kind == 1) && (!sums2 || (mean && rstd)));
+    ARG_TRY(((uintptr_t)Y | (uintptr_t)dZ) % 16 == 0);
+    const int nblk = head_blocks(n_rows);
+    if (!ws || ws_bytes < ddmp_head_bwd_workspace_bytes(n_rows)) return DDMP_EWORKSPACE;
+    float* partial = (float*)ws;
+    double* partial2 = (double*)((char*)ws + head_records_bytes(nblk));
+    HeadW w{W1, b1, W2, b2};
+    if (sums2)
+        hipLaunchKernelGGL((head_bwd_kernel<T, true>), dim3(nblk), dim3(kTile), 0, (hipStream_t)stream, Y, ldy, (int)n_rows,
+                           scale, shift, slope, w, kind, dout, dZ, lddz, mean, rstd, partial, partial2);
+    else
+        hipLaunchKernelGGL((head_bwd_kernel<T, false>), dim3(nblk), dim3(kTile), 0, (hipStream_t)stream, Y, ldy, (int)n_rows,
+                           scale, shift, slope, w, kind, dout, dZ, lddz, mean, rstd, partial, partial2);
+    LAUNCH_TRY();
+    hipLaunchKernelGGL(head_reduce_kernel, dim3(kParBlocks + (sums2 ? 1 : 0)), dim3(1024), 0, (hipStream_t)stream, partial,
+                       partial2, nblk, dW1, db1, dW2, db2, sums2, sums2 ? ctx.take_fin(H0) : FinalizeArgs());
+    LAUNCH_TRY();
+    return DDMP_OK;
+}
 
 }
 
@@ -208,19 +447,13 @@
                                  const float* shift, float slope, const float* W1, const float* b1,
                                  const float* W2, const float* b2, int kind, const float* x_pos, float* out,
                                  ddmp_stream stream) {
-    ARG_TRY(Y && scale && shift && W1 && b1 && W2 && b2 && out && n_rows > 0 && n_rows < INT32_MAX);
-    ARG_TRY(ldy >= H0 && ldy % 4 == 0 && (kind == 0 || kind == 1) && (kind == 1 || x_pos));
-    const int grid = (int)std::min<int64_t>(cdiv(n_rows, 256), 256 * 8);
-    HeadW w{W1, b1, W2, b2};
-    hipLaunchKernelGGL(head_fwd_kernel<float>, dim3(grid), dim3(256), 0, (hipStream_t)stream, Y, ldy, (int)n_rows, scale,
-                       shift, slope, w, kind, x_pos, out);
-    LAUNCH_TRY();
-    return DDMP_OK;
+    return head_fwd_launch<float>(Y, ldy, n_rows, scale, shift, slope, W1, b1, W2, b2, kind, x_pos, out, stream);
 }
 
 extern "C" size_t ddmp_head_bwd_workspace_bytes(int64_t n_rows) {
     if (n_rows <= 0) return 0;
-    return (size_t)head_bwd_blocks(n_rows) * kNPar * sizeof(float);
+    const int nblk = head_blocks(n_rows);
+    return head_records_bytes(nblk) + (size_t)nblk * 64 * sizeof(double);
 }
 
 extern "C" int ddmp_head_bwd_f32(const float* Y, int64_t ldy, int64_t n_rows, const float* scale,
@@ -228,50 +461,35 @@
                                  const float* W2, const float* b2, int kind, const float* dout, float* dZ,
                                  int64_t lddz, float* dW1, float* db1, float* dW2, float* db2, void* ws,
                                  size_t ws_bytes, ddmp_stream stream) {
-    ARG_TRY(Y && scale && shift && W1 && b1 && W2 && b2 && dout && dZ && dW1 && db1 && dW2 && db2);
-    ARG_TRY(n_rows > 0 && n_rows < INT32_MAX && ldy >= H0 && ldy % 4 == 0 && lddz >= H0 && lddz % 4 == 0);
-    ARG_TRY(kind == 0 || kind == 1);
-    const int nblk = head_bwd_blocks(n_rows);
-    if (!ws || ws_bytes < (size_t)nblk * kNPar * sizeof(float)) return DDMP_EWORKSPACE;
-    HeadW w{W1, b1, W2, b2};
-    hipLaunchKernelGGL(head_bwd_kernel<float>, dim3(nblk), dim3(256), 0, (hipStream_t)stream, Y, ldy, (int)n_rows, scale,
-                       shift, slope, w, kind, dout, dZ, lddz, (float*)ws);
-    LAUNCH_TRY();
-    hipLaunchKernelGGL(head_reduce_kernel, dim3((unsigned)cdiv(kNPar, 32)), dim3(256), 0, (hipStream_t)stream,
-                       (const float*)ws, nblk, dW1, db1, dW2, db2);
-    LAUNCH_TRY();
-    return DDMP_OK;
+    CallCtx ctx;
+    return head_bwd_launch<float>(Y, ldy, n_rows, scale, shift, slope, W1, b1, W2, b2, kind, dout, dZ, lddz, dW1, db1, dW2,
+                                  db2, nullptr, nullptr, nullptr, ws, ws_bytes, stream, ctx);
 }
 
 
 extern "C" int ddmp_head_fwd_bf16(const uint16_t* Y, int64_t ldy, int64_t n_rows, const float* scale, const float* shift,
                                   float slope, const float* W1, const float* b1, const float* W2, const float* b2,
                                   int kind, const float* x_pos, float* out, ddmp_stream stream) {
-    ARG_TRY(Y && scale && shift && W1 && b1 && W2 && b2 && out && n_rows > 0 && n_rows < INT32_MAX);
-    ARG_TRY(ldy >= H0 && ldy % 8 == 0 && b16_aligned(Y) && (kind == 0 || kind == 1) && (kind == 1 || x_pos));
-    const int grid = (int)std::min<int64_t>(cdiv(n_rows, 256), 256 * 8);
-    HeadW w{W1, b1, W2, b2};
-    hipLaunchKernelGGL(head_fwd_kernel<bf16_t>, dim3(grid), dim3(256), 0, (hipStream_t)stream, Y, ldy, (int)n_rows, scale,
-                       shift, slope, w, kind, x_pos, out);
-    LAUNCH_TRY();
-    return DDMP_OK;
+    return head_fwd_launch<bf16_t>(Y, ldy, n_rows, scale, shift, slope, W1, b1, W2, b2, kind, x_pos, out, stream);
 }
 
 extern "C" int ddmp_head_bwd_bf16(const uint16_t* Y, int64_t ldy, int64_t n_rows, const float* scale, const float* shift,
                                   float slope, const float* W1, const float* b1, const float* W2, const float* b2,
                                   int kind, const float* dout, uint16_t* dZ, int64_t lddz, float* dW1, float* db1,
                                   float* dW2, float* db2, void* ws, size_t ws_bytes, ddmp_stream stream) {
-    ARG_TRY(Y && scale && shift && W1 && b1 && W2 && b2 && dout && dZ && dW1 && db1 && dW2 && db2);
-    ARG_TRY(n_rows > 0 && n_rows < INT32_MAX && ldy >= H0 && ldy % 8 == 0 && lddz >= H0 && lddz % 8 == 0);
-    ARG_TRY((kind == 0 || kind == 1) && b16_aligned(Y) && b16_aligned(dZ));
-    const int nblk = head_bwd_blocks(n_rows);
-    if (!ws || ws_bytes < (size_t)nblk * kNPar * sizeof(float)) return DDMP_EWORKSPACE;
-    HeadW w{W1, b1, W2, b2};
-    hipLaunchKernelGGL(head_bwd_kernel<bf16_t>, dim3(nblk), dim3(256), 0, (hipStream_t)stream, Y, ldy, (int)n_rows, scale,
-                       shift, slope, w, kind, dout, dZ, lddz, (float*)ws);
-    LAUNCH_TRY();
-    hipLaunchKernelGGL(head_reduce_kernel, dim3((unsigned)cdiv(kNPar, 32)), dim3(256), 0, (hipStream_t)stream,
-                       (const float*)ws, nblk, dW1, db1, dW2, db2);
-    LAUNCH_TRY();
-    return DDMP_OK;
-}
+    CallCtx ctx;
+    return head_bwd_launch<bf16_t>(Y, ldy, n_rows, scale, shift, slope, W1, b1, W2, b2, kind, dout, dZ, lddz, dW1, db1, dW2,
+                                   db2, nullptr, nullptr, nullptr, ws, ws_bytes, stream, ctx);
+}
+
+int ddmp_head_bwd(const void* Y, int64_t ldy, int64_t n_rows, int dtype, const float* scale, const float* shift, float slope,
+                  const float* W1, const float* b1, const float* W2, const float* b2, int kind, const float* dout, void* dZ,
+                  int64_t lddz, float* dW1, float* db1, float* dW2, float* db2, const float* mean, const float* rstd,
+                  double* sums2, void* ws, size_t ws_bytes, ddmp_stream stream, CallCtx& ctx) {
+    ARG_TRY(dtype == DDMP_F32 || dtype == DDMP_BF16);
+    if (dtype == DDMP_BF16)
+        return head_bwd_launch<bf16_t>((const bf16_t*)Y, ldy, n_rows, scale, shift, slope, W1, b1, W2, b2, kind, dout,
+                                       (bf16_t*)dZ, lddz, dW1, db1, dW2, db2, mean, rstd, sums2, ws, ws_bytes, stream, ctx);
+    return head_bwd_launch<float>((const float*)Y, ldy, n_rows, scale, shift, slope, W1, b1, W2, b2, kind, dout, (float*)dZ,
+                                  lddz, dW1, db1, dW2, db2, mean, rstd, sums2, ws, ws_bytes, stream, ctx);
+}
diff --git a/dual-dmp_amd/csrc/opts.hip b/dual-dmp_amd/csrc/opts.hip
--- a/dual-dmp_amd/csrc/opts.hip
+++ b/dual-dmp_amd/csrc/opts.hip
@@ -53,6 +53,12 @@
     OptCall c(opts, stream, sums2, C);
     if (c.err) return c.err;
     return c.finish(ddmp_bn_bwd_reduce(dZ, lddz, Y, ldy, n_rows, C, dtype, scale, shift, mean, rstd, slope, sums2, workspace, workspace_bytes, stream, c.ctx));
+}
+
+extern "C" int ddmp_head_bwd_o(const void* Y, int64_t ldy, int64_t n_rows, int dtype, const float* scale, const float* shift, float slope, const float* W1, const float* b1, const float* W2, const float* b2, int kind, const float* dout, void* dZ, int64_t lddz, float* dW1, float* db1, float* dW2, float* db2, const float* mean, const float* rstd, double* sums2, void* workspace, size_t workspace_bytes, ddmp_stream stream, const ddmp_opts* opts) {
+    OptCall c(opts, stream, sums2, 32);
+    if (c.err) return c.err;
+    return c.finish(ddmp_head_bwd(Y, ldy, n_rows, dtype, scale, shift, slope, W1, b1, W2, b2, kind, dout, dZ, lddz, dW1, db1, dW2, db2, mean, rstd, sums2, workspace, workspace_bytes, stream, c.ctx));
 }
 
 extern "C" int ddmp_spmm_stats_o(const ddmp_graph* g, const void* X, int64_t ldx, void* Y, int64_t ldy, int C, int dtype, const float* bias, const float* pro_scale, const float* pro_shift, float slope, const float* ref, double* sums2, void* workspace, size_t workspace_bytes, ddmp_stream stream, const ddmp_opts* opts) {
diff --git a/dual-dmp_amd/engine.py b/dual-dmp_amd/engine.py
--- a/dual-dmp_amd/engine.py
+++ b/dual-dmp_amd/engine.py
@@ -426,11 +426,15 @@
             return {}
 
         torch._foreach_zero_([L.view(grads, "conv%d.bias" % (l + 1)) for l in range(12)])
-        ops.head_bwd(self.Y[11], self.bn4[11], L.view(params, "linear1.weight"), L.view(params, "linear1.bias"),
+        head_args = (self.Y[11], self.bn4[11], L.view(params, "linear1.weight"), L.view(params, "linear1.bias"),
                      L.view(params, "linear2.weight"), L.view(params, "linear2.bias"), self.kind, dout.contiguous(), dZ,
                      L.view(grads, "linear1.weight"), L.view(grads, "linear1.bias"),
-                     L.view(grads, "linear2.weight"), L.view(grads, "linear2.bias"), n_rows=n)
-        have_sums = False
+                     L.view(grads, "linear2.weight"), L.view(grads, "linear2.bias"))
+        have_sums = hasattr(ops, "head_bwd_bnred") and not _unfused("head_red")
+        if have_sums:
+            ops.head_bwd_bnred(*head_args, self.sums, n_rows=n, **arm(11))
+        else:
+            ops.head_bwd(*head_args, n_rows=n)
         fuse_red = hasattr(ops, "spmm_bnred") and (self.dtype == torch.float32
                                                    or not _unfused("bf16_spmm_red"))
 
diff --git a/dual-dmp_amd/ops.py b/dual-dmp_amd/ops.py
--- a/dual-dmp_amd/ops.py
+++ b/dual-dmp_amd/ops.py
@@ -1382,6 +1382,21 @@
     check(st, "ddmp_head_bwd")
 
 
+def head_bwd_bnred(y, bn4, W1, b1, W2, b2, kind, dout, dz, dW1, db1, dW2, db2, sums2, slope=SLOPE, n_rows=None, bn=None):
+    y, ldy = _mat(y, "y")
+    dz, lddz = _mat(dz, "dz", y)
+    n = y.shape[0] if n_rows is None else n_rows
+    L = _lib.lib()
+    ws = Workspace.get(L.ddmp_head_bwd_workspace_bytes(n), y.device)
+    with _timed("head_bwd_bnred", kind, n * (64.0 * y.element_size() + 12)):
+        o, keep = _mk_opts(bn, want_bn=True)
+        st = L.ddmp_head_bwd_o(_p(y), ldy, n, _dt(y), _p(bn4[0]), _p(bn4[1]), slope, _p(W1), _p(b1), _p(W2), _p(b2), kind,
+                               _p(dout), _p(dz), lddz, _p(dW1), _p(db1), _p(dW2), _p(db2), _p(bn4[2]), _p(bn4[3]),
+                               _p(sums2), _p(ws), ws.numel(), _stream(), o)
+    check(st, "ddmp_head_bwd_o")
+    return sums2
+
+
 def grad_sumsq(g, out=None):
     L = _lib.lib()
     if out is None:
diff --git a/include/ddmp_hip.h b/include/ddmp_hip.h
--- a/include/ddmp_hip.h
+++ b/include/ddmp_hip.h
@@ -397,6 +397,10 @@
     float* dW, int64_t lddw, int64_t n_rows, int M, int K, const float* a, const float* b, const float* c1,
     const float* c0, const float* pro_scale , const float* pro_shift , float slope, void* workspace,
     size_t workspace_bytes, ddmp_stream stream, const ddmp_opts* opts);
+int ddmp_head_bwd_o(const void* Y, int64_t ldy, int64_t n_rows, int dtype, const float* scale, const float* shift,
+    float slope, const float* W1, const float* b1, const float* W2, const float* b2, int kind, const float* dout, void* dZ,
+    int64_t lddz, float* dW1, float* db1, float* dW2, float* db2, const float* mean, const float* rstd, double* sums2,
+    void* workspace, size_t workspace_bytes, ddmp_stream stream, const ddmp_opts* opts);
 
 #if defined(__GNUC__)
 #pragma GCC visibility pop
```
